# wreuven/h264-scroll-encoder

Measured on AMD Instinct MI355X. Metric: composed frames/sec (1280x720, 360x360 dyn) at 1/2/4/8 GPU; bit-exact vs CPU, higher is better.
Workload: dtype u8; 1 GPU; BASELINE config 3: 256 concurrent 1280x720 streams + 360x360 synthetic dynamic rect (4x4 int transform + quant + CAVLC), composer_write_scroll_frame semantics; resolution=1280x720, streams_per_gpu=256, parallelism=static stream shard x1, no RCCL

## Files before the change

h264-scroll-encoder_amd/csrc/batch.h:

```cpp
#ifndef SCROLL_BATCH_H
#define SCROLL_BATCH_H

#include <hip/hip_runtime.h>

#include <stddef.h>
#include <stdint.h>

#include <vector>

#include "engine.h"
#include "dyn_engine.h"
#include "splice_engine.h"
#include "ingest_engine.h"
#include "pick_engine.h"

#define HIPCHK(x)                                                                  \
    do {                                                                           \
        hipError_t e_ = (x);                                                       \
        if (e_ != hipSuccess) {                                                    \
            set_err("%s failed: %s", #x, hipGetErrorString(e_));                   \
            return SCROLL_ERR_HIP;                                                 \
        }                                                                          \
    } while (0)

constexpr int NEV = 7;
struct ScrollBatch {
    int device = 0;
    int mode = SCROLL_MODE_COMPOSER;
    int max_streams = 0, max_frames = 0, nstreams = 0;
    int debug = 0;
    size_t arena_bytes = 0, ld_arena = 0;
    int ld_nal = 0;
    DevStream *d_st = nullptr;
    DevStream *h_st = nullptr;
    int32_t *d_off = nullptr;
    NalDesc *d_nal = nullptr;
    uint8_t *d_arena = nullptr;
    hipStream_t own = nullptr;
    hipStream_t last = nullptr;
    hipEvent_t ev[NEV] = {};
    int timing = 0;
    int timed_pending = 0;
    float ms[6] = {0, 0, 0, 0, 0, 0};
    std::vector<hipEvent_t> ring;
    std::vector<uint8_t> ring_dyn;
    int ev_dyn = 0;
    int ring_used = 0;
    double acc_ms[6] = {0, 0, 0, 0, 0, 0};
    int acc_n = 0;
    int host_valid = 1;
    int last_plan_mode = SCROLL_PLAN_COMPOSER;
    int last_nframes = 0;
    std::vector<NalDesc> nal_cache;
    int nal_cache_valid = 0;
    uint64_t *d_dbg = nullptr;
    size_t dbg_slots = 0;
    PlanPending *d_pend = nullptr;
    int dyn_on = 0;
    int dyn_pw = 0, dyn_ph = 0;
    int dyn_refs = 0;
    DynGeom geo{};
    DynFrame *d_dfr = nullptr;
    uint8_t *d_src = nullptr, *d_refs = nullptr, *d_stage = nullptr;
    DynScratch dx{};
    int recon_on = 0;
    uint8_t *d_rec = nullptr;
    unsigned long long *d_sse = nullptr;
    hipEvent_t rc_ev[2] = {};
    int rc_timed = 0;
    int recon_hinted = 0;
    int rc_last_hint = 0;
    std::vector<int> rc_fail;
    struct Probe {
        NalDesc *nal = nullptr;
        DynFrame *dfr = nullptr;
        PlanPending *pend = nullptr;
        uint32_t *rows = nullptr, *ctr = nullptr, *done = nullptr;
        uint4 *heads = nullptr;
        ScrollDynProbe *res = nullptr;
        uint8_t *cls = nullptr;
        int hinted = 0;
        int nframes = -1, nstreams = 0, nq = 0;
        uint8_t qps[SCROLL_DYN_PROBE_MAX_QPS] = {};
        hipEvent_t fin = nullptr;
        hipEvent_t ev[2] = {};
        int timed = 0;
    } pb;
    std::vector<uint8_t> h_qpf;
    int qpf_dev = 0;
    struct Rate {
        long long *level = nullptr;
        uint32_t *fb = nullptr;
        PickOut *out = nullptr;
        hipEvent_t fin = nullptr;
        int nframes = -1, nstreams = 0;
    } rt;
    int hint_on = 0;
    int hint_dirty = 0;
    int hint_max_mb = 0;
    std::vector<std::vector<ScrollHintRect>> h_hint;
    std::vector<int16_t> h_hint_mode;
    HintFrame *d_hf = nullptr;
    ScrollHintRect *d_pool = nullptr;
    size_t pool_cap = 0;
    struct SpliceHost {
        int x0 = 0, y0 = 0, w = 0, h = 0;
        std::vector<uint8_t> nal;
        const uint8_t *dnal = nullptr;
        size_t n = 0;
    };
    std::vector<SpliceHost> h_sp;
    std::vector<int32_t> h_dyn_pos;
    int fallback = 0;
    DynFork fork{};
    std::vector<int32_t> h_dyn_qp;
    int dyn_pos_custom = 0;
    int dyn_qp = 26;
    int hd_dirty = 0;
    uint32_t hd_mb_words = 0;
    size_t dyn_cap = 0;
    int sp_n = 0;
    int sp_dirty = 0;
    int sp_parse = 0;
    SpliceFrame *d_spf = nullptr;
    uint8_t *d_sp_nal = nullptr;
    uint32_t *d_sp_rbsp = nullptr;
    SpliceMbRec *d_sp_rec = nullptr;
    int32_t *d_sp_list = nullptr;
    SpliceUnit *d_sp_units = nullptr;
    int32_t *d_sp_lanes = nullptr;
    size_t sp_lanes_cap = 0, sp_nslots = 0;
    int sp_ymax = 1;
    size_t sp_nal_cap = 0, sp_rbsp_cap = 0, sp_rec_cap = 0, sp_list_cap = 0, sp_units_cap = 0;
    uint8_t *d_ing_in = nullptr;
    size_t ing_in_cap = 0;
    IngestFile *d_ing_files = nullptr;
    IngestScan *d_ing_scan = nullptr;
    IngestOut *d_ing_out = nullptr;
    int ing_cap = 0;
    void *d_ing_work = nullptr;
    size_t ing_work_bytes = 0;
    hipEvent_t ing_ev[2] = {};
    uint32_t *d_ipcm_cnt = nullptr;
    size_t ipcm_cap = 0;
    uint8_t *d_ipcm_stg = nullptr;
    size_t ipcm_stg_cap = 0;
    unsigned long long *d_ipcm_hw = nullptr;
    size_t ipcm_hw_cap = 0;
    uint32_t ipcm_epoch = 0;
    double ipcm_ms = 0.0;
    int ipcm_n = 0;
    uint32_t *ipcm_over = nullptr;
    uint32_t *d_ipcm_sticky = nullptr;
    size_t ipcm_over_stride = 0;
    std::vector<hipEvent_t> ipcm_ev;
    size_t ipcm_ev_used = 0;
    double ing_ms = 0.0;
    int ing_n = 0;
    int dyn_grow = 0;
    int32_t *d_upd = nullptr;
    size_t upd_cap = 0;
    uint64_t *d_out_tab = nullptr;
    size_t out_tab_cap = 0;
    hipEvent_t out_ev = nullptr;
};

#pragma GCC visibility push(hidden)
namespace scroll {
namespace batch {

void set_err(const char *fmt, ...);
int usable_devices(std::vector<int> *ids);
int check_cfg(const ComposerConfig *c);
void cfg_to_dev(const ComposerConfig *c, DevStream *d);
void dev_to_cfg(const DevStream *d, ComposerConfig *c);
hipError_t timing_event(hipEvent_t *e);
int hip_fail(const char *who, hipError_t e, bool clear = false);
int dev_grow(void **p, size_t *cap, size_t n, size_t size, const char *who);
int batch_host_sync(ScrollBatch *b);
int launch(ScrollBatch *b, int nframes, int plan_mode, int nal_max, hipStream_t hs, int plan_flags = 0);
int stream_fail_code(ScrollBatch *b, int s);
int load_nals(ScrollBatch *b);

void probe_release(ScrollBatch *b);
void dyn_release(ScrollBatch *b);
int dyn_grow_pools(ScrollBatch *b);
int dyn_reserve_gen(ScrollBatch *b, size_t need);

void rate_release(ScrollBatch *b);
int qp_frames_any(ScrollBatch *b, bool *any);

int hint_upload(ScrollBatch *b);
int hd_setup(ScrollBatch *b);
int hd_upload(ScrollBatch *b);
int splice_upload(ScrollBatch *b);
int splice_frame_status(ScrollBatch *b, size_t i, int *status);
const char *splice_msg(int e);

int ipcm_async_check(ScrollBatch *b);

}
}
#pragma GCC visibility pop

#endif
```

h264-scroll-encoder_amd/csrc/batch_core.hip:

```cpp
#include <hip/hip_runtime.h>

#include <stdarg.h>
#include <stdint.h>
#include <stdio.h>
#include <stdlib.h>
#include <string.h>

#include <algorithm>
#include <vector>

#include "batch.h"
#include "scroll_engine.h"
#include "dyn_engine.h"
#include "recon_engine.h"
#include "hrecon_engine.h"
#include "hint_engine.h"
#include "splice_engine.h"
#include "hdyn_engine.h"

using namespace scroll::batch;

static void event_ms(const hipEvent_t *e, bool dyn, bool lite, float out[6])
{
    auto el = [&](int a, int b) {
        float v = 0.0f;
        return hipEventElapsedTime(&v, e[a], e[b]) == hipSuccess ? v : 0.0f;
    };
    if (lite) {
        for (int k = 0; k < 6; ++k) out[k] = 0.0f;
        if (dyn) out[2] = out[4] = el(1, 6);
        else out[1] = el(1, 4);
        return;
    }
    if (dyn) {
        out[0] = el(0, 1) + el(2, 3);
        out[1] = el(3, 4);
        out[2] = el(1, 2);
        out[3] = el(4, 5);
        out[4] = el(1, 6);
        out[5] = el(6, 2);
    } else {
        out[0] = el(0, 1);
        out[1] = el(1, 4);
        out[2] = out[3] = out[4] = out[5] = 0.0f;
    }
}

static void fold_ring(ScrollBatch *b)
{
    for (int i = 0; i + NEV <= b->ring_used; i += NEV) {
        float m[6];
        event_ms(&b->ring[i], (b->ring_dyn[i / NEV] & 1) != 0, (b->ring_dyn[i / NEV] & 2) != 0, m);
        for (int k = 0; k < 6; ++k) b->acc_ms[k] += m[k];
        b->acc_n++;
    }
    b->ring_used = 0;
}

static int ring_events(ScrollBatch *b, hipEvent_t **evs)
{
    if ((size_t)b->ring_used + NEV > b->ring.size()) {
        if (b->ring.size() >= (size_t)NEV * 256) {
            HIPCHK(hipStreamSynchronize(b->last));
            fold_ring(b);
        } else {
            for (int i = 0; i < NEV; ++i) {
                hipEvent_t e;
                HIPCHK(timing_event(&e));
                b->ring.push_back(e);
            }
            b->ring_dyn.push_back(0);
        }
    }
    *evs = &b->ring[b->ring_used];
    b->ring_used += NEV;
    return SCROLL_OK;
}

static int dbg_stamps(ScrollBatch *b, size_t slots, hipStream_t hs)
{
    if (slots > b->dbg_slots) {
        if (b->d_dbg) (void)hipFree(b->d_dbg);
        HIPCHK(hipMalloc(&b->d_dbg, slots * 8 * sizeof(uint64_t)));
        b->dbg_slots = slots;
    }
    HIPCHK(hipMemsetAsync(b->d_dbg, 0, slots * 8 * sizeof(uint64_t), hs));
    return SCROLL_OK;
}

static int rc_events(ScrollBatch *b)
{
    if (!b->rc_ev[0]) {
        HIPCHK(hipEventCreate(&b->rc_ev[0]));
        HIPCHK(hipEventCreate(&b->rc_ev[1]));
    }
    return SCROLL_OK;
}

namespace scroll {
namespace batch {

static thread_local char g_err[512];

void set_err(const char *fmt, ...)
{
    va_list ap;
    va_start(ap, fmt);
    vsnprintf(g_err, sizeof(g_err), fmt, ap);
    va_end(ap);
}

int usable_devices(std::vector<int> *ids)
{
    int n = 0;
    if (hipGetDeviceCount(&n) != hipSuccess || n <= 0) {
        set_err("no HIP device visible (libh264scroll needs an MI355X / gfx950)");
        return 0;
    }
    int ok = 0;
    for (int i = 0; i < n; ++i) {
        hipDeviceProp_t p;
        if (hipGetDeviceProperties(&p, i) != hipSuccess) continue;
        if (strncmp(p.gcnArchName, "gfx950", 6) == 0) {
            ok++;
            if (ids) ids->push_back(i);
        }
    }
    if (!ok) set_err("no gfx950 device among %d HIP devices", n);
    return ok;
}

int check_cfg(const ComposerConfig *c)
{
    if (c->log2_max_frame_num < 1 || c->log2_max_frame_num > 16 ||
        (c->pic_order_cnt_type == 0 &&
         (c->log2_max_pic_order_cnt_lsb < 1 || c->log2_max_pic_order_cnt_lsb > 16)) ||
        c->num_waypoints < 0 || c->num_waypoints > MAX_WAYPOINTS || c->width < 0 ||
        c->height < 0) {
        set_err("unsupported ComposerConfig (log2 fields must be 1..16, num_waypoints 0..8)");
        return SCROLL_ERR_CONFIG;
    }
    return SCROLL_OK;
}

void cfg_to_dev(const ComposerConfig *c, DevStream *d)
{
    d->w = c->width;
    d->h = c->height;
    d->log2_mfn = c->log2_max_frame_num;
    d->poc_type = c->pic_order_cnt_type;
    d->log2_poc = c->log2_max_pic_order_cnt_lsb;
    d->deblock = c->deblocking_filter_control_present_flag;
    d->frame_num = c->frame_num;
    d->nwp = c->num_waypoints;
    for (int i = 0; i < 8; ++i) {
        d->wp_off[i] = c->waypoints[i].offset_px;
        d->wp_lt[i] = c->waypoints[i].long_term_idx;
        d->wp_valid[i] = c->waypoints[i].valid;
    }
}

void dev_to_cfg(const DevStream *d, ComposerConfig *c)
{
    c->frame_num = d->frame_num;
    c->num_waypoints = d->nwp;
    for (int i = 0; i < 8; ++i) {
        c->waypoints[i].offset_px = d->wp_off[i];
        c->waypoints[i].long_term_idx = d->wp_lt[i];
        c->waypoints[i].valid = d->wp_valid[i];
    }
}

hipError_t timing_event(hipEvent_t *e)
{
    return hipEventCreateWithFlags(e, hipEventDisableSystemFence);
}

int hip_fail(const char *who, hipError_t e, bool clear)
{
    set_err("%s: %s", who, hipGetErrorString(e));
    if (clear) (void)hipGetLastError();
    return e == hipErrorOutOfMemory ? SCROLL_ERR_OOM : SCROLL_ERR_HIP;
}

int dev_grow(void **p, size_t *cap, size_t n, size_t size, const char *who)
{
    if (n <= *cap) return SCROLL_OK;
    (void)hipFree(*p);
    *p = nullptr;
    *cap = 0;
    hipError_t e = hipMalloc(p, std::max<size_t>(n, 1) * size);
    if (e != hipSuccess) return hip_fail(who, e);
    *cap = n;
    return SCROLL_OK;
}

int batch_host_sync(ScrollBatch *b)
{
    if (b->host_valid) return SCROLL_OK;
    HIPCHK(hipSetDevice(b->device));
    HIPCHK(hipStreamSynchronize(b->last));
    HIPCHK(hipMemcpy(b->h_st, b->d_st, (size_t)b->nstreams * sizeof(DevStream),
                     hipMemcpyDeviceToHost));
    b->host_valid = 1;
    return SCROLL_OK;
}

int launch(ScrollBatch *b, int nframes, int plan_mode, int nal_max, hipStream_t hs, int plan_flags)
{
    int S = b->nstreams;
    if (S == 0) return SCROLL_OK;
    hipEvent_t *rev = nullptr;
    if (b->timing) {
        int rc = ring_events(b, &rev);
        if (rc) return rc;
    }
    const bool hint = b->hint_on && plan_mode != SCROLL_PLAN_EXPLICIT;
    const bool dyn = (b->dyn_on || hint) && plan_mode != SCROLL_PLAN_EXPLICIT;
    const bool lite = b->timing == 2;
    const bool lite_row = lite && dyn && !hint;
    auto mark = [&](int k) -> int {
        if (!b->timing || (!dyn && k != 0 && k != 1 && k != 4)) return SCROLL_OK;
        if (lite) {
            if ((k == 1 || k == (dyn ? 6 : 4)) && !lite_row) HIPCHK(hipEventRecord(rev[k], hs));
            return SCROLL_OK;
        }
        HIPCHK(hipEventRecord(b->ev[k], hs));
        HIPCHK(hipEventRecord(rev[k], hs));
        return SCROLL_OK;
    };
    if (b->timing) {
        b->ring_dyn[(b->ring_used - NEV) / NEV] = (uint8_t)((dyn ? 1 : 0) | (lite ? 2 : 0));
        if (!lite) b->ev_dyn = dyn ? 1 : 0;
    }
    const int ld_fr = b->max_frames;
    const int plan_debug = b->debug & (PLAN_REWIND - 1);
    int rc = mark(0);
    if (rc) return rc;
    if (!dyn) {
        scroll_launch_plan(hs, S, b->d_st, b->d_off, b->max_frames, b->d_nal, b->ld_nal, nframes, plan_mode,
                           plan_debug | plan_flags, b->d_pend, b->d_dfr, ld_fr);
        HIPCHK(hipGetLastError());
        if ((rc = mark(1)) || (rc = mark(2)) || (rc = mark(3))) return rc;
    } else {
        const bool dyn_rect = b->dyn_on && !hint;
        scroll_launch_plan(hs, S, b->d_st, b->d_off, b->max_frames, b->d_nal, b->ld_nal, nframes, plan_mode,
                           plan_debug | plan_flags | PLAN_STATE | PLAN_DYN, b->d_pend, b->d_dfr,
                           ld_fr, nullptr, 0u, 0u, dyn_rect ? b->dx.ctr : nullptr);
        HIPCHK(hipGetLastError());
        if ((rc = mark(1))) return rc;
        uint64_t *stamps = nullptr;
        if (b->debug & SCROLL_DEBUG_DYN_STAMPS) {
            const size_t slots = (2 + (size_t)b->geo.ngroups) * (size_t)nframes * S;
            if ((rc = dbg_stamps(b, slots, hs))) return rc;
            stamps = b->d_dbg + 2 * (size_t)nframes * S * 8;
        }
        b->geo.debug = b->debug;
        if (hint) {
            if (b->sp_parse) {
                if (splice_launch_parse(hs, b->sp_n, b->sp_ymax, b->d_sp_list, b->d_spf, b->d_sp_units,
                                        b->d_sp_lanes, b->sp_nslots, b->d_st, ld_fr, b->d_sp_rbsp, b->d_sp_rec)) {
                    set_err("k_splice_parse launch: %s", hipGetErrorString(hipGetLastError()));
                    return SCROLL_ERR_HIP;
                }
                b->sp_parse = 0;
            }
            if (b->fallback && b->dyn_on &&
                hint_launch_fb(hs, nframes, S, b->d_st, b->d_nal, b->ld_nal, b->d_pend, b->d_dfr, ld_fr,
                               b->d_hf, b->d_pool)) {
                set_err("k_hint_fb launch: %s", hipGetErrorString(hipGetLastError()));
                return SCROLL_ERR_HIP;
            }
            if (hint_launch_stage(hs, nframes, S, b->d_st, b->d_nal, b->ld_nal, b->d_pend,
                                  b->d_dfr, ld_fr, b->d_hf, b->d_pool, b->d_stage,
                                  b->geo.slot_bytes)) {
                set_err("k_hint_stage launch: %s", hipGetErrorString(hipGetLastError()));
                return SCROLL_ERR_HIP;
            }
            const bool combined = b->dyn_on;
            if (combined &&
                hdyn_launch_code(hs, nframes, S, b->d_st, b->d_nal, b->ld_nal, b->d_pend, b->d_dfr, ld_fr,
                                 b->d_hf, b->d_pool, b->d_spf, &b->geo, b->d_src, b->d_refs,
                                 b->d_sp_rec, b->d_sp_rbsp, b->hd_mb_words)) {
                set_err("k_hdyn_code launch: %s", hipGetErrorString(hipGetLastError()));
                return SCROLL_ERR_HIP;
            }
            if (combined && b->recon_on && b->recon_hinted) {
                const bool timed = b->timing != 0;
                if (timed && (rc = rc_events(b))) return rc;
                if (hrecon_launch(hs, nframes, S, b->d_st, b->d_nal, b->ld_nal, b->d_pend, b->d_dfr, ld_fr,
                                  b->d_hf, b->d_pool, b->d_spf, &b->geo, b->d_src, b->d_refs, b->d_rec, b->d_sse,
                                  timed ? b->rc_ev[0] : nullptr, timed ? b->rc_ev[1] : nullptr)) {
                    set_err("k_hdyn_recon launch: %s", hipGetErrorString(hipGetLastError()));
                    return SCROLL_ERR_HIP;
                }
                b->rc_timed = timed ? 1 : 0;
                b->rc_last_hint = 1;
                std::fill(b->rc_fail.begin(), b->rc_fail.end(), 0);
            }
            if ((b->sp_n > 0 || combined) &&
                splice_launch_stage(hs, nframes, S, b->d_st, b->d_nal, b->ld_nal, b->d_pend,
                                    b->d_dfr, ld_fr, b->d_hf, b->d_pool, b->d_spf, b->d_sp_rec,
                                    b->d_sp_rbsp, b->d_stage, b->geo.slot_bytes)) {
                set_err("k_splice_stage launch: %s", hipGetErrorString(hipGetLastError()));
                return SCROLL_ERR_HIP;
            }
            if ((rc = mark(6))) return rc;
        } else {
            b->dx.epoch = b->dx.epoch % 0xffffffu + 1u;
            const DynGeom &G = b->geo;
            const DynFork *fk = nullptr;
            static const bool fork_on = [] {
                const char *e = getenv("SCROLL_DYN_FORK");
                return e && e[0] == '1';
            }();
            if (fork_on) {
                if (!b->fork.side) {
                    HIPCHK(hipStreamCreateWithFlags(&b->fork.side, hipStreamNonBlocking));
                    HIPCHK(hipEventCreateWithFlags(&b->fork.e0, hipEventDisableTiming));
                    HIPCHK(hipEventCreateWithFlags(&b->fork.e1, hipEventDisableTiming));
                }
                fk = &b->fork;
            }
            if (dyn_launch_code(hs, nframes, S, b->d_st, b->d_nal, b->ld_nal, b->d_pend, b->d_dfr, ld_fr, &G,
                                b->d_src, b->d_refs, &b->dx, b->dx.epoch, b->dyn_pw / 16, stamps, fk,
                                lite_row ? rev[1] : nullptr, lite_row ? rev[6] : nullptr)) {
                set_err("k_dyn_code launch: %s", hipGetErrorString(hipGetLastError()));
                return SCROLL_ERR_HIP;
            }
            if ((rc = mark(6))) return rc;
            if (b->recon_on) {
                const bool timed = b->timing != 0;
                if (timed && (rc = rc_events(b))) return rc;
                if (recon_launch(hs, nframes, S, b->d_st, b->d_nal, b->ld_nal, b->d_pend, b->d_dfr, ld_fr, &G,
                                 b->dx.rows, b->d_src, b->d_refs, b->d_rec, b->d_sse, b->dx.ctr,
                                 timed ? b->rc_ev[0] : nullptr, timed ? b->rc_ev[1] : nullptr)) {
                    set_err("k_dyn_recon launch: %s", hipGetErrorString(hipGetLastError()));
                    return SCROLL_ERR_HIP;
                }
                b->rc_timed = timed ? 1 : 0;
                b->rc_last_hint = 0;
            }
            if (dyn_launch_pack(hs, nframes, S, b->d_st, b->d_nal, b->ld_nal, b->d_pend, b->d_dfr, ld_fr, &G,
                                &b->dx, b->d_stage, stamps ? b->d_dbg : nullptr, fk)) {
                set_err("k_dyn_static / k_dyn_epfix launch: %s", hipGetErrorString(hipGetLastError()));
                return SCROLL_ERR_HIP;
            }
        }
        if ((rc = mark(2))) return rc;
        scroll_launch_plan(hs, S, b->d_st, b->d_off, b->max_frames, b->d_nal, b->ld_nal, nframes, plan_mode,
                           plan_debug | plan_flags | PLAN_SIZE | PLAN_DYN, b->d_pend, b->d_dfr,
                           ld_fr, (b->dyn_on && !b->hint_on) ? (const uint32_t *)b->dx.ctr : nullptr,
                           b->geo.rs_spill_cap, b->geo.gen_cap);
        HIPCHK(hipGetLastError());
        if ((rc = mark(3))) return rc;
    }
    const size_t slots = scroll_emit_stamp_slots(nal_max, S);
    if (slots && (b->debug & SCROLL_DEBUG_EMIT_STAMPS) && (rc = dbg_stamps(b, slots, hs))) return rc;
    scroll_launch_emit(hs, S, nal_max, b->d_st, b->d_nal, b->ld_nal, b->d_arena, (uint64_t)b->ld_arena, b->debug,
                       b->d_dbg);
    HIPCHK(hipGetLastError());
    if ((rc = mark(4))) return rc;
    if (dyn && dyn_launch_emit(hs, nframes, S, b->d_st, b->d_nal, b->ld_nal, b->d_dfr, ld_fr,
                               &b->geo, b->d_stage, hint ? nullptr : &b->dx, b->d_arena,
                               (uint64_t)b->ld_arena,
                               (b->debug & SCROLL_DEBUG_DYN_STAMPS) && b->d_dbg
                                   ? b->d_dbg + (size_t)nframes * S * 8 : nullptr)) {
        set_err("k_dyn_gather launch: %s", hipGetErrorString(hipGetLastError()));
        return SCROLL_ERR_HIP;
    }
    if ((rc = mark(5))) return rc;
    if (b->timing == 1) b->timed_pending = 1;
    b->host_valid = 0;
    b->nal_cache_valid = 0;
    b->last = hs;
    return SCROLL_OK;
}

int stream_fail_code(ScrollBatch *b, int s)
{
    const int32_t e = b->h_st[s].err;
    if (!e) return SCROLL_OK;
    if (e & SCROLL_DEVERR_HANDOFF) return SCROLL_ERR_DEVICE;
    if (e & SCROLL_DEVERR_SPLICE) {
        int st = 0;
        for (int ff = 0; ff < b->max_frames && !st; ++ff)
            if (splice_frame_status(b, (size_t)s * b->max_frames + ff, &st)) break;
        return st == HDYN_STATUS_OVERFLOW ? SCROLL_ERR_OVERFLOW : SCROLL_ERR_CONFIG;
    }
    if (e & SCROLL_DEVERR_HINT) return SCROLL_ERR_CONFIG;
    return SCROLL_ERR_OVERFLOW;
}

int load_nals(ScrollBatch *b)
{
    if (b->nal_cache_valid) return SCROLL_OK;
    int rc = batch_host_sync(b);
    if (rc) return rc;
    b->nal_cache.resize((size_t)b->nstreams * b->ld_nal);
    HIPCHK(hipMemcpy(b->nal_cache.data(), b->d_nal, b->nal_cache.size() * sizeof(NalDesc),
                     hipMemcpyDeviceToHost));
    b->nal_cache_valid = 1;
    return SCROLL_OK;
}

}
}

extern "C" {

const char *scroll_last_error(void) { return g_err; }

const char *scroll_version(void) { return "h264scroll-amd 0.1 (gfx950)"; }

int scroll_device_count(void) { return usable_devices(nullptr); }

int scroll_batch_create(ScrollBatch **out, const ScrollBatchDesc *desc)
{
    if (!out || !desc || desc->max_streams <= 0 || desc->max_frames <= 0 ||
        desc->arena_bytes == 0 ||
        (desc->mode != SCROLL_MODE_COMPOSER && desc->mode != SCROLL_MODE_EXPERIMENT)) {
        set_err("scroll_batch_create: bad descriptor");
        return SCROLL_ERR_ARG;
    }
    *out = nullptr;
    std::vector<int> ids;
    if (!usable_devices(&ids)) return SCROLL_ERR_NO_DEVICE;
    int n = 0;
    (void)hipGetDeviceCount(&n);
    if (desc->device < 0 || desc->device >= n) {
        set_err("scroll_batch_create: device %d out of range (%d visible)", desc->device, n);
        return SCROLL_ERR_ARG;
    }
    bool ok = false;
    for (int i : ids) ok |= (i == desc->device);
    if (!ok) {
        set_err("scroll_batch_create: device %d is not gfx950", desc->device);
        return SCROLL_ERR_NO_DEVICE;
    }
    HIPCHK(hipSetDevice(desc->device));
    ScrollBatch *b = new ScrollBatch();
    b->device = desc->device;
    b->mode = desc->mode;
    b->max_streams = desc->max_streams;
    b->max_frames = desc->max_frames;
    b->arena_bytes = desc->arena_bytes;
    b->ld_arena = (desc->arena_bytes + 128 + 255) & ~(size_t)255;
    b->ld_nal = 2 * desc->max_frames;
    size_t S = (size_t)desc->max_streams;
    hipError_t e = hipSuccess;
    if (e == hipSuccess) e = hipMalloc(&b->d_st, S * sizeof(DevStream));
    if (e == hipSuccess) e = hipHostMalloc(&b->h_st, S * sizeof(DevStream), hipHostMallocDefault);
    if (e == hipSuccess) e = hipMalloc(&b->d_off, S * (size_t)desc->max_frames * sizeof(int32_t));
    if (e == hipSuccess) e = hipMalloc(&b->d_nal, S * (size_t)b->ld_nal * sizeof(NalDesc));
    if (e == hipSuccess) e = hipMalloc(&b->d_arena, S * b->ld_arena);
    if (e == hipSuccess) e = hipMalloc(&b->d_pend, S * sizeof(PlanPending));
    if (e == hipSuccess) e = hipStreamCreateWithFlags(&b->own, hipStreamNonBlocking);
    for (int i = 0; i < NEV && e == hipSuccess; ++i) e = timing_event(&b->ev[i]);
    if (e == hipSuccess) e = hipMemset(b->d_st, 0, S * sizeof(DevStream));
    if (e == hipSuccess) e = hipMemset(b->d_off, 0, S * (size_t)desc->max_frames * sizeof(int32_t));
    if (e != hipSuccess) {
        scroll_batch_destroy(b);
        return hip_fail("scroll_batch_create", e);
    }
    memset(b->h_st, 0, S * sizeof(DevStream));
    b->last = b->own;
    *out = b;
    return SCROLL_OK;
}

void scroll_batch_destroy(ScrollBatch *b)
{
    if (!b) return;
    (void)hipSetDevice(b->device);
    if (b->own) (void)hipStreamSynchronize(b->own);
    for (int i = 0; i < NEV; ++i)
        if (b->ev[i]) (void)hipEventDestroy(b->ev[i]);
    for (hipEvent_t e : b->ring) (void)hipEventDestroy(e);
    if (b->fork.side) {
        (void)hipStreamSynchronize(b->fork.side);
        (void)hipStreamDestroy(b->fork.side);
        (void)hipEventDestroy(b->fork.e0);
        (void)hipEventDestroy(b->fork.e1);
    }
    if (b->own) (void)hipStreamDestroy(b->own);
    (void)hipFree(b->d_st);
    (void)hipHostFree(b->h_st);
    (void)hipFree(b->d_off);
    (void)hipFree(b->d_nal);
    (void)hipFree(b->d_arena);
    (void)hipFree(b->d_out_tab);
    (void)hipFree(b->d_upd);
    if (b->out_ev) (void)hipEventDestroy(b->out_ev);
    (void)hipFree(b->d_pend);
    (void)hipFree(b->d_dfr);
    (void)hipFree(b->d_src);
    (void)hipFree(b->d_refs);
    (void)hipFree(b->d_stage);
    (void)hipFree(b->d_rec);
    (void)hipFree(b->d_sse);
    for (hipEvent_t e : b->rc_ev)
        if (e) (void)hipEventDestroy(e);
    probe_release(b);
    (void)hipFree(b->dx.qpf);
    rate_release(b);
    (void)hipFree(b->d_hf);
    (void)hipFree(b->d_pool);
    (void)hipFree(b->d_spf);
    (void)hipFree(b->d_sp_nal);
    (void)hipFree(b->d_sp_rbsp);
    (void)hipFree(b->d_sp_rec);
    (void)hipFree(b->d_sp_list);
    (void)hipFree(b->d_sp_units);
    (void)hipFree(b->d_sp_lanes);
    (void)hipFree(b->d_ing_in);
    (void)hipFree(b->d_ipcm_cnt);
    (void)hipFree(b->d_ipcm_stg);
    (void)hipFree(b->d_ipcm_hw);
    (void)hipFree(b->d_ing_files);
    (void)hipFree(b->d_ing_scan);
    (void)hipFree(b->d_ing_out);
    (void)hipFree(b->d_ing_work);
    for (hipEvent_t e : b->ing_ev)
        if (e) (void)hipEventDestroy(e);
    for (hipEvent_t e : b->ipcm_ev)
        if (e) (void)hipEventDestroy(e);
    (void)hipFree(b->d_ipcm_sticky);
    if (b->d_dbg) (void)hipFree(b->d_dbg);
    delete b;
}

int scroll_batch_num_streams(const ScrollBatch *b) { return b ? b->nstreams : 0; }

int scroll_batch_set_debug(ScrollBatch *b, int flags)
{
    if (!b) return SCROLL_ERR_ARG;
    b->debug = flags;
    return SCROLL_OK;
}

int scroll_batch_add_stream(ScrollBatch *b, const ComposerConfig *cfg)
{
    if (!b || !cfg) return SCROLL_ERR_ARG;
    if (b->nstreams >= b->max_streams) {
        set_err("scroll_batch_add_stream: batch full (%d streams)", b->max_streams);
        return SCROLL_ERR_ARG;
    }
    int rc = check_cfg(cfg);
    if (rc) return rc;
    if (b->dyn_on && (cfg->width != b->dyn_pw || cfg->height != b->dyn_ph)) {
        set_err("scroll_batch_add_stream: the dynamic rect needs %dx%d streams", b->dyn_pw,
                b->dyn_ph);
        return SCROLL_ERR_CONFIG;
    }
    if (b->hint_on && ((cfg->width / 16) * (cfg->height / 16) > b->hint_max_mb ||
                       cfg->width / 16 > HINT_MAX_MBW)) {
        set_err("scroll_batch_add_stream: hint staging slots hold %d MBs per picture, %d per row",
                b->hint_max_mb, HINT_MAX_MBW);
        return SCROLL_ERR_CONFIG;
    }
    rc = batch_host_sync(b);
    if (rc) return rc;
    int s = b->nstreams;
    DevStream *d = &b->h_st[s];
    if (b->dyn_qp != 26 && !cfg->deblocking_filter_control_present_flag) {
        set_err("scroll_batch_add_stream: a stream with the deblocking filter on (no "
                "deblocking_filter_control_present_flag) needs the rect at QP 26, the batch's is %d",
                b->dyn_qp);
        return SCROLL_ERR_CONFIG;
    }
    memset(d, 0, sizeof(*d));
    cfg_to_dev(cfg, d);
    d->dyn_qp = b->dyn_qp;
    d->out_pos = 0;
    d->out_cap = b->arena_bytes;
    HIPCHK(hipSetDevice(b->device));
    HIPCHK(hipMemcpy(b->d_st + s, d, sizeof(DevStream), hipMemcpyHostToDevice));
    b->nstreams++;
    return s;
}

int scroll_batch_get_config(ScrollBatch *b, int s, ComposerConfig *cfg)
{
    if (!b || !cfg || s < 0 || s >= b->nstreams) return SCROLL_ERR_ARG;
    int rc = batch_host_sync(b);
    if (rc) return rc;
    const DevStream *d = &b->h_st[s];
    composer_config_init(cfg, d->w, d->h);
    cfg->log2_max_frame_num = d->log2_mfn;
    cfg->pic_order_cnt_type = d->poc_type;
    cfg->log2_max_pic_order_cnt_lsb = d->log2_poc;
    cfg->deblocking_filter_control_present_flag = d->deblock;
    dev_to_cfg(d, cfg);
    return SCROLL_OK;
}

int scroll_batch_set_config(ScrollBatch *b, int s, const ComposerConfig *cfg)
{
    if (!b || !cfg || s < 0 || s >= b->nstreams) return SCROLL_ERR_ARG;
    int rc = check_cfg(cfg);
    if (rc) return rc;
    rc = batch_host_sync(b);
    if (rc) return rc;
    DevStream *d = &b->h_st[s];
    if (!cfg->deblocking_filter_control_present_flag) {
        bool bad = d->dyn_qp != 26;
        const size_t F = (size_t)b->max_frames, i0 = (size_t)s * F;
        for (size_t f = 0; !bad && f < F && i0 + f < b->h_dyn_qp.size(); ++f) {
            const int q = b->h_dyn_qp[i0 + f];
            bad = q >= 0 && q != 26;
        }
        bool any = false;
        if (!bad && b->dx.qpf && !qp_frames_any(b, &any))
            for (size_t f = 0; !bad && f < F; ++f) bad = b->h_qpf[i0 + f] != 0xFFu && b->h_qpf[i0 + f] != 26u;
        if (bad) {
            set_err("scroll_batch_set_config: stream %d's rect QP is not 26: it cannot turn the deblocking "
                    "filter on (no deblocking_filter_control_present_flag)", s);
            return SCROLL_ERR_CONFIG;
        }
    }
    cfg_to_dev(cfg, d);
    HIPCHK(hipSetDevice(b->device));
    HIPCHK(hipMemcpy(b->d_st + s, d, sizeof(DevStream), hipMemcpyHostToDevice));
    return SCROLL_OK;
}

int scroll_batch_set_offsets(ScrollBatch *b, const int32_t *offsets, int nframes)
{
    if (!b || !offsets || nframes < 0 || nframes > b->max_frames) return SCROLL_ERR_ARG;
    if (nframes == 0 || b->nstreams == 0) return SCROLL_OK;
    HIPCHK(hipSetDevice(b->device));
    HIPCHK(hipMemcpy2D(b->d_off, (size_t)b->max_frames * sizeof(int32_t), offsets,
                       (size_t)nframes * sizeof(int32_t), (size_t)nframes * sizeof(int32_t),
                       (size_t)b->nstreams, hipMemcpyHostToDevice));
    return SCROLL_OK;
}

int32_t *scroll_batch_offsets_device(ScrollBatch *b) { return b ? b->d_off : nullptr; }

int scroll_batch_compose(ScrollBatch *b, int nframes, void *hip_stream)
{
    return scroll_batch_compose_ex(b, nframes, hip_stream, 0);
}

int scroll_batch_compose_ex(ScrollBatch *b, int nframes, void *hip_stream, int flags)
{
    if (!b || nframes < 0 || nframes > b->max_frames) {
        set_err("scroll_batch_compose: nframes %d out of range", nframes);
        return SCROLL_ERR_ARG;
    }
    if (b->dyn_on && !b->dyn_refs) {
        set_err("scroll_batch_compose: dynamic rect without reference pictures");
        return SCROLL_ERR_CONFIG;
    }
    HIPCHK(hipSetDevice(b->device));
    const bool combined = b->hint_on && b->dyn_on;
    if (b->dyn_pos_custom && !b->hint_on) {
        set_err("scroll_batch_compose: per-frame dynamic rect positions need UI hints "
                "(scroll_batch_set_hints)");
        return SCROLL_ERR_CONFIG;
    }
    if (b->recon_on && b->hint_on) {
        bool spliced = b->sp_n > 0;
        for (const ScrollBatch::SpliceHost &sp : b->h_sp) spliced |= sp.w > 0;
        if (!b->recon_hinted || spliced) {
            set_err("scroll_batch_compose: the dynamic rect's reconstruction (scroll_batch_set_dyn_recon) "
                    "covers the plain dynamic rect, and the rect under UI hints with "
                    "scroll_batch_set_dyn_recon_hinted, never spliced slices: clear the hints / splices, opt "
                    "in or turn it off");
            return SCROLL_ERR_CONFIG;
        }
    }
    if (b->hint_on && b->dx.qpf) {
        bool any = false;
        int rc = qp_frames_any(b, &any);
        if (rc) return rc;
        if (any) {
            set_err("scroll_batch_compose: per-frame rect QPs are set (scroll_batch_set_dyn_qp_frames / "
                    "scroll_batch_dyn_pick) and so are UI hints: clear one of them "
                    "(scroll_batch_clear_dyn_qp_frames; under hints: scroll_batch_set_dyn_qp_at)");
            return SCROLL_ERR_CONFIG;
        }
    }
    if (b->hint_on && b->sp_dirty) {
        int rc = splice_upload(b);
        if (rc) return rc;
        if (combined) b->hd_dirty = 1;
    }
    if (combined && b->hd_dirty) {
        int rc = hd_upload(b);
        if (rc) return rc;
    }
    if (b->hint_on && b->hint_dirty) {
        int rc = hint_upload(b);
        if (rc) return rc;
    }
    hipStream_t hs = hip_stream ? (hipStream_t)hip_stream : b->own;
    int plan = b->mode == SCROLL_MODE_EXPERIMENT ? SCROLL_PLAN_EXPERIMENT : SCROLL_PLAN_COMPOSER;
    int nal_max = plan == SCROLL_PLAN_COMPOSER ? 2 * nframes : nframes;
    b->last_plan_mode = plan;
    b->last_nframes = nframes;
    return launch(b, nframes, plan, nal_max, hs,
                  (flags & SCROLL_COMPOSE_REWIND) ? PLAN_REWIND : 0);
}

int scroll_batch_sync(ScrollBatch *b)
{
    if (!b) return SCROLL_ERR_ARG;
    {
        int rc0 = batch_host_sync(b);
        if (rc0) return rc0;
        if ((rc0 = ipcm_async_check(b))) return rc0;
    }
    if (b->timed_pending) {
        event_ms(b->ev, b->ev_dyn != 0, false, b->ms);
        b->timed_pending = 0;
    }
    int rc = SCROLL_OK;
    for (int s = 0; s < b->nstreams; ++s) {
        if (!b->h_st[s].err) continue;
        if (b->rc_last_hint && (size_t)s < b->rc_fail.size())
            b->rc_fail[s] = stream_fail_code(b, s);
        if (rc == SCROLL_OK && (b->h_st[s].err & SCROLL_DEVERR_HANDOFF)) {
            set_err("stream %d: a dynamic-rect row waited past its bound for the row above's "
                    "TotalCoeffs (k_dyn_row hand-off); the stream committed nothing", s);
            rc = SCROLL_ERR_DEVICE;
        } else if (rc == SCROLL_OK && (b->h_st[s].err & SCROLL_DEVERR_SPLICE)) {
            int st = 0, ff = 0;
            for (; ff < b->max_frames && !st; ++ff)
                if (splice_frame_status(b, (size_t)s * b->max_frames + ff, &st)) break;
            if (st == HDYN_STATUS_OVERFLOW) {
                set_err("stream %d frame %d: a dynamic-rect MB under hints outgrew its %u-byte "
                        "region (raise slot_bytes of scroll_batch_set_dyn_rect)", s, ff - 1,
                        4u * b->hd_mb_words);
                rc = SCROLL_ERR_OVERFLOW;
            } else {
                set_err("stream %d frame %d: %s: %s", s, ff - 1,
                        b->dyn_on ? "dynamic rect under hints" : "spliced slice", splice_msg(st));
                rc = SCROLL_ERR_CONFIG;
            }
        } else if (rc == SCROLL_OK && (b->h_st[s].err & SCROLL_DEVERR_HINT)) {
            set_err("stream %d: a hint rect names a reference that is not valid in its frame "
                    "(ref 2 + i needs waypoint i)", s);
            rc = SCROLL_ERR_CONFIG;
        } else if (rc == SCROLL_OK && (b->h_st[s].err & SCROLL_DEVERR_DYN)) {
            uint32_t used[2] = {0, 0};
            if (b->dyn_on && !b->hint_on && b->dx.ctr)
                HIPCHK(hipMemcpy(used, b->dx.ctr, sizeof(used), hipMemcpyDeviceToHost));
            if (used[0] > b->geo.rs_spill_cap || used[1] > b->geo.gen_cap) {
                const int grc = dyn_grow_pools(b);
                set_err("stream %d: the dynamic rect's %s pool ran out (%u of %u); %s", s,
                        used[0] > b->geo.rs_spill_cap ? "row-stage spill" : "general-path record",
                        used[0] > b->geo.rs_spill_cap ? used[0] : used[1],
                        used[0] > b->geo.rs_spill_cap ? b->geo.rs_spill_cap : b->geo.gen_cap,
                        grc ? "growing it failed" : "grown: compose again");
            } else {
                set_err("stream %d: a staged NAL outgrew its staging slot (%llu bytes)", s,
                        (unsigned long long)b->geo.slot_bytes);
            }
            rc = SCROLL_ERR_OVERFLOW;
        } else if (rc == SCROLL_OK) {
            set_err("stream %d: output arena overflow (%llu bytes used, capacity %llu)", s,
                    (unsigned long long)b->h_st[s].out_pos,
                    (unsigned long long)b->h_st[s].out_cap);
            rc = SCROLL_ERR_OVERFLOW;
        }
        b->h_st[s].err = 0;
        HIPCHK(hipMemcpy(&b->d_st[s].err, &b->h_st[s].err, sizeof(int32_t),
                         hipMemcpyHostToDevice));
    }
    if (rc) return rc;
    return SCROLL_OK;
}

size_t scroll_batch_output_size(ScrollBatch *b, int s)
{
    if (!b || s < 0 || s >= b->nstreams || batch_host_sync(b)) return 0;
    return (size_t)b->h_st[s].out_pos;
}

int scroll_batch_copy_output(ScrollBatch *b, int s, size_t from, uint8_t *dst, size_t n)
{
    if (!b || s < 0 || s >= b->nstreams || (!dst && n)) return SCROLL_ERR_ARG;
    int rc = batch_host_sync(b);
    if (rc) return rc;
    if (from + n > b->h_st[s].out_pos) {
        set_err("scroll_batch_copy_output: range beyond stream output");
// ... 178 lines not shown
```

h264-scroll-encoder_amd/csrc/dyn_engine.h:

```cpp
#ifndef SCROLL_DYN_ENGINE_H
#define SCROLL_DYN_ENGINE_H

#include <hip/hip_runtime.h>
#include "engine.h"

typedef struct {
    uint32_t *rows;
    uint16_t *meta;
    uint2 *body_lo, *body_hi;
    uint4 *body_w;
    uint4 *heads;
    unsigned long long *tcx;
    uint32_t *rowstage;
    uint32_t *gbits;
    uint32_t *spill;
    uint32_t *ctr;
    uint32_t ctr_frames;
    uint32_t epoch;
    uint8_t *qpf;
} DynScratch;
#define DYN_HEAD_VECS 16
#define DYN_CTR_LIST 4

typedef struct {
    hipStream_t side;
    hipEvent_t e0, e1;
} DynFork;
int dyn_launch_rows(hipStream_t hs, int nframes, int S, const DevStream *st, const NalDesc *nal, int ld_nal,
                    const PlanPending *pend, DynFrame *dfr, int ld_fr, const DynGeom *g, uint32_t *rows,
                    uint32_t *ctr, uint4 *heads, const uint8_t *qpf);
int dyn_launch_code(hipStream_t hs, int nframes, int S, DevStream *st, const NalDesc *nal,
                    int ld_nal, const PlanPending *pend, DynFrame *dfr, int ld_fr,
                    const DynGeom *g, const uint8_t *src, const uint8_t *refs, const DynScratch *x,
                    uint32_t epoch, int mbw, uint64_t *stamps, const DynFork *fk, hipEvent_t ev0 = nullptr,
                    hipEvent_t ev1 = nullptr);
int dyn_launch_static(hipStream_t hs, int nframes, int S, DevStream *st, const NalDesc *nal, int ld_nal,
                      const PlanPending *pend, DynFrame *dfr, int ld_fr, const DynGeom *g, const DynScratch *x);
int dyn_launch_pack(hipStream_t hs, int nframes, int S, DevStream *st, const NalDesc *nal,
                    int ld_nal, const PlanPending *pend, DynFrame *dfr, int ld_fr,
                    const DynGeom *g, const DynScratch *x, uint8_t *eps, uint64_t *stamps, const DynFork *fk);
int dyn_launch_emit(hipStream_t hs, int nframes, int S, const DevStream *st, const NalDesc *nal,
                    int ld_nal, const DynFrame *dfr, int ld_fr, const DynGeom *g,
                    const uint8_t *stage, const DynScratch *x, uint8_t *arena, uint64_t ld_arena,
                    uint64_t *stamps);
int dyn_launch_synth(hipStream_t hs, int nframes, int S, uint8_t *src, const DynGeom *g,
                     int stream_base, int t0);

void dyn_rowstage_geom(DynGeom *g, int mbw, int mbh);
size_t dyn_slot_bound(int mbw, int mbh, int rw, int rh);
uint32_t dyn_ep_cap(int rw, int rh, int debug);

#endif
```

h264-scroll-encoder_amd/csrc/dyn_kernels.hip:

```cpp
#include <hip/hip_runtime.h>

#include <stdint.h>
#include <mutex>

#include "dyn_device.h"
#include "dyn_engine.h"
#include "nal_ctx.h"
#include "stage_util.h"

using namespace scroll;
using namespace scroll::dyn;
using namespace scroll::stage;

namespace {

__constant__ Tabs g_tabs = SCROLL_DYN_TABS;
constexpr Tabs k_tabs = SCROLL_DYN_TABS;
__constant__ PTabs g_ptabs = make_ptabs(k_tabs);
__device__ uint32_t g_tzrb[TZRB_N];
__constant__ LvTab g_lvt = make_lvt();

struct QpPair {
    QParams l, c;
};
struct QpTab {
    QpPair q[QP_MAX + 1];
};
constexpr QpTab make_qptab()
{
    QpTab T{};
    for (int i = 0; i <= QP_MAX; ++i) T.q[i] = QpPair{qparams(i), qparams(qp_chroma(i))};
    return T;
}
__constant__ QpTab g_qptab = make_qptab();

__global__ __launch_bounds__(256) void k_tzrb_init()
{
    const int i = blockIdx.x * 256 + threadIdx.x;
    if (i < TZRB_N) g_tzrb[i] = i < 65536 ? tzrb_entry(g_tabs, (uint32_t)i, 16) : tzrb_entry(g_tabs, (uint32_t)(i - 65536), 15);
}

__device__ inline void load_ptabs(PTabs &dst, int t, int nthr)
{
    constexpr int N = (int)(sizeof(PTabs) / 16);
    static_assert(sizeof(PTabs) % 16 == 0, "PTabs copies as uint4");
    for (int i = t; i < N; i += nthr) reinterpret_cast<uint4 *>(&dst)[i] = reinterpret_cast<const uint4 *>(&g_ptabs)[i];
}

__device__ inline void load_rowtabs(RowTabs &dst, int t, int nthr)
{
    constexpr int NC = (int)(sizeof(dst.ct) / 4), NZ = (int)(sizeof(dst.tzdc) / 4), NR = (int)(sizeof(dst.rb) / 4);
    static_assert(sizeof(dst.ct) % 4 == 0 && sizeof(dst.tzdc) % 4 == 0 && sizeof(dst.rb) % 4 == 0, "word copies");
    const uint32_t *ct = reinterpret_cast<const uint32_t *>(g_ptabs.ct);
    const uint32_t *tz = reinterpret_cast<const uint32_t *>(g_ptabs.tzdc);
    const uint32_t *rb = reinterpret_cast<const uint32_t *>(g_ptabs.rb);
    uint32_t *dc = reinterpret_cast<uint32_t *>(dst.ct), *dz = reinterpret_cast<uint32_t *>(dst.tzdc);
    uint32_t *dr = reinterpret_cast<uint32_t *>(dst.rb);
    for (int i = t; i < NC + NZ + NR; i += nthr) {
        if (i < NC) dc[i] = ct[i];
        else if (i < NC + NZ) dz[i - NC] = tz[i - NC];
        else dr[i - NC - NZ] = rb[i - NC - NZ];
    }
}


constexpr int HEAD_MAX = 160;
constexpr int HDR_MAX = 1024;
constexpr int OBUF = 6400;

constexpr uint32_t DF_OVER = 1u, DF_GENERAL = 2u, DF_HANDOFF = 4u;
constexpr uint64_t HANDOFF_TICKS = 5000000ull;
constexpr uint64_t HANDOFF_GAP = 100000ull;
constexpr uint32_t DF_EPSLOW = 0x100u;
constexpr uint32_t DF_FIXED = 0x200u;

constexpr int EPC_ROW = 256, EPC_STATIC = 4096;

__device__ inline uint32_t ep_data(uint32_t w, uint32_t gi, uint32_t bits)
{
    const uint32_t b0 = 32u * gi;
    if (__builtin_expect(b0 + 32u <= bits, 1)) return w;
    return w | (bits > b0 ? 0xffffffffu >> (bits - b0) : 0xffffffffu);
}

__device__ inline uint32_t ep_run_starts(uint32_t pw, uint32_t w, uint32_t nx, uint32_t gi, uint32_t bits)
{
    uint64_t X = (uint64_t)ep_data(w, gi, bits) << 32 | ep_data(nx, gi + 1u, bits);
    X |= X << 1;
    X |= X << 2;
    X |= X << 4;
    X |= X << 8;
    X |= X << 6;
    const uint32_t z22 = ~(uint32_t)(X >> 32);
    return z22 & ((ep_data(w, gi, bits) >> 1) | (pw << 31));
}

__device__ inline bool ep_quick(uint32_t w, uint32_t nx)
{
    uint32_t y = w | w << 1;
    y |= y << 2;
    y |= y << 4;
    y |= y << 8;
    y |= y << 6;
    const uint32_t tz = w ? (uint32_t)__builtin_ctz(w) : 32u, lz = nx ? (uint32_t)__builtin_clz(nx) : 32u;
    return (~y & 0xffe00000u) != 0u || tz + lz >= 22u;
}

__device__ inline void flush_window(const uint32_t *buf, uint32_t n, uint32_t p0, bool last, uint32_t *out,
                                    uint32_t *ncand, uint32_t *cg, uint32_t cmax, int t, int nthr)
{
    const int lane = t & 63;
    for (uint32_t i0 = 0; i0 < n; i0 += (uint32_t)nthr) {
        const uint32_t i = i0 + (uint32_t)t;
        bool q = false;
        if (i < n) {
            const uint32_t w = buf[i];
            out[p0 + i] = w;
            q = ep_quick(w, i + 1 < n ? buf[i + 1] : (last ? 0xffffffffu : 0u));
        }
        const uint64_t m = __builtin_amdgcn_ballot_w64(q);
        if (m) {
            uint32_t base = 0;
            if (lane == (int)__builtin_ctzll(m)) base = atomicAdd(ncand, (uint32_t)__builtin_popcountll(m));
            base = (uint32_t)__shfl((int)base, (int)__builtin_ctzll(m), 64);
            const uint32_t k = base + (uint32_t)__builtin_popcountll(m & ((1ull << lane) - 1ull));
            if (q && k < cmax) cg[1 + k] = p0 + i;
        }
    }
}

__device__ inline uint32_t ld32(const uint8_t *p) { return *reinterpret_cast<const uint32_t *>(p); }

constexpr int NPC = DYN_PIECES;

__device__ inline void put_body(uint2 *BL, uint2 *BH, size_t i, uint4 v, bool hi)
{
    BL[i] = make_uint2(v.x, v.y);
    if (hi) BH[i] = make_uint2(v.z, v.w);
}

__device__ inline uint4 get_body(const uint2 *BL, const uint2 *BH, size_t i, bool hi)
{
    const uint2 a = BL[i], b = hi ? BH[i] : make_uint2(0u, 0u);
    return make_uint4(a.x, a.y, b.x, b.y);
}

__device__ inline int rec_of(int q, int pc, int ndt)
{
    return pc < 16 ? 16 * q + pc : (pc < 18 ? 24 * ndt + 2 * q + (pc - 16) : 16 * ndt + 8 * q + (pc - 18));
}
constexpr uint32_t M_OVF = 1u << 15;
constexpr uint32_t ROW_GEN = 1u << 31, ROW_OFF = 0x0fffffffu;

#ifndef SCROLL_CODE_T
#define SCROLL_CODE_T 256
#endif
constexpr int CODE_T = SCROLL_CODE_T, CODE_NW = CODE_T / 64;
#ifndef SCROLL_SORT_KEYS
#define SCROLL_SORT_KEYS 9
#endif
constexpr int SORT_KEYS = SCROLL_SORT_KEYS;
static_assert(SORT_KEYS >= 2 && SORT_KEYS <= 17, "TotalCoeff classes");

__device__ inline void code_frame(const DevStream *__restrict__ st,
                                                     const DynFrame *__restrict__ dfr, int ld_fr,
                                                     const PlanPending *__restrict__ pend,
                                                     const NalDesc *__restrict__ nal, int ld_nal,
                                                     DynGeom g, const uint32_t *__restrict__ rows,
                                                     const uint8_t *__restrict__ src,
                                                     const uint8_t *__restrict__ refs,
                                                     uint16_t *__restrict__ meta, uint2 *__restrict__ blo,
                                                     uint2 *__restrict__ bhi, uint4 *__restrict__ bwd, int s,
                                                     int f, int bx)
{
    __shared__ uint4 lv[CODE_T];
    __shared__ int16_t lw[CODE_T][16];
    __shared__ uint16_t wc[CODE_NW][SORT_KEYS];
    __shared__ uint16_t order[CODE_T];
    __shared__ PTabs ptabs;
    __shared__ int32_t wo[8], wv[8];
    const int t = threadIdx.x;
    const int lane = t & 63, wave = t >> 6;
    const DynFrame df = dfr[(size_t)s * ld_fr + f];
    if (df.nal < 0 || !(df.err & DF_GENERAL)) return;
    load_ptabs(ptabs, t, CODE_T);
    if (t < 8) {
        wo[t] = pend[s].wo[t];
        wv[t] = pend[s].wv[t];
    }
    __syncthreads();

    const int ndt = g.w * g.h, ntask = 24 * ndt;
    const int task = bx * CODE_T + t;
    const int qpy = __builtin_amdgcn_readfirstlane((int)df.ep);
    const QParams ql = qparams_rt(qpy), qc = qparams_rt(qp_chroma(qpy));
    const bool wide = qpy < QP_MIN;
    const size_t nb = (size_t)s * ld_fr + f;
    const uint32_t *rw = rows + nb * (size_t)(32 * g.h);
    const int w = st[s].w, h = st[s].h;
    const uint32_t ysz = (uint32_t)w * (uint32_t)h, csz = ysz / 4;
    const uint8_t *rb = refs + (size_t)s * g.ref_ld;
    const uint8_t *fs = src + (size_t)s * g.src_ld + (size_t)f * g.src_fr;
    const int lstride = 16 * g.w, cstride = 8 * g.w;
    const uint8_t *fcb = fs + (size_t)256 * ndt, *fcr = fcb + (size_t)64 * ndt;
    const uint32_t m_rw = magic32((uint32_t)g.w);
    const size_t gs = df.rbsp_bytes;
    uint16_t *M = meta + gs * (size_t)(NPC * ndt);
    uint2 *BL = blo + gs * (size_t)(NPC * ndt), *BH = bhi + gs * (size_t)(NPC * ndt);
    uint4 *BW = bwd + gs * (size_t)(NPC * ndt);

    const bool luma = task < 16 * ndt;
    const bool act = task < ntask;
    int k, r, p = 0;
    if (luma) {
        k = task >> 4;
        r = task & 15;
    } else {
        const int jj = task - 16 * ndt;
        k = jj >> 3;
        p = (jj >> 2) & 1;
        r = jj & 3;
    }
    const int ry = (int)div_m((uint32_t)k, m_rw), cx = k - ry * g.w;
    const int col = g.x0 + cx;
    uint32_t pk[4] = {0, 0, 0, 0};
    int n = 0, w0 = 0;
    if (act && luma) {
        const int bx = r & 3, by = r >> 2;
        const uint8_t *sp = fs + (size_t)(16 * ry + 4 * by) * lstride + 16 * cx + 4 * bx;
        const uint8_t *pp = rb + 16 * col + 4 * bx;
        const uint32_t *re = rw + 16 * ry + 4 * by;
        uint32_t sv[4], pv[4];
#pragma unroll
        for (int i = 0; i < 4; ++i) {
            sv[i] = ld32(sp + (size_t)i * lstride);
            pv[i] = ld32(pp + re[i]);
        }
        int res[16], W[16];
#pragma unroll
        for (int i = 0; i < 4; ++i)
#pragma unroll
            for (int x = 0; x < 4; ++x)
                res[4 * i + x] = (int)((sv[i] >> (8 * x)) & 255u) - (int)((pv[i] >> (8 * x)) & 255u);
        fwd4x4(res, W);
#pragma unroll
        for (int k2 = 0; k2 < 16; ++k2) {
            const int v = quant(W[ZZ[k2]], ZZ[k2], ql);
            pk[k2 >> 2] |= ((uint32_t)v & 255u) << (8 * (k2 & 3));
            if (wide) lw[t][k2] = (int16_t)v;
            n += v != 0;
        }
    } else if (act) {
        const int bx = r & 1, by = r >> 1;
        const uint8_t *sp = (p ? fcr : fcb) + (size_t)(8 * ry + 4 * by) * cstride + 8 * cx + 4 * bx;
        const int X = 8 * col + 4 * bx;
        const uint8_t *cp = rb + (size_t)p * csz + X;
        const uint32_t *re = rw + 16 * g.h + 8 * ry + 4 * by;
        int res[16], W[16];
#pragma unroll
        for (int i = 0; i < 4; ++i) {
            const uint32_t sv = ld32(sp + (size_t)i * cstride);
            const uint32_t ea = re[i];
            int pred[4];
            if (!(ea & ROW_GEN)) {
                const uint32_t fr = (ea >> 28) & 7u;
                const uint32_t av = ld32(cp + (ea & ROW_OFF));
                const uint32_t bv = fr ? ld32(cp + (re[8 * g.h + i] & ROW_OFF)) : 0u;
#pragma unroll
                for (int x = 0; x < 4; ++x) {
                    const int a = (int)((av >> (8 * x)) & 255u), b = (int)((bv >> (8 * x)) & 255u);
                    pred[x] = ((8 - (int)fr) * a + (int)fr * b + 4) >> 3;
                }
            } else {
                {
                    const NalDesc d = nal[(size_t)s * ld_nal + df.nal];
                    const int off = d.off, a_end = (h - off) / 16;
                    const int row = g.y0 + ry;
                    int32_t wl0[8] = {0, 0, 0, 0, 0, 0, 0, 0};
                    const NalCtx c = nal_ctx(st + s, d, wo, wl0, wv);
                    const Regions rg = regions(c);
                    const bool cA = row < a_end;
                    const int ref = cA ? rg.ra : rg.rb, q = 4 * (cA ? rg.mva : rg.mvb);
                    const int o = q >> 3, fr = q & 7;
                    const WpTab T{wo, wv, h};
                    RefPics P;
                    P.w = w;
                    P.h = h;
                    const size_t pic = (size_t)ysz + 2 * csz;
                    for (int i2 = 0; i2 < 2; ++i2) {
                        P.pl[i2][0] = rb + i2 * pic;
                        P.pl[i2][1] = P.pl[i2][0] + ysz;
                        P.pl[i2][2] = P.pl[i2][1] + csz;
                    }
                    const int ya = 8 * row + 4 * by + i + o;
                    for (int x = 0; x < 4; ++x) {
                        const int a = chroma_px_any<9>(T, P, ref, 1 + p, X + x, ya);
                        const int b = fr ? chroma_px_any<9>(T, P, ref, 1 + p, X + x, ya + 1) : 0;
                        pred[x] = ((8 - fr) * a + fr * b + 4) >> 3;
                    }
                }
            }
#pragma unroll
            for (int x = 0; x < 4; ++x) res[4 * i + x] = (int)((sv >> (8 * x)) & 255u) - pred[x];
        }
        fwd4x4(res, W);
        w0 = W[0];
#pragma unroll
        for (int k2 = 1; k2 < 16; ++k2) {
            const int v = quant(W[ZZ[k2]], ZZ[k2], qc);
            pk[(k2 - 1) >> 2] |= ((uint32_t)v & 255u) << (8 * ((k2 - 1) & 3));
// ... 32 lines not shown
            CapSink cap{0, 0, 0};
            const int tc = cavlc_dc4(cap, ptabs, dq);
            const size_t idx = (size_t)24 * ndt + 2 * k + p;
            if (cap.n <= 128) {
                M[idx] = (uint16_t)(cap.n | (uint32_t)tc << 8);
                if (cap.n)
                    put_body(BL, BH, idx, make_uint4((uint32_t)cap.lo, (uint32_t)(cap.lo >> 32), (uint32_t)cap.hi,
                                                     (uint32_t)(cap.hi >> 32)), cap.n > 64);
            } else {
                M[idx] = (uint16_t)((uint32_t)tc << 8 | M_OVF);
                put_body(BL, BH, idx, make_uint4(((uint32_t)dq[0] & 0xffffu) | (uint32_t)dq[1] << 16,
                                                 ((uint32_t)dq[2] & 0xffffu) | (uint32_t)dq[3] << 16, 0u, 0u), false);
            }
        }
        if (t < SORT_KEYS) {
            uint32_t tot = 0;
#pragma unroll
            for (int w2 = 0; w2 < CODE_NW; ++w2) tot += wc[w2][t];
            uint32_t kb = tot;
#pragma unroll
            for (int d = 1; d < 32; d <<= 1) {
                const uint32_t o = __shfl_up(kb, d, 64);
                if (lane >= d) kb += o;
            }
            uint32_t run = kb - tot;
#pragma unroll
            for (int w2 = 0; w2 < CODE_NW; ++w2) {
                const uint32_t c = wc[w2][t];
                wc[w2][t] = (uint16_t)run;
                run += c;
            }
        }
        __syncthreads();
        order[wc[wave][key] + below] = (uint16_t)t;
    }
    __syncthreads();
    const int u = order[t];
    const int tk = bx * CODE_T + u;
    const uint4 v4 = lv[u];
    const bool ul = tk < 16 * ndt;
    CapSink cap{0, 0, 0};
    int t1 = 0;
    bool ok = true;
    int tc = 0;
    if (tk < ntask && !wide) {
        tc = cavlc_body(cap, ptabs, v4, ul ? 16 : 15, t1, ok);
    } else if (tk < ntask) {
        const int max = ul ? 16 : 15;
        tc = tc_t1_of(lw[u], max, t1);
        uint32_t tv;
        int tl;
        coeff_token(g_tabs, tc, t1, 0, tv, tl);
        SkipSink<CapSink> sk{cap, (uint32_t)tl};
        cavlc_block(sk, g_tabs, lw[u], max, 0);
        ok = cap.n <= 128;
    }
    if (tk < ntask) {
        const uint16_t mm = ok ? (uint16_t)(cap.n | (uint32_t)tc << 8 | (uint32_t)t1 << 13)
                               : (uint16_t)((uint32_t)tc << 8 | (uint32_t)t1 << 13 | M_OVF);
        M[tk] = mm;
        uint4 ov = v4;
        if (wide && !ok) {
            const uint4 *l2 = reinterpret_cast<const uint4 *>(lw[u]);
            ov = l2[0];
            BW[tk] = l2[1];
        }
        if ((mm & 255u) || (mm & M_OVF))
            put_body(BL, BH, tk,
                     ok ? make_uint4((uint32_t)cap.lo, (uint32_t)(cap.lo >> 32), (uint32_t)cap.hi,
                                     (uint32_t)(cap.hi >> 32))
                        : ov,
                     (mm & 255u) > 64u || (mm & M_OVF));
    }
}

#ifndef SCROLL_CODE_GEN_Y
#define SCROLL_CODE_GEN_Y 64
#endif
constexpr int CODE_GEN_Y = SCROLL_CODE_GEN_Y;
__global__ __launch_bounds__(CODE_T) void k_dyn_code_general(const DevStream *__restrict__ st,
                                                             const DynFrame *__restrict__ dfr, int ld_fr,
                                                             const PlanPending *__restrict__ pend,
                                                             const NalDesc *__restrict__ nal, int ld_nal,
                                                             DynGeom g, const uint32_t *__restrict__ rows,
                                                             const uint8_t *__restrict__ src,
                                                             const uint8_t *__restrict__ refs,
                                                             uint16_t *__restrict__ meta,
                                                             uint2 *__restrict__ blo, uint2 *__restrict__ bhi,
                                                             uint4 *__restrict__ bwd, const uint32_t *__restrict__ ctr)
{
    const uint32_t n = min(__builtin_amdgcn_readfirstlane(ctr[1]), g.gen_cap);
    for (uint32_t j = blockIdx.y; j < n; j += gridDim.y) {
        const uint32_t q = __builtin_amdgcn_readfirstlane(ctr[DYN_CTR_LIST + j]);
        const int s = (int)(q / (uint32_t)ld_fr), f = (int)(q - (uint32_t)s * (uint32_t)ld_fr);
        code_frame(st, dfr, ld_fr, pend, nal, ld_nal, g, rows, src, refs, meta, blo, bhi, bwd, s, f, blockIdx.x);
        __syncthreads();
    }
}

struct LdsOrWin {
    uint32_t *b;
    uint32_t lo, n;
    __device__ inline void operator()(uint32_t i, uint32_t v) const
    {
        const uint32_t k = i - lo;
        if (k < n) atomicOr(&b[k], v);
    }
};
typedef OrSink<LdsOrWin> WSink;


__device__ inline int tc_of(uint32_t m) { return (int)((m >> 8) & 31u); }

struct HeadSel {
    int a_end, mbw;
    __device__ inline int sel(int row, int col) const
    {
        const bool curA = row < a_end, abvA = (row - 1) < a_end;
        return 3 * (row == 0 ? 0 : (curA ? 1 : (abvA ? 2 : 3))) + (col == 0 ? 0 : (col == mbw - 1 ? 2 : 1));
    }
};
struct HeadCtx : HeadSel {
    Regions rg;
    int nrefs;
    template <class S>
    __device__ inline void put_class(S &sk, int cls) const
    {
        const int ty = cls / 3, pos = cls - 3 * ty;
        const int x = pos == 0 ? 0 : (pos == 1 ? min(1, mbw - 1) : mbw - 1);
        const bool cur = ty == 0 ? 0 < a_end : ty == 1;
        const bool abv = ty == 1 || ty == 2;
        const int ref = cur ? rg.ra : rg.rb, mv4 = 4 * (cur ? rg.mva : rg.mvb);
        const int aref = abv ? rg.ra : rg.rb, amv4 = 4 * (abv ? rg.mva : rg.mvb);
        int px, py;
        predict(x, ty == 0 ? 0 : 1, mbw, ref, mv4, aref, amv4, px, py);
        put_mb_head(sk, ref, 0 - px, mv4 - py, nrefs);
    }
    template <class S>
    __device__ inline void put_slow(S &sk, int row, int col) const
    {
        const bool curA = row < a_end, abvA = (row - 1) < a_end;
        const int ref = curA ? rg.ra : rg.rb, mv4 = 4 * (curA ? rg.mva : rg.mvb);
        const int aref = abvA ? rg.ra : rg.rb, amv4 = 4 * (abvA ? rg.mva : rg.mvb);
        int px, py;
        predict(col, row, mbw, ref, mv4, aref, amv4, px, py);
        put_mb_head(sk, ref, 0 - px, mv4 - py, nrefs);
    }
};

__device__ inline HeadCtx head_ctx(const NalCtx &c)
{
    HeadCtx H;
    H.rg = regions(c);
    H.a_end = (c.h - c.off) / 16;
    H.mbw = c.w / 16;
    H.nrefs = 2 + c.nwp;
    return H;
}

__device__ inline HeadSel head_sel(const DevStream *S, const NalDesc &d)
{
    HeadSel H;
    H.a_end = (S->h - d.off) / 16;
    H.mbw = S->w / 16;
    return H;
}

__device__ inline uint32_t row_static_bits(const HeadCtx &H, const uint32_t *hlen, int row, const Rect &R)
{
    const int mbw = H.mbw;
    const bool in = row >= R.y0 && row < R.y0 + R.h;
    auto isdyn = [&](int col) { return in && col >= R.x0 && col < R.x0 + R.w; };
    const int base = H.sel(row, 0) - 0;
    uint32_t bits = isdyn(0) ? 0u : hlen[base] + 1u;
    if (mbw >= 2) {
        if (!isdyn(mbw - 1)) bits += hlen[base + 2] + 1u;
        int nmid = mbw - 2;
        if (in) nmid -= max(0, min(R.x0 + R.w, mbw - 1) - max(R.x0, 1));
        bits += (uint32_t)nmid * (hlen[base + 1] + 1u);
    }
    return bits;
}

__device__ inline void lb_store(unsigned long long *p, uint64_t v)
{
    __hip_atomic_store(p, v, __ATOMIC_RELAXED, __HIP_MEMORY_SCOPE_AGENT);
}

__host__ __device__ inline uint64_t rs_group_words(const DynGeom &g, int nA, int gi)
{
    if (gi < nA) return (uint64_t)gi * g.rs_static_words;
    if (gi < nA + g.h) return (uint64_t)nA * g.rs_static_words + (uint64_t)(gi - nA) * g.rs_row_words;
    return (uint64_t)(gi - g.h) * g.rs_static_words + (uint64_t)g.h * g.rs_row_words;
}

__host__ __device__ inline uint64_t rs_runs_words(const DynGeom &g, int nA, int gi)
{
    const bool row = gi >= nA && gi < nA + g.h;
    return rs_group_words(g, nA, gi) + (row ? g.rs_row_words - EPC_ROW : g.rs_static_words - EPC_STATIC);
}

constexpr uint32_t LO_LEN = 0x7ffu;

__device__ inline void piece_token(const uint16_t (*ct)[68], uint32_t mv, int nC, uint32_t &tv, uint32_t &tl)
{
    const int tc = tc_of(mv), t1 = (int)((mv >> 13) & 3u);
    if (nC >= 8) {
        tv = tc ? (uint32_t)(((tc - 1) << 2) | t1) : 3u;
        tl = 6;
    } else {
        const uint32_t e = ct[nC < 2 ? 0 : (nC < 4 ? 1 : 2)][4 * tc + t1];
        tv = e & 255u;
        tl = e >> 8;
    }
}

__device__ inline void wave_sync()
{
    __builtin_amdgcn_fence(__ATOMIC_RELEASE, "wavefront");
    __builtin_amdgcn_wave_barrier();
    __builtin_amdgcn_fence(__ATOMIC_ACQUIRE, "wavefront");
}

template <int CTRL, int ROWS>
__device__ inline uint32_t dpp_or0(uint32_t v)
{
    return (uint32_t)__builtin_amdgcn_update_dpp(0, (int)v, CTRL, ROWS, 0xf, false);
}

__device__ inline uint32_t seg32_incl_sum(uint32_t v)
{
    v += dpp_or0<0x111, 0xf>(v);
    v += dpp_or0<0x112, 0xf>(v);
    v += dpp_or0<0x114, 0xf>(v);
    v += dpp_or0<0x118, 0xf>(v);
    v += dpp_or0<0x142, 0xa>(v);
    return v;
}

__device__ inline uint32_t wave_incl_sum_dpp(uint32_t v)
{
    v = seg32_incl_sum(v);
    v += dpp_or0<0x143, 0xc>(v);
    return v;
}

template <class S>
__device__ inline void ovf_code(S &sk, const PTabs &PT, const Tabs &TB, uint4 bd, const uint4 *bw, int pc, int nC)
{
    if (nC == -1) {
        const int dq[4] = {(int)(int16_t)(bd.x & 0xffffu), (int)(int16_t)(bd.x >> 16),
                           (int)(int16_t)(bd.y & 0xffffu), (int)(int16_t)(bd.y >> 16)};
        cavlc_dc4(sk, PT, dq);
    } else if (bw) {
        const uint4 hi = *bw;
        const uint32_t w8[8] = {bd.x, bd.y, bd.z, bd.w, hi.x, hi.y, hi.z, hi.w};
        int16_t l16[16];
#pragma unroll
        for (int i = 0; i < 8; ++i) {
            l16[2 * i] = (int16_t)(w8[i] & 0xffffu);
            l16[2 * i + 1] = (int16_t)(w8[i] >> 16);
        }
        cavlc_block(sk, TB, l16, pc < 16 ? 16 : 15, nC);
    } else {
        const int8_t *lvp = reinterpret_cast<const int8_t *>(&bd);
        cavlc_block(sk, TB, lvp, pc < 16 ? 16 : 15, nC);
    }
}

__device__ __attribute__((noinline)) uint32_t ovf_bits(const PTabs &PT, const Tabs &TB, uint4 bd, const uint4 *bw,
                                                       int pc, int nC)
{
    CountSink cn{0};
    ovf_code(cn, PT, TB, bd, bw, pc, nC);
    return cn.n;
}

typedef __attribute__((address_space(3))) uint32_t *LdsWords;
__device__ __attribute__((noinline)) void ovf_put(LdsWords win, uint32_t lo, uint32_t n, uint32_t pos,
                                                  const PTabs &PT, const Tabs &TB, uint4 bd, const uint4 *bw, int pc,
                                                  int nC)
{
    uint32_t *buf = (uint32_t *)win;
    WSink sk{LdsOrWin{buf, lo, n}, 0, 0, 0};
    sk.start(pos);
    ovf_code(sk, PT, TB, bd, bw, pc, nC);
    sk.finish();
}

__device__ inline uint4 body_msb(uint64_t hi, uint64_t lo, uint32_t n)
{
    const uint32_t k = 128u - n;
    uint64_t H, Lw;
    if (k >= 64u) {
        H = k >= 128u ? 0ull : lo << (k - 64u);
        Lw = 0ull;
    } else {
        H = k ? (hi << k) | (lo >> (64u - k)) : hi;
        Lw = lo << k;
    }
    return make_uint4((uint32_t)(H >> 32), (uint32_t)H, (uint32_t)(Lw >> 32), (uint32_t)Lw);
}

__global__ __launch_bounds__(256) void k_dyn_rows(const DevStream *__restrict__ st,
                                                  const NalDesc *__restrict__ nal, int ld_nal,
                                                  const PlanPending *__restrict__ pend,
                                                  DynFrame *__restrict__ dfr, int ld_fr, DynGeom g,
                                                  uint32_t *__restrict__ rows, uint32_t *__restrict__ ctr,
                                                  uint4 *__restrict__ heads, const uint8_t *__restrict__ qpf)
{
    __shared__ int32_t wo[8], wl[8], wv[8];
    __shared__ int32_t gen;
    const int s = blockIdx.y, f = blockIdx.x, t = threadIdx.x;
    DynFrame *DF = dfr + (size_t)s * ld_fr + f;
    const int j = DF->nal;
    if (j < 0) return;
    if (t < 8) {
        wo[t] = pend[s].wo[t];
        wl[t] = pend[s].wl[t];
        wv[t] = pend[s].wv[t];
    }
    if (t == 0) gen = 0;
    __syncthreads();
    const DevStream *S = st + s;
    const NalDesc d = nal[(size_t)s * ld_nal + j];
    const NalCtx c = nal_ctx(S, d, wo, wl, wv);
    if (t < 12) {
        const HeadCtx H = head_ctx(c);
        CapSink hc{0, 0, 0};
        H.put_class(hc, t);
        uint4 *hv = heads + ((size_t)s * ld_fr + f) * DYN_HEAD_VECS;
        hv[t] = body_msb(hc.hi, hc.lo, min(hc.n, 128u));
        reinterpret_cast<uint32_t *>(hv + 12)[t] = hc.n | (hc.over() ? 0x80000000u : 0u);
    }
    const Regions rg = regions(c);
    const int w = c.w, h = c.h, a_end = (h - c.off) / 16;
    const uint32_t ysz = (uint32_t)w * (uint32_t)h, pic = ysz + ysz / 2;
    const WpTab T{wo, wv, h};
    uint32_t *rw = rows + ((size_t)s * ld_fr + f) * (size_t)(32 * g.h);
    bool my_gen = false;
    for (int i = t; i < 32 * g.h; i += 256) {
        uint32_t e;
        if (i < 16 * g.h) {
            const int Y = 16 * g.y0 + i, row = Y >> 4;
            const bool cA = row < a_end;
            int yo;
            const int b = luma_row(T, cA ? rg.ra : rg.rb, Y + (cA ? rg.mva : rg.mvb), yo);
            e = (uint32_t)b * pic + (uint32_t)yo * (uint32_t)w;
        } else {
            const int i2 = i - 16 * g.h, bot = i2 >= 8 * g.h;
            const int Y = 8 * g.y0 + (bot ? i2 - 8 * g.h : i2), row = Y >> 3;
            const bool cA = row < a_end;
            const int q = 4 * (cA ? rg.mva : rg.mvb), o = q >> 3, fr = q & 7;
            int yo;
            const int b = chroma_row(T, cA ? rg.ra : rg.rb, Y + o + bot, yo);
            if (b < 0) {
                e = ROW_GEN;
                if (!bot || fr) my_gen = true;
            } else {
                e = ((uint32_t)b * pic + ysz + (uint32_t)yo * (uint32_t)(w / 2)) | (uint32_t)fr << 28;
            }
        }
        rw[i] = e;
    }
    const uint32_t qe = qpf ? qpf[(size_t)s * ld_fr + f] : 0xFFu;
    const int qpy = qe <= 51u ? (int)qe : S->dyn_qp;
    if (my_gen || qpy < QP_MIN) gen = 1;
    __syncthreads();
    if (t == 0) {
        uint32_t e = 0u;
        if (gen) {
            const uint32_t k = atomicAdd(&ctr[1], 1u);
            if (k < g.gen_cap) {
                DF->rbsp_bytes = k;
                ctr[DYN_CTR_LIST + k] = (uint32_t)((size_t)s * ld_fr + f);
                e = DF_GENERAL;
            } else {
                e = DF_OVER;
            }
        }
        DF->err = e;
        DF->ep = (uint32_t)qpy;
    }
}

constexpr int GW = 64;
#ifndef SCROLL_GBUF_WORDS
#define SCROLL_GBUF_WORDS 256
#endif
constexpr int GBUF_WORDS = SCROLL_GBUF_WORDS;

struct StaticFixed {
    uint32_t ncand;
    uint32_t buf[GBUF_WORDS];
    uint64_t hhi[12], hlo[12];
    uint4 pat[12];
    uint32_t hlen[12];
    int32_t head_over;
    int32_t wo[8], wl[8], wv[8];
    uint32_t moff[DYN_STATIC_ROWS + 1];
};

__global__ __launch_bounds__(GW) void k_dyn_static(const DevStream *__restrict__ st,
                                                   const NalDesc *__restrict__ nal, int ld_nal,
                                                   const PlanPending *__restrict__ pend,
                                                   const DynFrame *__restrict__ dfr, int ld_fr, DynGeom g,
                                                   uint32_t *__restrict__ rowstage, uint32_t *__restrict__ gbits)
{
    __shared__ StaticFixed L;
    constexpr int SR = DYN_STATIC_ROWS;
    const Rect R{g.x0, g.y0, g.w, g.h};
    const int nA = max(1, (R.y0 + SR - 1) / SR);
    const int gi = (int)blockIdx.x >= nA ? (int)blockIdx.x + R.h : (int)blockIdx.x;
    const int ng = g.ngroups, f = blockIdx.y, s = blockIdx.z, t = threadIdx.x;
    const size_t nb = (size_t)s * ld_fr + f;
    const DynFrame df = dfr[nb];
    const int j = df.nal;
    if (j < 0) return;
    const bool first = gi == 0, last = gi == ng - 1;
    if (t < 8) {
        L.wo[t] = pend[s].wo[t];
        L.wl[t] = pend[s].wl[t];
        L.wv[t] = pend[s].wv[t];
    }
    if (t == 0) {
        L.head_over = 0;
        L.ncand = 0;
    }
    const DevStream *S = st + s;
    const NalDesc d = nal[(size_t)s * ld_nal + j];
    wave_sync();
    NalCtx c = nal_ctx(S, d, L.wo, L.wl, L.wv);
    c.qpd = (int)df.ep - QP_DEFAULT;
    const HeadCtx H = head_ctx(c);
    const int mbw = H.mbw, mbh = c.h / 16;
    int ra, rb;
    if (gi < nA) {
        ra = gi * SR;
        rb = min(ra + SR, R.y0);
    } else {
        ra = R.y0 + R.h + (gi - nA - R.h) * SR;
        rb = min(ra + SR, mbh);
    }
    uint32_t F = 0;
    if (first) {
        CountSink hc{0};
        emit_slice_header(hc, c);
        F = hc.n;
    }
    if (t < 12) {
        CapSink hc{0, 0, 0};
        H.put_class(hc, t);
        L.hhi[t] = hc.hi;
        L.hlo[t] = hc.lo;
        L.hlen[t] = hc.n;
        if (hc.over()) L.head_over = 1;
        if (hc.n < 128u) {
            const uint64_t hi = (hc.hi << 1) | (hc.lo >> 63), lo = (hc.lo << 1) | 1u;
            L.pat[t] = body_msb(hi, lo, hc.n + 1u);
        } else {
            L.head_over = 1;
        }
    }
    wave_sync();
    const bool head_over = L.head_over;
    auto head_bits = [&](int r, int col) -> uint32_t {
        if (!head_over) return L.hlen[H.sel(r, col)];
        CountSink cn{0};
        H.put_slow(cn, r, col);
        return cn.n;
    };
    uint32_t len = 0;
    const int r = ra + t;
    if (r < rb) {
        if (!head_over) {
            len = row_static_bits(H, L.hlen, r, R);
        } else {
            for (int col = 0; col < mbw; ++col) len += head_bits(r, col) + 1u;
        }
    }
    const uint32_t incl = wave_incl_sum(len, t);
    if (r < rb) L.moff[r - ra] = F + incl - len;
    const uint32_t rows_end = F + __shfl(incl, GW - 1, GW);
    if (t == 0) L.moff[rb - ra] = rows_end;
    const uint32_t bits = rows_end + (last ? 1u : 0u);
    if (t == 0) gbits[nb * (size_t)ng + gi] = bits;
    wave_sync();

    uint32_t *out = rowstage + nb * g.rs_frame_words + rs_group_words(g, nA, gi);
    const uint32_t nw = min((bits + 31u) >> 5, g.rs_static_words - EPC_STATIC);
    const int ne = rb - ra;
    auto cnt_le = [&](uint32_t x) -> int {
        int lo = 0, hi = ne + 1;
        while (lo < hi) {
            const int mid = (lo + hi) >> 1;
            if (L.moff[mid] <= x) lo = mid + 1;
            else hi = mid;
        }
        return lo;
    };
    const uint32_t m_mbw = magic32((uint32_t)mbw);
    for (uint32_t p0 = 0; p0 < nw; p0 += GBUF_WORDS) {
        const uint32_t n = min((uint32_t)GBUF_WORDS, nw - p0);
        for (uint32_t i = (uint32_t)t; i < n; i += GW) L.buf[i] = 0u;
        wave_sync();
        const LdsOrWin win{L.buf, p0, n};
        if (head_over && first && t == 0 && p0 * 32u < F) {
            WSink hs{win, 0, 0, 0};
            hs.start(0);
            emit_slice_header(hs, c);
            hs.finish();
        }
        if (!head_over) {
            const uint32_t rbeg = L.moff[0], rend = L.moff[ne];
            for (uint32_t i = (uint32_t)t; i < n; i += GW) {
                const uint32_t W0 = 32u * (p0 + i), W1 = W0 + 32u;
                uint32_t acc = 0, b = max(W0, rbeg), R0 = 0, R1 = 0, L0 = 0, Lm = 1;
                int b3 = 0;
                float inv = 1.0f;
                while (b < W1 && b < rend) {
                    if (b >= R1 || b < R0) {
                        const int e = cnt_le(b) - 1;
                        R0 = L.moff[e];
                        R1 = L.moff[e + 1];
                        b3 = H.sel(ra + e, 0);
                        L0 = L.hlen[b3] + 1u;
                        Lm = L.hlen[b3 + 1] + 1u;
                        inv = 1.0f / (float)Lm;
                    }
                    const uint32_t o = b - R0;
                    uint32_t cl = (uint32_t)b3, off = o;
                    if (o >= L0) {
                        const uint32_t o2 = o - L0;
                        uint32_t q = (uint32_t)((float)o2 * inv);
                        if (q * Lm > o2) --q;
                        else if ((q + 1u) * Lm <= o2) ++q;
                        if (q < (uint32_t)(mbw - 2)) {
                            cl = (uint32_t)b3 + 1u;
                            off = o2 - q * Lm;
                        } else {
                            cl = (uint32_t)b3 + 2u;
                            off = o2 - (uint32_t)(mbw - 2) * Lm;
                        }
                    }
                    const uint32_t k = min(L.hlen[cl] + 1u - off, W1 - b);
                    const uint4 P = L.pat[cl];
                    const uint32_t wi = off >> 5, sh = off & 31u;
                    const uint32_t w0 = wi == 0 ? P.x : (wi == 1 ? P.y : (wi == 2 ? P.z : P.w));
                    const uint32_t w1 = wi == 0 ? P.y : (wi == 1 ? P.z : (wi == 2 ? P.w : 0u));
                    uint32_t v = sh ? __builtin_amdgcn_alignbit(w0, w1, 32u - sh) : w0;
                    v &= k >= 32u ? 0xffffffffu : ~(0xffffffffu >> k);
                    acc |= v >> (b - W0);
                    b += k;
                }
                L.buf[i] = acc;
            }
            wave_sync();
            if (first && t == 0 && p0 * 32u < F) {
                WSink hs{win, 0, 0, 0};
                hs.start(0);
                emit_slice_header(hs, c);
                hs.finish();
            }
            if (last && t == 0) {
                WSink sk{win, 0, 0, 0};
                sk.start(bits - 1u);
                sk.put(1, 1);
                sk.finish();
            }
            wave_sync();
            flush_window(L.buf, n, p0, p0 + n >= nw, out, &L.ncand,
                         rowstage + nb * g.rs_frame_words + rs_runs_words(g, nA, gi), EPC_STATIC - 1, t, GW);
            wave_sync();
            continue;
        }
        const int ea = max(cnt_le(32u * p0) - 1, 0), eb = min(cnt_le(32u * (p0 + n) - 1u), ne);
        const int nm = eb * mbw;
        for (int m = ea * mbw + t; m < nm; m += GW) {
            const int rr = (int)div_m((uint32_t)m, m_mbw), col = m - rr * mbw, rw = ra + rr;
            uint32_t off = L.moff[rr];
            WSink sk{win, 0, 0, 0};
            if (!head_over) {
                const int b3 = H.sel(rw, 0);
                off += col == 0 ? 0u : L.hlen[b3] + 1u + (uint32_t)(col - 1) * (L.hlen[b3 + 1] + 1u);
                if (off >= 32u * (p0 + n)) continue;
                const int cls = b3 + (col == 0 ? 0 : (col == mbw - 1 ? 2 : 1));
                if (off + L.hlen[cls] + 1u <= 32u * p0) continue;
                sk.start(off);
                sk.put_cap(CapSink{L.hhi[cls], L.hlo[cls], L.hlen[cls]});
            } else {
                for (int c2 = 0; c2 < col; ++c2) off += head_bits(rw, c2) + 1u;
                sk.start(off);
                H.put_slow(sk, rw, col);
            }
            sk.put(1, 1);
            sk.finish();
        }
        if (last && t == 0) {
            WSink sk{win, 0, 0, 0};
            sk.start(bits - 1u);
            sk.put(1, 1);
            sk.finish();
        }
        wave_sync();
        flush_window(L.buf, n, p0, p0 + n >= nw, out, &L.ncand,
                     rowstage + nb * g.rs_frame_words + rs_runs_words(g, nA, gi), EPC_STATIC - 1, t, GW);
        wave_sync();
    }
    if (t == 0) rowstage[nb * g.rs_frame_words + rs_runs_words(g, nA, gi)] = L.ncand;
}


__device__ inline CapSink cap_of_msb(uint64_t a, uint64_t b, uint32_t n)
{
    if (n == 0u) return CapSink{0, 0, 0};
    const uint32_t sh = 128u - n;
    if (sh >= 64u) return CapSink{0, a >> (sh - 64u), n};
    if (sh == 0u) return CapSink{a, b, n};
    return CapSink{a >> sh, (b >> sh) | (a << (64u - sh)), n};
}

__device__ inline void put_piece(uint32_t *buf, uint32_t p0, uint32_t n, uint32_t pos, uint32_t tv, uint32_t tl,
                                 uint4 b, uint32_t bl)
{
    const uint32_t tw = tv & low_mask((int)tl);
    const uint32_t c0 = __builtin_amdgcn_alignbit(tw, b.x, tl), c1 = __builtin_amdgcn_alignbit(b.x, b.y, tl);
    const uint32_t c2 = __builtin_amdgcn_alignbit(b.y, b.z, tl), c3 = __builtin_amdgcn_alignbit(b.z, b.w, tl);
    const uint32_t c4 = __builtin_amdgcn_alignbit(b.w, 0u, tl);
    const uint32_t sh = pos & 31u;
    const uint32_t o[6] = {c0 >> sh, __builtin_amdgcn_alignbit(c0, c1, sh), __builtin_amdgcn_alignbit(c1, c2, sh),
                           __builtin_amdgcn_alignbit(c2, c3, sh), __builtin_amdgcn_alignbit(c3, c4, sh),
                           __builtin_amdgcn_alignbit(c4, 0u, sh)};
    const uint32_t nw = (sh + tl + bl + 31u) >> 5, w0 = (pos >> 5) - p0;
#pragma unroll
    for (uint32_t j = 0; j < 6; ++j)
        if (j < nw && w0 + j < n && o[j]) atomicOr(&buf[w0 + j], o[j]);
}

constexpr uint32_t ROW_PAD = 4;

__device__ inline void put_piece1(uint32_t *buf, uint32_t pos, uint32_t tv, uint32_t tl, uint4 b, uint32_t bl)
{
    const uint32_t tw = tv & low_mask((int)tl);
    const uint32_t c0 = __builtin_amdgcn_alignbit(tw, b.x, tl), c1 = __builtin_amdgcn_alignbit(b.x, b.y, tl);
    const uint32_t c2 = __builtin_amdgcn_alignbit(b.y, b.z, tl), c3 = __builtin_amdgcn_alignbit(b.z, b.w, tl);
    const uint32_t c4 = __builtin_amdgcn_alignbit(b.w, 0u, tl);
    const uint32_t sh = pos & 31u, nw = (sh + tl + bl + 31u) >> 5;
    uint32_t *d = buf + (pos >> 5);
    atomicOr(d, c0 >> sh);
    if (nw > 1u) atomicOr(d + 1, __builtin_amdgcn_alignbit(c0, c1, sh));
    if (nw > 2u) atomicOr(d + 2, __builtin_amdgcn_alignbit(c1, c2, sh));
    if (nw > 3u) {
        atomicOr(d + 3, __builtin_amdgcn_alignbit(c2, c3, sh));
        if (nw > 4u) {
            atomicOr(d + 4, __builtin_amdgcn_alignbit(c3, c4, sh));
            if (nw > 5u) atomicOr(d + 5, __builtin_amdgcn_alignbit(c4, 0u, sh));
        }
    }
}

constexpr int ROW_MAXT = 1024;
#ifndef SCROLL_ROW_WAVES
#define SCROLL_ROW_WAVES 8
#endif
#ifndef SCROLL_ROW_NP
#define SCROLL_ROW_NP 3
#endif
#ifndef SCROLL_ROW_NP_WIDE
#define SCROLL_ROW_NP_WIDE 4
#endif
#ifndef SCROLL_ROW_WIDE
#define SCROLL_ROW_WIDE 40
#endif
constexpr int ROW_NPMAX = 8;
#ifndef SCROLL_ROW_GB
#define SCROLL_ROW_GB 896
#endif
constexpr int ROW_GB = SCROLL_ROW_GB;

struct RowFixed {
    RowTabs ptabs;
    union {
        uint32_t buf[ROW_GB + 4];
        struct {
            uint32_t kc[2][SORT_KEYS];
            uint32_t kc_pad[32 - 2 * SORT_KEYS];
            uint32_t lvt[LVT_N];
        };
    };
    uint64_t hhi[12], hlo[12];
    uint32_t hlen[12];
    int32_t wo[8], wl[8], wv[8];
    int32_t head_over;
    uint32_t rt[32];
    uint32_t ncand;
    uint32_t spill;
    uint32_t pcd[NPC];
};

static_assert(2 * SORT_KEYS <= 32 && 32 + LVT_N <= ROW_GB, "the sort counts and the level table share the bit window");
static_assert(ROW_PAD == 4, "RowFixed::buf holds ROW_PAD spare words");
static_assert(offsetof(RowFixed, lvt) % 8 == 0, "the level table is copied in 8-byte words");

__host__ __device__ inline size_t row_lds_base(int w)
{
    return (size_t)16 * NPC * w + (size_t)4 * (w + 1) + (size_t)2 * (3 * NPC * w) + (size_t)10 * w + 16;
}
#ifndef SCROLL_ROW_GB_WIDE
#define SCROLL_ROW_GB_WIDE 1248
#endif
constexpr int ROW_GB_WIDE = SCROLL_ROW_GB_WIDE;
__host__ __device__ inline size_t row_wide_off(int w) { return (row_lds_base(w) + 15) & ~(size_t)15; }
__host__ __device__ inline bool row_wide_win(int w)
{
    return w > SCROLL_ROW_WIDE && row_wide_off(w) + 4 * (size_t)(ROW_GB_WIDE + ROW_PAD) + sizeof(RowFixed) <= 163840;
}
__host__ __device__ inline size_t row_lds_bytes(int w)
{
    return row_wide_win(w) ? row_wide_off(w) + 4 * (size_t)(ROW_GB_WIDE + ROW_PAD) : row_lds_base(w);
}

__host__ __device__ constexpr uint32_t pc_desc(int pc)
{
    if (pc == 16 || pc == 17) return 1u << 17;
    int da = 0, db = 0, e = 0;
    bool al = false, bt = false;
    if (pc < 16) {
        const int bx = pc & 3, by = pc >> 2;
        al = bx == 0;
        da = al ? 3 - NPC : -1;
        bt = by == 0;
        db = bt ? 0 : -4;
        e = bt ? pc : 0;
    } else {
        const int b = (pc - 18) & 3, bx = b & 1, by = b >> 1;
        al = bx == 0;
        da = al ? 1 - NPC : -1;
        bt = by == 0;
        db = bt ? 0 : -2;
        e = bt ? (pc < 22 ? pc - 14 : pc - 16) : 0;
    }
    return (uint32_t)(da + 32) | (al ? 1u : 0u) << 6 | (uint32_t)(db + 32) << 7 | (bt ? 1u : 0u) << 13 |
           (uint32_t)e << 14;
}

struct EpfLds {
    uint32_t *goff, *gb, *gw, *cw, *cbase, *lst, *cnt;
    uint32_t *ws;
};
__host__ __device__ inline int row_chroma0(int w) { return (16 * w + 63) & ~63; }
__host__ __device__ inline int row_vtasks(int w) { return row_chroma0(w) + 8 * w; }

__host__ __device__ inline int row_threads(int w)
{
    const int nt = row_vtasks(w), np = w > SCROLL_ROW_WIDE ? SCROLL_ROW_NP_WIDE : SCROLL_ROW_NP;
    const int a = (((nt + np - 1) / np) + 63) & ~63;
    const int b = (((nt + ROW_NPMAX - 1) / ROW_NPMAX) + 63) & ~63;
    const int t = a > b ? a : b;
    return t < ROW_MAXT ? t : ROW_MAXT;
}

struct BlkPix {
    uint32_t a[4], b[4], c;
};

__device__ inline __amdgpu_buffer_rsrc_t buf_rsrc(const void *p, uint32_t n)
{
    return __builtin_amdgcn_make_buffer_rsrc(const_cast<void *>(p), (short)0, (int)n, 0x00020000);
}

struct FetchOff {
    uint32_t s, b[4], c;
    int pb;
};

__device__ inline void fetch_luma(FetchOff &o, int v, int ry, const DynGeom &g, const uint32_t *rt)
{
    const int k = v >> 4, r = v & 15, bx = r & 3, by = r >> 2;
    o.s = (uint32_t)((16 * ry + 4 * by) * (16 * g.w) + 16 * k + 4 * bx);
    const uint32_t po = (uint32_t)(16 * (g.x0 + k) + 4 * bx);
#pragma unroll
    for (int i = 0; i < 4; ++i) o.b[i] = po + rt[4 * by + i];
    o.c = o.b[3];
}

__device__ inline void fetch_chroma(FetchOff &o, int e, int ry, const DynGeom &g, uint32_t csz, const uint32_t *ru,
                                    const uint32_t *rd)
{
    const int ndt = g.w * g.h, k = e >> 3, p = (e >> 2) & 1, r = e & 3, bx = r & 1, by = r >> 1;
    o.s = (uint32_t)(256 * ndt + (p ? 64 * ndt : 0) + (8 * ry + 4 * by) * (8 * g.w) + 8 * k + 4 * bx);
    const uint32_t co = (uint32_t)p * csz + (uint32_t)(8 * (g.x0 + k) + 4 * bx);
#pragma unroll
    for (int i = 0; i < 4; ++i) o.b[i] = co + (ru[4 * by + i] & ROW_OFF);
    o.c = co + (rd[4 * by + 3] & ROW_OFF);
}

__device__ inline void fetch_pass9(const FetchOff &o, uint32_t adv, uint32_t stride, __amdgpu_buffer_rsrc_t fs,
                                   __amdgpu_buffer_rsrc_t rb, BlkPix &px)
{
#pragma unroll
    for (int i = 0; i < 4; ++i) {
        px.a[i] = __builtin_amdgcn_raw_buffer_load_b32(fs, o.s, adv + (uint32_t)i * stride, 0);
        px.b[i] = __builtin_amdgcn_raw_buffer_load_b32(rb, o.b[i], adv, 0);
    }
    px.c = __builtin_amdgcn_raw_buffer_load_b32(rb, o.c, adv, 0);
}

__device__ inline uint32_t bilin4(uint32_t b, uint32_t c, uint32_t f)
{
    const uint32_t g = 8u - f;
    const uint32_t be = b & 0x00ff00ffu, bo = (b >> 8) & 0x00ff00ffu;
    const uint32_t ce = c & 0x00ff00ffu, co = (c >> 8) & 0x00ff00ffu;
    const uint32_t ve = __umul24(g, be) + __umul24(f, ce) + 0x00040004u;
    const uint32_t vo = __umul24(g, bo) + __umul24(f, co) + 0x00040004u;
    return ((ve >> 3) & 0x00ff00ffu) | (((vo >> 3) & 0x00ff00ffu) << 8);
}

static_assert(NPC == 26 && NPC * DYN_MAX_W < 18724, "div_npc's reciprocal (10083 / 2^18) is exact below 18724");
__device__ inline int div_npc(int i) { return (int)(__umul24((uint32_t)i, 10083u) >> 18); }

__device__ inline int row_slot(int task, int w)
{
    const int jj = task - 16 * w;
    const bool l = jj < 0;
    const int k = l ? task >> 4 : jj >> 3, pc = l ? task & 15 : 18 + (jj & 7);
    return (int)__umul24((uint32_t)k, (uint32_t)NPC) + pc;
}

struct RowArgs {
    DevStream *st;
    const NalDesc *nal;
    const PlanPending *pend;
    DynFrame *dfr;
    const uint32_t *rows;
    const uint8_t *src, *refs;
    const uint4 *heads;
    int32_t ld_nal, ld_fr;
    DynGeom g;
    unsigned long long *tcx;
    uint32_t epoch, pad0;
    uint32_t *rowstage, *gbits, *spill, *ctr;
    const uint16_t *meta;
    const uint2 *blo, *bhi;
    const uint4 *bwd;
    uint64_t *stamps;
};
static_assert(std::is_trivially_copyable<RowArgs>::value && std::is_standard_layout<RowArgs>::value,
              "RowArgs is copied into the kernel-argument segment as it is: offsetof = kernarg offset");
static_assert(offsetof(RowArgs, st) == 0 && alignof(RowArgs) == 8 && sizeof(RowArgs) % 8 == 0,
              "the only kernel parameter starts the kernel-argument segment");
static_assert(offsetof(RowArgs, tcx) % 16 == 0 && offsetof(RowArgs, epoch) == offsetof(RowArgs, tcx) + 8,
              "tcx and epoch: one 16-byte scalar load");
static_assert(offsetof(RowArgs, gbits) == offsetof(RowArgs, rowstage) + 8 &&
                  offsetof(RowArgs, ctr) == offsetof(RowArgs, rowstage) + 24,
              "phase 5's four pointers are adjacent");

typedef const char __attribute__((address_space(4))) *KargPtr;
__device__ inline KargPtr kargs_here()
{
    KargPtr p = (KargPtr)__builtin_amdgcn_kernarg_segment_ptr();
    asm volatile("" : "+s"(p));
    return p;
}
template <class T>
__device__ inline T karg_at(KargPtr p, size_t off)
{
    return *reinterpret_cast<const T __attribute__((address_space(4))) *>(p + off);
}
#define row_arg(K, F) karg_at<decltype(RowArgs::F)>(K, offsetof(RowArgs, F))

template <bool GEN, bool DBG>
__global__ __launch_bounds__(ROW_MAXT) __attribute__((amdgpu_waves_per_eu(SCROLL_ROW_WAVES))) void k_dyn_row(const RowArgs a)
{
    __shared__ RowFixed L;
    extern __shared__ uint4 rdyn[];
    const DynGeom &g = a.g;
    uint64_t *const stamps = DBG ? a.stamps : nullptr;
    const uint64_t t_entry = stamps ? __builtin_amdgcn_s_memrealtime() : 0ull;
    const int r = blockIdx.x, t = threadIdx.x, T = blockDim.x, lane = t & 63, wave = t >> 6, nwv = T >> 6;
    int f = blockIdx.y, s = blockIdx.z;
    const int ld_fr = a.ld_fr;
    if (GEN) {
        const uint32_t *ctr = a.ctr;
        const uint32_t j = blockIdx.y, n = min(__builtin_amdgcn_readfirstlane(ctr[1]), g.gen_cap);
        if (j >= n) return;
        const uint32_t q = __builtin_amdgcn_readfirstlane(ctr[DYN_CTR_LIST + j]);
        s = (int)(q / (uint32_t)ld_fr);
        f = (int)(q - (uint32_t)s * (uint32_t)ld_fr);
    }
    const size_t nb = (size_t)s * ld_fr + f;
    constexpr bool general = GEN;
    constexpr int SR = DYN_STATIC_ROWS;
    uint64_t *stp = nullptr;
    if (DBG && stamps && t == 0)
        stp = stamps + (((size_t)s * gridDim.y + f) * g.ngroups + (max(1, (g.y0 + SR - 1) / SR) + r)) * 8;
    if (stp) stp[0] = t_entry;
    const Rect R{g.x0, g.y0, g.w, g.h};
    const int w = R.w, ndt = R.w * R.h, row = R.y0 + r, npc = NPC * w, ntask = 24 * w;
    const int nA = max(1, (R.y0 + SR - 1) / SR);
    const DevStream *S = a.st + s;
    const uint32_t *const rows = a.rows;
    const int mbw = g.pw / 16;
    const uint32_t ysz = (uint32_t)g.pw * (uint32_t)g.ph, csz = ysz / 4;
    const int L0 = row_chroma0(w), nl = 16 * w, ntv = L0 + 8 * w;
    const int np = (ntv + T - 1) / T;
    const int wv0 = 64 * __builtin_amdgcn_readfirstlane(wave);
    auto kind_of = [&](int q) -> int {
        const int v0 = q * T + wv0;
        return v0 < nl ? 0 : (v0 < ntv ? 1 : 2);
    };
    const __amdgpu_buffer_rsrc_t fs = buf_rsrc(a.src + (size_t)s * g.src_ld + (size_t)f * g.src_fr, (uint32_t)g.src_fr);
    const __amdgpu_buffer_rsrc_t rb = buf_rsrc(a.refs + (size_t)s * g.ref_ld, 3u * ysz);
// ... 707 lines not shown
                    v = (a[k] & ~(0xffffffffu >> keep)) | (y[0] >> keep);
                }
                a[k] = v;
            }
        }
#pragma unroll
        for (int k = 0; k < 8; ++k) w[k] = __builtin_bswap32(a[k]);
    } else {
#pragma unroll
        for (int k = 0; k < 8; ++k) {
            const uint32_t Pk = P + 32u * (uint32_t)k;
            int g2 = gg;
            w[k] = Pk < T ? __builtin_bswap32(rs_word_span(Pk, g2, ng, T, goff, gb, gw, fr)) : 0u;
        }
    }
}

template <int NT>
__device__ uint32_t ep_scan(const uint32_t *fr, int ng, uint32_t T, const uint32_t *goff, const uint32_t *gb,
                            const uint32_t *gw, uint32_t *cbuf, int *wmax, uint32_t &ep_n, uint32_t *eplist, int t, uint32_t ecap)
{
    constexpr int CH = NT * 4 * EPS_KW;
    const uint32_t nin = (T + 7) >> 3;
    uint4 *cbuf4 = reinterpret_cast<uint4 *>(cbuf);
    if (t == 0) ep_n = 0;
    __syncthreads();
    ScanLoads ld;
    int gcarry = 0;
    if (nin > 0) {
        gcarry = rs_group_at(32u * (uint32_t)t, ng, goff);
        scan_load<NT>(ld, 0u, t, ng, T, goff, gb, gw, fr, gcarry);
    }
    for (uint32_t c0 = 0; c0 < nin; c0 += CH) {
        {
            const uint32_t P0 = c0 * 8u + 32u * (uint32_t)t;
#pragma unroll
            for (int k = 0; k < EPS_KW; ++k) {
                const uint32_t P = P0 + 32u * NT * (uint32_t)k;
                const int g0 = ld.g[k];
                const uint32_t lp = P - goff[g0], sh = lp & 31u;
                uint32_t v = 0;
                if (P < T) {
                    const uint32_t avail = gb[g0] - lp;
                    v = sh ? (ld.x0[k] << sh) | (ld.x1[k] >> (32u - sh)) : ld.x0[k];
                    if (avail < 32u) {
                        v &= ~(0xffffffffu >> avail);
                        if (goff[g0] + gb[g0] < T) {
                            if (g0 + 1 < ng && gb[g0 + 1] >= 32u - avail) {
                                v |= ld.y[k] >> avail;
                            } else {
                                int g2 = g0;
                                v = rs_word_span(P, g2, ng, T, goff, gb, gw, fr);
                            }
                        }
                    }
                }
                cbuf[t + NT * k] = __builtin_bswap32(v);
            }
        }
        const uint32_t cn = c0 + CH;
        if (cn < nin) scan_load<NT>(ld, cn, t, ng, T, goff, gb, gw, fr, gcarry);
        lds_barrier();
        int lz = -1;
        if (t == 0 && c0 > 0 && (cbuf[0] & 255u) <= 3u) {
            for (int64_t P = 8ll * c0 - 32; P >= 0; P -= 32) {
                const uint32_t w = rs_word((uint32_t)P, ng, T, goff, gb, gw, fr);
                if (w) {
                    lz = (int)(P >> 3) + 3 - (__builtin_ctz(w) >> 3);
                    break;
                }
            }
        }
        const uint32_t ib = c0 + 4u * EPS_KW * (uint32_t)t;
        uint32_t wv[EPS_KW];
#pragma unroll
        for (int j = 0; j < EPS_KW / 4; ++j) {
            const uint4 a = cbuf4[(EPS_KW / 4) * t + j];
            wv[4 * j] = a.x; wv[4 * j + 1] = a.y; wv[4 * j + 2] = a.z; wv[4 * j + 3] = a.w;
        }
        int lnz = -1;
#pragma unroll
        for (int w = 0; w < EPS_KW; ++w) {
            const uint32_t m = ib + 4u * w < nin ? wv[w] : 0u;
            if (m) lnz = (int)(ib + 4u * w) + 3 - (__builtin_clz(m) >> 3);
        }
        if (t == 0 && lnz < 0) lnz = lz;
        int ex, tot;
        block_excl_max<NT / 64, true>(lnz, wmax, ex, tot);
        int prev = t == 0 ? lz : ex;
        uint32_t ins = 0;
#pragma unroll
        for (int i = 0; i < 4 * EPS_KW; ++i) {
            const uint32_t gi2 = ib + (uint32_t)i;
            const uint32_t b = gi2 < nin ? (wv[i >> 2] >> (8 * (i & 3))) & 255u : 256u;
            ins |= (ep_insert(b, (int)gi2 - 1 - prev) ? 1u : 0u) << i;
            prev = b ? (int)gi2 : prev;
        }
        if (ins) {
            uint32_t k = atomicAdd(&ep_n, (uint32_t)__builtin_popcount(ins));
            while (ins) {
                const int i = __builtin_ctz(ins);
                ins &= ins - 1u;
                if (k < ecap) eplist[k] = ib + (uint32_t)i;
                k++;
            }
        }
    }
    __syncthreads();
    return ep_n;
}

#ifndef SCROLL_EPF_T
#define SCROLL_EPF_T 128
#endif
#ifndef SCROLL_EPF_LIST
#define SCROLL_EPF_LIST 2048
#endif
constexpr int EPF_T = SCROLL_EPF_T;

__device__ inline void ep_put(uint32_t j, bool bm, uint32_t *lst, uint32_t *nlst, uint32_t lcap)
{
    if (bm) {
        atomicOr(&lst[j >> 5], 1u << (j & 31u));
    } else {
        const uint32_t q = atomicAdd(nlst, 1u);
        if (q < lcap) lst[q] = j;
    }
}

__device__ inline void ep_eval_bytes(uint32_t B, uint32_t Bend, uint32_t nin, int ng, uint32_t T,
                                     const uint32_t *goff, const uint32_t *gb, const uint32_t *gw,
                                     const uint32_t *fr, bool bm, uint32_t *lst, uint32_t *nlst, uint32_t lcap)
{
    uint32_t cw = 0, ci = 0xffffffffu;
    auto byte_at = [&](uint32_t i) -> uint32_t {
        if ((i >> 2) != ci) {
            ci = i >> 2;
            cw = rs_word(32u * ci, ng, T, goff, gb, gw, fr);
        }
        return (cw >> (8u * (3u - (i & 3u)))) & 255u;
    };
    int k = 0;
    for (int64_t i = (int64_t)B - 1; i >= 0; --i) {
        if (byte_at((uint32_t)i)) break;
        ++k;
    }
    for (uint32_t i = B; i < nin; ++i) {
        const uint32_t b = byte_at(i);
        if (ep_insert(b, k)) ep_put(i, bm, lst, nlst, lcap);
        if (b == 0) {
            ++k;
        } else {
            if (i >= Bend) break;
            k = 0;
        }
    }
}

__device__ inline int cand_group(uint32_t i, int ng, const uint32_t *cbase)
{
    int lo = 0, hi = ng;
    while (hi - lo > 1) {
        const int mid = (lo + hi) >> 1;
        if (cbase[mid] <= i) lo = mid;
        else hi = mid;
    }
    return lo;
}

template <int NT, int LCAP>
__device__ __attribute__((always_inline)) inline uint32_t ep_list_windows(uint32_t *lst, uint32_t n, uint32_t nin,
                                                                          uint32_t *eplist, uint32_t *ws, int t,
                                                                          int lane, int wave, uint32_t ecap)
{
    const uint32_t ws0 = (n + 4u * NT - 1u) / (4u * NT) * (4u * NT);
    const uint32_t HW = (uint32_t)LCAP - ws0, CH = HW / (uint32_t)NT;
    uint32_t *win = lst + ws0;
    const uint4 *wv = reinterpret_cast<const uint4 *>(win) + (uint32_t)t * (CH / 4u);
    uint32_t base = 0;
    for (uint32_t w0 = 0; w0 < nin; w0 += 32u * HW) {
        for (uint32_t i = (uint32_t)t; i < HW / 4u; i += (uint32_t)NT)
            reinterpret_cast<uint4 *>(win)[i] = make_uint4(0u, 0u, 0u, 0u);
        __syncthreads();
        for (uint32_t i = (uint32_t)t; i < n; i += (uint32_t)NT) {
            const uint32_t v = lst[i] - w0;
            if (v < 32u * HW) atomicOr(&win[v >> 5], 1u << (v & 31u));
        }
        __syncthreads();
        uint32_t mine = 0;
        for (uint32_t k = 0; k < CH / 4u; ++k) {
            const uint4 q = wv[k];
            mine += (uint32_t)(__builtin_popcount(q.x) + __builtin_popcount(q.y) + __builtin_popcount(q.z) +
                               __builtin_popcount(q.w));
        }
        const uint32_t incl = wave_incl_sum(mine, lane);
        if (lane == 63) ws[wave] = incl;
        __syncthreads();
        uint32_t ex = base, tot = 0;
        for (int q = 0; q < NT / 64; ++q) {
            if (q < wave) ex += ws[q];
            tot += ws[q];
        }
        ex += incl - mine;
        for (uint32_t k = 0; mine && k < CH / 4u; ++k) {
            const uint4 q = wv[k];
            const uint32_t wv4[4] = {q.x, q.y, q.z, q.w};
#pragma unroll
            for (int e = 0; e < 4; ++e)
                for (uint32_t m = wv4[e]; m; m &= m - 1u) {
                    if (ex < ecap)
                        eplist[ex] = w0 + 32u * ((uint32_t)t * CH + 4u * k + (uint32_t)e) + (uint32_t)__builtin_ctz(m);
                    ++ex;
                }
        }
        base += tot;
        __syncthreads();
    }
    return base;
}

template <int NT, int LCAP>
__device__ inline void ep_fix(DevStream *st, DynFrame *DF, size_t nb, int s, const DynGeom &g,
                              const uint32_t *rowstage, const uint32_t *gbits, uint8_t *eps, const EpfLds &E,
                              int t, uint64_t *stp)
{
    static_assert(NT >= 128 && NT % 64 == 0, "ep_fix: one seam wave and at least one candidate wave");
    static_assert(LCAP % (4 * NT) == 0 && LCAP >= 8 * NT, "ep_fix: the bitmap in whole 16-byte chunks per thread");
    auto stamp = [&](int k) {
        if (stp && t == 0) stp[k] = __builtin_amdgcn_s_memrealtime();
    };
    stamp(0);
    uint32_t *goff = E.goff, *gb = E.gb, *gw = E.gw, *cw = E.cw, *cbase = E.cbase, *lst = E.lst;
    uint32_t &nlst = E.cnt[0], &nu = E.cnt[1], &slow = E.cnt[2], &bad = E.cnt[3];
    const uint32_t lcap = LCAP;
    const uint32_t err0 = DF->err;
    if (err0 & (DF_OVER | DF_HANDOFF)) {
        if (t == 0) {
            DF->rbsp_bytes = 0;
            DF->ep = 0;
            DF->err = err0 | DF_FIXED;
            atomicOr((unsigned int *)&st[s].err,
                     (err0 & DF_HANDOFF) ? SCROLL_DEVERR_HANDOFF : SCROLL_DEVERR_DYN);
        }
        return;
    }
    const int ng = g.ngroups;
    constexpr int SR = DYN_STATIC_ROWS;
    const int nA = max(1, (g.y0 + SR - 1) / SR);
    const uint32_t *fr = rowstage + nb * g.rs_frame_words;
    for (uint32_t i = (uint32_t)t; i < lcap / 4u; i += (uint32_t)NT)
        reinterpret_cast<uint4 *>(lst)[i] = make_uint4(0u, 0u, 0u, 0u);
    if (t < 64) {
        if (t == 0) bad = 0u;
        wave_sync();
        rs_table(gbits, nb, g, fr, goff, gb, gw, cw, t, &bad, cbase);
        wave_sync();
        uint32_t carry = 0;
        bool ov = false;
        for (int g0 = 0; g0 < ng; g0 += 64) {
            const int gi = g0 + t;
            const uint32_t c = gi < ng ? cbase[gi] : 0u;
            const uint32_t cmax = (gi >= nA && gi < nA + g.h) ? EPC_ROW - 1u : EPC_STATIC - 1u;
            const uint32_t cc = min(c, cmax);
            const uint32_t incl = wave_incl_sum(cc, t);
            if (gi < ng) cbase[gi] = carry + incl - cc;
            ov |= __builtin_amdgcn_ballot_w64(c > cmax) != 0;
            carry += __shfl(incl, 63, 64);
        }
        if (t == 0) {
            cbase[ng] = carry;
            slow = ov ? 1u : 0u;
            nlst = 0;
        }
    }
    __syncthreads();
    stamp(1);
    if (bad) {
        if (t == 0) {
            DF->err = DF_OVER | DF_FIXED;
            DF->rbsp_bytes = 0;
            DF->ep = 0;
            atomicOr((unsigned int *)&st[s].err, SCROLL_DEVERR_DYN);
        }
        return;
    }
    const uint32_t T = goff[ng];
    const uint32_t nin = (T + 7) >> 3;
    if (((nin + 31u) & ~31u) > g.slot_bytes - DYN_OVF_BYTES) {
        if (t == 0) {
            DF->err = DF_OVER | DF_FIXED;
            DF->rbsp_bytes = 0;
            DF->ep = 0;
            atomicOr((unsigned int *)&st[s].err, SCROLL_DEVERR_DYN);
        }
        return;
    }
    const uint32_t nbw = (nin + 31u) >> 5;
    const bool bm = nbw <= lcap;
    const int wave = t >> 6, lane = t & 63;
    constexpr int NC = NT;
    const uint32_t nc = cbase[ng];
    if (!slow) {
        if (wave == NT / 64 - 1) {
            for (int k = lane; k < ng; k += 64) {
                const uint32_t S = goff[k];
                if (S < T) ep_eval_bytes(S >> 3, (S + 7) >> 3, nin, ng, T, goff, gb, gw, fr, bm, lst, &nlst, lcap);
            }
            if (stp && lane == 0) stp[7] = __builtin_amdgcn_s_memrealtime();
        }
        constexpr int CB = NC >= 192 ? 2 : 4;
        for (uint32_t i0 = 0; i0 < nc; i0 += (uint32_t)(CB * NC)) {
            uint32_t wi[CB], gg[CB];
#pragma unroll
            for (int q = 0; q < CB; ++q) {
                const uint32_t ci = i0 + (uint32_t)(q * NC + t);
                gg[q] = ci < nc ? (uint32_t)cand_group(ci, ng, cbase) : 0u;
                wi[q] = ci < nc ? fr[cw[gg[q]] + 1u + (ci - cbase[gg[q]])] : 0xffffffffu;
            }
            uint32_t pw[CB], w[CB], nx[CB], nwd[CB];
#pragma unroll
            for (int q = 0; q < CB; ++q) {
                const uint32_t *src = fr + gw[gg[q]];
                nwd[q] = (gb[gg[q]] + 31u) >> 5;
                const bool ok = wi[q] < nwd[q];
                pw[q] = ok && wi[q] ? src[wi[q] - 1u] : 0u;
                w[q] = ok ? src[wi[q]] : 0u;
                nx[q] = ok && wi[q] + 1u < nwd[q] ? src[wi[q] + 1u] : 0u;
            }
#pragma unroll
            for (int q = 0; q < CB; ++q) {
                if (wi[q] >= nwd[q]) continue;
                const uint32_t bits = gb[gg[q]], O = goff[gg[q]], x = wi[q];
                const uint32_t *src = fr + gw[gg[q]];
                const uint32_t wd = ep_data(w[q], x, bits);
                const uint32_t nd = x + 1u < nwd[q] ? ep_data(nx[q], x + 1u, bits) : 0xffffffffu;
                uint32_t m = ep_run_starts(pw[q], wd, nd, x, bits);
                while (m) {
                    const uint32_t a = (uint32_t)__builtin_clz(m);
                    m &= ~(0x80000000u >> a);
                    const uint64_t Y = ((uint64_t)wd << 32 | nd) << a;
                    uint32_t e = bits;
                    if (Y) {
                        e = 32u * x + a + (uint32_t)__builtin_clzll(Y);
                    } else {
                        for (uint32_t r = x + 2u; r < nwd[q]; ++r) {
                            const uint32_t v = ep_data(src[r], r, bits);
                            if (v) {
                                e = 32u * r + (uint32_t)__builtin_clz(v);
                                break;
                            }
                        }
                    }
                    const uint32_t A = (O + 32u * x + a + 7u) & ~7u, E2 = O + e;
                    for (uint32_t j = A + 16u; j + 6u <= E2; j += 16u) ep_put(j >> 3, bm, lst, &nlst, lcap);
                }
            }
        }
        stamp(4);
    }
    __syncthreads();
    stamp(2);
    const uint32_t n = nlst;
    uint32_t *eplist = reinterpret_cast<uint32_t *>(eps + nb * eps_stride(g));
    if (slow || (!bm && n > lcap)) {
        static_assert(NT * EPS_KW <= LCAP, "ep_scan's chunk buffer is the position set's LDS");
        __syncthreads();
        const uint32_t ne = ep_scan<NT>(fr, ng, T, goff, gb, gw, lst, reinterpret_cast<int *>(E.ws), nlst, eplist, t, g.ep_cap);
        if (t == 0) {
            DF->err = DF_EPSLOW | DF_FIXED;
            DF->rbsp_bytes = nin;
            DF->ep = ne;
        }
        return;
    }
    constexpr int CW = LCAP / NT;
    if (!bm && n <= lcap - 4u * NT) {
        const uint32_t base = ep_list_windows<NT, LCAP>(lst, n, nin, eplist, E.ws, t, lane, wave, g.ep_cap);
        stamp(3);
        if (t == 0) nu = base;
    } else if (!bm) {
        const uint32_t P = n <= 1u ? 1u : 1u << (32 - __builtin_clz(n - 1u));
        for (uint32_t i = (uint32_t)t + n; i < P; i += (uint32_t)NT) lst[i] = 0xffffffffu;
        __syncthreads();
        for (uint32_t k = 2; k <= P; k <<= 1)
            for (uint32_t j = k >> 1; j > 0; j >>= 1) {
                for (uint32_t i = (uint32_t)t; i < P; i += (uint32_t)NT) {
                    const uint32_t l = i ^ j;
                    if (l > i) {
                        const uint32_t a = lst[i], b = lst[l];
                        if ((a > b) == ((i & k) == 0u)) {
                            lst[i] = b;
                            lst[l] = a;
                        }
                    }
                }
                __syncthreads();
            }
        stamp(3);
        const uint32_t C = (n + (uint32_t)NT - 1u) / (uint32_t)NT, c0 = (uint32_t)t * C, c1 = min(c0 + C, n);
        uint32_t mine = 0;
        for (uint32_t i = c0; i < c1; ++i) mine += (i == 0u || lst[i] != lst[i - 1u]) ? 1u : 0u;
        uint32_t ex = 0;
        const uint32_t incl = wave_incl_sum(mine, lane);
        if (lane == 63) E.ws[wave] = incl;
        __syncthreads();
        for (int q = 0; q < wave; ++q) ex += E.ws[q];
        ex += incl - mine;
        if (t == NT - 1) nu = ex + mine;
        for (uint32_t i = c0; i < c1; ++i)
            if (i == 0u || lst[i] != lst[i - 1u]) {
                if (ex < g.ep_cap) eplist[ex] = lst[i];
                ++ex;
            }
    } else {
        stamp(3);
        uint4 bw[CW / 4];
        uint32_t mine = 0;
#pragma unroll
        for (int k = 0; k < CW / 4; ++k) {
            bw[k] = reinterpret_cast<const uint4 *>(lst)[t * (CW / 4) + k];
            mine += (uint32_t)(__builtin_popcount(bw[k].x) + __builtin_popcount(bw[k].y) +
                               __builtin_popcount(bw[k].z) + __builtin_popcount(bw[k].w));
        }
        uint32_t ex = 0;
        {
            const uint32_t incl = wave_incl_sum(mine, lane);
            if (lane == 63) E.ws[wave] = incl;
            __syncthreads();
            for (int q = 0; q < wave; ++q) ex += E.ws[q];
            ex += incl - mine;
            if (t == NT - 1) nu = ex + mine;
        }
        if (mine) {
#pragma unroll
            for (int k = 0; k < CW / 4; ++k) {
                const uint32_t wv4[4] = {bw[k].x, bw[k].y, bw[k].z, bw[k].w};
#pragma unroll
                for (int e = 0; e < 4; ++e)
                    for (uint32_t m = wv4[e]; m; m &= m - 1u) {
                        if (ex < g.ep_cap)
                            eplist[ex] = 32u * (uint32_t)(t * CW + 4 * k + e) + (uint32_t)__builtin_ctz(m);
                        ++ex;
                    }
            }
        }
    }
    __syncthreads();
    if (t == 0) {
        DF->err = DF_FIXED;
        DF->rbsp_bytes = nin;
        DF->ep = nu;
        if (stp) stp[6] = (uint64_t)nc | (uint64_t)nu << 32;
    }
    stamp(5);
}

constexpr int EPF_LIST = SCROLL_EPF_LIST;
#ifndef SCROLL_EPF_WAVES
#define SCROLL_EPF_WAVES 0
#endif
#if SCROLL_EPF_WAVES
#define EPF_ATTR __attribute__((amdgpu_waves_per_eu(SCROLL_EPF_WAVES)))
#else
#define EPF_ATTR
#endif
template <int NT, int LCAP>
__global__ __launch_bounds__(NT) EPF_ATTR void k_dyn_epfix(DevStream *__restrict__ st, DynFrame *__restrict__ dfr,
                                                     int ld_fr, int nframes, DynGeom g,
                                                     const uint32_t *__restrict__ rowstage,
                                                     const uint32_t *__restrict__ gbits, uint8_t *__restrict__ eps,
                                                     uint64_t *__restrict__ stamps)
{
    __shared__ __attribute__((aligned(16))) uint32_t lst[LCAP];
    extern __shared__ uint32_t gdyn[];
    const GTab GT = gtab_of(gdyn, g.ngroups);
    uint32_t *goff = GT.goff, *gb = GT.gb, *gw = GT.gw, *cw = GT.cw, *cbase = GT.cbase;
    __shared__ uint32_t cnt[4], ws[NT / 64];
    const int f = blockIdx.x, s = blockIdx.y, t = threadIdx.x;
    if (f >= nframes) return;
    const size_t nb = (size_t)s * ld_fr + f;
    DynFrame *DF = dfr + nb;
    if (DF->nal < 0) return;
    const EpfLds E{goff, gb, gw, cw, cbase, lst, cnt, ws};
    ep_fix<NT, LCAP>(st, DF, nb, s, g, rowstage, gbits, eps, E, t, stamps ? stamps + ((size_t)s * nframes + f) * 8 : nullptr);
}
constexpr int EPF_BIG_LIST = 8192;
constexpr int EPF_BIG_MBS = 1024;
inline bool epf_big_rect(int64_t mbs)
{
    static const int env = [] {
        const char *e = getenv("SCROLL_EPF_BIG");
        return e ? atoi(e) : -1;
    }();
    return env >= 0 ? env != 0 : mbs > EPF_BIG_MBS;
}

__device__ inline void store16(uint8_t *A, uint64_t p, const uint8_t *src, uint64_t lo, uint64_t hi)
{
    if (p >= lo && p + 16 <= hi) {
        *reinterpret_cast<uint4 *>(A + p) = *reinterpret_cast<const uint4 *>(src);
        return;
    }
    for (int i = 0; i < 16; ++i)
        if (p + i >= lo && p + i < hi) A[p + i] = src[i];
}

__device__ __attribute__((always_inline)) inline void emit_serial(const NalDesc &d, const DynFrame &df, size_t nb, int s,
                                                      const DynGeom &g, const uint8_t *__restrict__ stage,
                                                      const uint32_t *__restrict__ rowstage,
                                                      const uint32_t *__restrict__ gbits,
                                                      uint8_t *__restrict__ arena, uint64_t ld_arena,
                                                      uint32_t *goff, uint32_t *gb, uint32_t *gw, uint8_t *ob,
                                                      int32_t *wmax, uint32_t *wsum, int t)
{
    uint8_t *A = arena + (size_t)s * ld_arena;
    const uint64_t o0 = d.out_off, o1 = o0 + d.size;
    const bool RS = rowstage != nullptr;
    const uint8_t *in = RS ? nullptr : stage + nb * g.slot_bytes;
    const uint32_t *fr = RS ? rowstage + nb * g.rs_frame_words : nullptr;
    if (RS) rs_table(gbits, nb, g, fr, goff, gb, gw, nullptr, t);
    __syncthreads();
    const int ng = g.ngroups;
    const uint32_t T = RS ? goff[ng] : 0u;
    const uint32_t nin = df.rbsp_bytes;

    uint64_t lb = o0 & ~127ull;
    uint32_t fill = (uint32_t)(o0 - lb);
    if (t < 5) ob[fill + t] = t < 3 ? 0 : (t == 3 ? 1 : nal_header_byte(0));
    fill += 5;
    int carry = -1;
    for (uint32_t i0 = 0; i0 < nin; i0 += DT * 16) {
        const uint32_t ib = i0 + 16u * (uint32_t)t;
        const uint32_t n = ib < nin ? min(16u, nin - ib) : 0u;
        uint8_t b[16];
        {
            uint4 v = make_uint4(0, 0, 0, 0);
            if (n && RS) {
                const uint32_t P = 8u * ib;
                v = make_uint4(__builtin_bswap32(rs_word(P, ng, T, goff, gb, gw, fr)),
                               __builtin_bswap32(rs_word(P + 32u, ng, T, goff, gb, gw, fr)),
                               __builtin_bswap32(rs_word(P + 64u, ng, T, goff, gb, gw, fr)),
                               __builtin_bswap32(rs_word(P + 96u, ng, T, goff, gb, gw, fr)));
            } else if (n) {
                v = *reinterpret_cast<const uint4 *>(in + ib);
            }
            const uint32_t wv[4] = {v.x, v.y, v.z, v.w};
#pragma unroll
            for (int i = 0; i < 16; ++i) b[i] = (uint8_t)(wv[i >> 2] >> (8 * (i & 3)));
        }
        int lnz = -1;
#pragma unroll
        for (int i = 0; i < 16; ++i)
            if ((uint32_t)i < n && b[i]) lnz = (int)(ib + i);
        int ex, tot;
        block_excl_max(lnz, wmax, ex, tot);
        int prev = max(carry, ex);
        uint32_t ins = 0, cnt = 0;
#pragma unroll
        for (int i = 0; i < 16; ++i) {
            if ((uint32_t)i >= n) break;
            if (ep_insert(b[i], (int)(ib + i) - 1 - prev)) {
                ins |= 1u << i;
                cnt++;
            }
            if (b[i]) prev = (int)(ib + i);
        }
        uint32_t opos, otot;
        block_excl_sum(n + cnt, wsum, opos, otot);
        uint32_t p = fill + opos;
        for (int i = 0; i < 16; ++i) {
            if ((uint32_t)i >= n) break;
            if ((ins >> i) & 1u) ob[p++] = 3;
            ob[p++] = b[i];
        }
        __syncthreads();
        const uint32_t nf = fill + otot, nlines = nf >> 7;
        for (uint32_t c = (uint32_t)t; c < nlines * 8; c += DT)
            store16(A, lb + 16u * c, ob + 16u * c, o0, o1);
        const uint32_t rem = nf - (nlines << 7);
        const uint8_t keep = (uint32_t)t < rem ? ob[(nlines << 7) + t] : 0;
        __syncthreads();
        if ((uint32_t)t < rem) ob[t] = keep;
        lb += (uint64_t)nlines << 7;
        fill = rem;
        carry = max(carry, tot);
        __syncthreads();
    }
    for (uint32_t c = (uint32_t)t; 16u * c < fill; c += DT) store16(A, lb + 16u * c, ob + 16u * c, o0, o1);
}
static_assert(OBUF <= 4 * EPLIST_MAX && NW <= EPLIST_MAX, "emit_serial's buffers fit the gathers' LDS lists");

__device__ inline uint32_t pick4(const uint32_t w[8], int i)
{
    const uint32_t a = (i & 1) ? w[1] : w[0], b = (i & 1) ? w[3] : w[2];
    const uint32_t c = (i & 1) ? w[5] : w[4], e = (i & 1) ? w[7] : w[6];
    const uint32_t ab = (i & 2) ? b : a, ce = (i & 2) ? e : c;
    return (i & 4) ? ce : ab;
}

#ifndef SCROLL_GATHER_Z
#define SCROLL_GATHER_Z 1
#endif
constexpr int GATHER_Z = SCROLL_GATHER_Z;

template <int U, bool RS>
__global__ __launch_bounds__(DT) void k_dyn_emit_gather(const DevStream *__restrict__ st,
                                                        const NalDesc *__restrict__ nal, int ld_nal,
                                                        const DynFrame *__restrict__ dfr, int ld_fr,
                                                        DynGeom g, const uint8_t *__restrict__ stage,
                                                        const uint32_t *__restrict__ rowstage,
                                                        const uint32_t *__restrict__ gbits,
                                                        uint8_t *__restrict__ arena, uint64_t ld_arena,
                                                        uint64_t *__restrict__ stamps)
{
    __shared__ alignas(16) uint32_t raw[EPLIST_MAX];
    __shared__ uint32_t sp[EPLIST_MAX];
    extern __shared__ uint32_t gdyn[];
    const GTab GT = gtab_of(gdyn, RS ? g.ngroups : 0);
    uint32_t *goff = GT.goff, *gb = GT.gb, *gw = GT.gw;
    const int s = blockIdx.y, f = dyn_frame_of(blockIdx.x, s), t = threadIdx.x;
    uint64_t *stp = stamps && t == 0 && blockIdx.z == 0 ? stamps + ((size_t)s * gridDim.x + f) * 8 : nullptr;
    if (stp) stp[0] = __builtin_amdgcn_s_memrealtime();
    const DynFrame df = dfr[(size_t)s * ld_fr + f];
    const int j = df.nal;
    if (j < 0 || j >= st[s].nnal || (df.err & ~(DF_EPSLOW | DF_FIXED))) return;
    const uint32_t n = df.ep;
    const NalDesc d = nal[(size_t)s * ld_nal + j];
    if (d.slow != 2) return;
    const size_t nb = (size_t)s * ld_fr + f;
    if (n > min(ep_cap(g, RS), (uint32_t)EPLIST_MAX)) {
        if (blockIdx.z == 0)
            emit_serial(d, df, nb, s, g, stage, rowstage, gbits, arena, ld_arena, goff, gb, gw,
                        reinterpret_cast<uint8_t *>(raw), reinterpret_cast<int32_t *>(sp), sp + NW, t);
        return;
    }
    const uint8_t *in = RS ? nullptr : stage + nb * g.slot_bytes;
    const uint32_t *el = reinterpret_cast<const uint32_t *>(RS ? stage + nb * eps_stride(g)
                                                               : in + g.slot_bytes - DYN_OVF_BYTES);
    const uint32_t *fr = RS ? rowstage + nb * g.rs_frame_words : nullptr;
    if (RS) rs_table(gbits, nb, g, fr, goff, gb, gw, nullptr, t);
    const bool sorted = RS && !(df.err & DF_EPSLOW);
    for (uint32_t i = t; i < n; i += DT) (sorted ? sp : raw)[i] = el[i];
    __syncthreads();
    const int ng = RS ? g.ngroups : 0;
    const uint32_t T = RS ? goff[ng] : 0u;
    const __amdgpu_buffer_rsrc_t rr = buf_rsrc(fr, RS ? 0xfffffffcu : 0u);
    int gcar = 0;
    for (uint32_t i = t; i < (sorted ? 0u : n); i += DT) {
        const uint32_t v = raw[i];
        uint32_t r = 0;
        for (uint32_t k = 0; k < n; ++k) r += raw[k] < v ? 1u : 0u;
        sp[r] = v;
    }
    __syncthreads();
    if (stp) {
        stp[1] = __builtin_amdgcn_s_memrealtime();
        stp[3] = n;
        stp[4] = (uint64_t)(uint32_t)__builtin_amdgcn_s_getreg((31 << 11) | 4);
    }

    uint8_t *A = arena + (size_t)s * ld_arena;
    const uint64_t o0 = d.out_off, o1 = o0 + d.size;
    const uint32_t nin = df.rbsp_bytes;
    const uint8_t hdr[5] = {0, 0, 0, 1, nal_header_byte(0)};
    const uint64_t cfirst = o0 >> 4, cnal = ((o1 + 15) >> 4) - cfirst;
    const uint64_t per = (cnal + gridDim.z - 1) / gridDim.z;
    const uint64_t cbeg = cfirst + per * blockIdx.z, cend = min(cfirst + cnal, cbeg + per);
    int lg = 0;
    while ((1u << lg) <= n) lg++;
    int cs = 10;
    while ((d.size >> cs) >= 1024) cs++;
    const int nblk = (int)(d.size >> cs) + 1;
    for (int bi = t; bi < nblk; bi += DT) {
        const int64_t e0 = (int64_t)bi << cs;
        uint32_t K = 0;
        for (int b = lg - 1; b >= 0; --b) {
            const uint32_t k2 = K + (1u << b);
            K = k2 <= n && (int64_t)(sp[k2 - 1] + (k2 - 1)) < e0 ? k2 : K;
        }
        raw[bi] = K;
    }
    __syncthreads();
    for (uint64_t cb = cbeg + (uint64_t)t; cb < cend; cb += (uint64_t)U * DT) {
        uint32_t Ku[U], epm[U], shv[U];
        bool inner[U];
        uint4 x[U], y[U];
#pragma unroll
        for (int u = 0; u < U; ++u) {
            const uint64_t q0 = (cb + (uint64_t)u * DT) << 4;
            const int64_t u0 = (int64_t)q0 - (int64_t)o0 - 5;
            uint32_t K = u0 > 0 ? raw[min((int)(u0 >> cs), nblk - 1)] : 0u;
            while (K < n && (int64_t)(sp[K] + K) < u0) K++;
            Ku[u] = K;
            inner[u] = u0 >= 0 && q0 + 16 <= o1;
            epm[u] = 0;
            shv[u] = 0;
            x[u] = y[u] = make_uint4(0, 0, 0, 0);
            if (inner[u]) {
                uint32_t em = 0;
                for (uint32_t m = K; m < n; ++m) {
                    const int64_t e = (int64_t)(sp[m] + m) - u0;
                    if (e >= 16) break;
                    em |= 1u << e;
                }
                epm[u] = em;
                const uint32_t i0 = (uint32_t)u0 - K, a0 = i0 & ~15u;
                shv[u] = i0 & 15u;
                if constexpr (RS) {
                    uint32_t w8[8];
                    rs_load8(8u * a0, gcar, ng, T, goff, gb, gw, fr, rr, w8);
                    x[u] = make_uint4(w8[0], w8[1], w8[2], w8[3]);
                    y[u] = make_uint4(w8[4], w8[5], w8[6], w8[7]);
                } else {
                    x[u] = *reinterpret_cast<const uint4 *>(in + a0);
                    if (a0 + 16 < nin) y[u] = *reinterpret_cast<const uint4 *>(in + a0 + 16);
                }
            }
        }
#pragma unroll
        for (int u = 0; u < U; ++u) {
            const uint64_t c = cb + (uint64_t)u * DT;
            if (c >= cend) break;
            const uint64_t q0 = c << 4;
            if (inner[u]) {
                const uint32_t w[8] = {x[u].x, x[u].y, x[u].z, x[u].w, y[u].x, y[u].y, y[u].z, y[u].w};
                const uint32_t sh = shv[u], em = epm[u];
                uint32_t o[4];
                if (em == 0) {
                    const int wi = (int)(sh >> 2), bs = (int)(sh & 3u);
#pragma unroll
                    for (int k = 0; k < 4; ++k) {
                        const uint32_t lo = pick4(w, wi + k), hi = pick4(w, wi + k + 1);
                        o[k] = bs ? __builtin_amdgcn_alignbyte(hi, lo, (uint32_t)bs) : lo;
                    }
                } else {
#pragma unroll
                    for (int k = 0; k < 4; ++k) {
                        const uint32_t b0 = 4u * (uint32_t)k;
                        const uint32_t r0 = sh + b0 - (uint32_t)__builtin_popcount(em & ((1u << b0) - 1u));
                        const uint32_t base = r0 >> 2;
                        const uint32_t lo = pick4(w, (int)base), hi = pick4(w, (int)base + 1);
                        uint32_t sel = 0, three = 0;
#pragma unroll
                        for (int i = 0; i < 4; ++i) {
                            const uint32_t bb = b0 + (uint32_t)i;
                            uint32_t v;
                            if ((em >> bb) & 1u) {
                                v = 0x0cu;
                                three |= 3u << (8 * i);
                            } else {
                                v = sh + bb - (uint32_t)__builtin_popcount(em & ((1u << bb) - 1u)) - 4u * base;
                            }
                            sel |= v << (8 * i);
                        }
                        o[k] = __builtin_amdgcn_perm(hi, lo, sel) | three;
                    }
                }
                *reinterpret_cast<uint4 *>(A + q0) = make_uint4(o[0], o[1], o[2], o[3]);
            } else {
                uint32_t kk = Ku[u];
                uint32_t w8[8] = {0, 0, 0, 0, 0, 0, 0, 0}, a0 = 0;
                if constexpr (RS) {
                    const int64_t ue = (int64_t)q0 - (int64_t)o0 - 5;
                    a0 = (uint32_t)(ue > 0 ? ue : 0) - kk;
                    a0 &= ~15u;
                    if (a0 < nin) rs_load8(8u * a0, gcar, ng, T, goff, gb, gw, fr, rr, w8);
                }
                for (int b = 0; b < 16; ++b) {
                    const uint64_t q = q0 + (uint64_t)b;
                    if (q < o0 || q >= o1) continue;
                    const int64_t uu = (int64_t)q - (int64_t)o0 - 5;
                    uint8_t v;
                    if (uu < 0) {
                        v = hdr[q - o0];
                    } else if (kk < n && (int64_t)(sp[kk] + kk) == uu) {
                        v = 3;
                        kk++;
                    } else if constexpr (RS) {
                        const uint32_t r = (uint32_t)uu - kk - a0;
                        const uint32_t wd = pick4(w8, (int)(r >> 2));
// ... 30 lines not shown
                                                  const DynFrame *__restrict__ dfr, int ld_fr, DynGeom g,
                                                  const uint8_t *__restrict__ eps,
                                                  const uint32_t *__restrict__ rowstage,
                                                  const uint32_t *__restrict__ gbits,
                                                  uint8_t *__restrict__ arena, uint64_t ld_arena,
                                                  uint64_t *__restrict__ stamps)
{
    __shared__ alignas(16) uint32_t raw[EPLIST_MAX];
    __shared__ uint32_t sp[EPLIST_MAX + 1];
    extern __shared__ uint32_t gdyn[];
    const GTab GT = gtab_of(gdyn, g.ngroups);
    uint32_t *goff = GT.goff, *gb = GT.gb, *gw = GT.gw;
    const int s = blockIdx.y, f = dyn_frame_of(blockIdx.x, s), t = threadIdx.x;
    const DynFrame df = dfr[(size_t)s * ld_fr + f];
    const int j = df.nal;
    if (j < 0 || j >= st[s].nnal || (df.err & ~(DF_EPSLOW | DF_FIXED))) return;
    const uint32_t n = df.ep;
    const NalDesc d = nal[(size_t)s * ld_nal + j];
    if (d.slow != 2) return;
    const bool sorted = !(df.err & DF_EPSLOW);
    const uint32_t wcap = (g.debug & SCROLL_DEBUG_DYN_EPWIN) ? 7u : (uint32_t)EPLIST_MAX - 1u;
    if (n > ep_cap(g, true) || (!sorted && n > wcap)) {
        if (blockIdx.z == 0)
            emit_serial(d, df, (size_t)s * ld_fr + f, s, g, nullptr, rowstage, gbits, arena, ld_arena, goff, gb,
                        gw, reinterpret_cast<uint8_t *>(raw), reinterpret_cast<int32_t *>(sp), sp + NW, t);
        return;
    }
    uint64_t *stp = stamps && blockIdx.z == 0 && t == 0 ? stamps + ((size_t)s * gridDim.x + blockIdx.x) * 8 : nullptr;
    if (stp) stp[0] = __builtin_amdgcn_s_memrealtime();
    const size_t nb = (size_t)s * ld_fr + f;
    const uint32_t *el = reinterpret_cast<const uint32_t *>(eps + nb * eps_stride(g));
    const uint32_t *fr = rowstage + nb * g.rs_frame_words;
    rs_table(gbits, nb, g, fr, goff, gb, gw, nullptr, t);
    const int ng = g.ngroups;
    const uint64_t rsb = 4u * (((uint64_t)g.rs_frames - nb) * g.rs_frame_words +
                               (uint64_t)g.rs_spill_cap * g.rs_spill_words);
    const __amdgpu_buffer_rsrc_t rr = buf_rsrc(fr, (uint32_t)min(rsb, (uint64_t)0xfffffffcu));
    uint8_t *A = arena + (size_t)s * ld_arena;
    const uint64_t o0 = d.out_off, o1 = o0 + d.size;
    const uint8_t hdr[5] = {0, 0, 0, 1, nal_header_byte(0)};
    const uint64_t cfirst = o0 >> 4;
    const uint32_t cnal = (uint32_t)(((o1 + 15) >> 4) - cfirst);
    const uint32_t per = ((cnal + gridDim.z - 1) / gridDim.z + GR - 1) / GR * GR;
    const uint32_t cbeg = per * blockIdx.z, cend = min(cnal, cbeg + per);
    const int32_t d0 = (int32_t)(o0 - (cfirst << 4)) + 5;
    const int32_t nebsp = (int32_t)(d.size - 5);
    int gg = 0;
    const bool whole = n <= wcap;
    __shared__ uint32_t win[3];
    __shared__ uint32_t slowq[SLOWQ], nslow;
    uint32_t kb = 0, T = 0;
    int32_t ub = 0;
    int cs = 8, nblk = 1;
    auto slow_byte = [&](uint32_t c, uint32_t b) {
        const uint64_t qa = ((cfirst + c) << 4) + (uint64_t)b;
        if (qa < o0 || qa >= o1) return;
        const int32_t uu = (int32_t)(qa - o0) - 5;
        uint8_t v;
        if (uu < 0) {
            v = hdr[qa - o0];
        } else {
            const int32_t du = uu - ub;
            uint32_t K = raw[du > 0 ? min(du >> cs, nblk - 1) : 0];
            while ((int32_t)(sp[K] + K) < uu) K++;
            if ((int32_t)(sp[K] + K) == uu) {
                v = 3;
            } else {
                const uint32_t ri = (uint32_t)uu - K - kb;
                const uint32_t wd = rs_word(32u * (ri >> 2), ng, T, goff, gb, gw, fr);
                v = (uint8_t)(wd >> (8u * (3u - (ri & 3u))));
            }
        }
        A[qa] = v;
    };
    struct GRun {
        uint32_t c, K, s, rem, yo;
        int32_t u0;
        bool fast, two;
        uint32_t x[GRW + 1];
    };
    uint32_t wend = cend;
    auto prep = [&](uint32_t c, GRun &S) {
        const int32_t u0 = 16 * (int32_t)c - d0, du = u0 - ub;
        uint32_t K = raw[du > 0 ? min(du >> cs, nblk - 1) : 0];
        uint32_t wo = 0u;
        S.c = c;
        S.u0 = u0;
        S.fast = false;
        S.two = false;
        S.s = 32u;
        S.rem = S.yo = 0u;
        if (c + GR <= wend && u0 >= 0 && u0 + 16 * GR <= nebsp) {
            while ((int32_t)(sp[K] + K) < u0) K++;
            const uint32_t i0 = (uint32_t)u0 - K - kb, P = 8u * i0;
            while (gg + 1 < ng && goff[gg + 1] <= P) ++gg;
            const uint32_t lp = P - goff[gg], rem = gb[gg] - lp;
            const uint32_t sh = lp & 31u, adj = sh ? 0u : 1u, wb = gw[gg] + (lp >> 5);
            const uint32_t s = sh + 32u * adj, q = (s + rem) >> 5;
            const bool two = rem < 128u * GR && gg + 1 < ng;
            if (wb >= adj && (!two || (gb[gg + 1] >= 128u * GR - rem && gw[gg + 1] >= q))) {
                S.fast = true;
                S.two = two;
                S.s = s;
                S.rem = rem;
                wo = 4u * (wb - adj);
                S.yo = two ? 4u * (gw[gg + 1] - q) : 0u;
            }
        }
        S.K = K;
#pragma unroll
        for (int k = 0; k < GR; ++k) {
            const auto xa = __builtin_amdgcn_raw_buffer_load_b128(rr, wo + 16u * (uint32_t)k, 0, 0);
            S.x[4 * k] = (uint32_t)xa[0]; S.x[4 * k + 1] = (uint32_t)xa[1];
            S.x[4 * k + 2] = (uint32_t)xa[2]; S.x[4 * k + 3] = (uint32_t)xa[3];
        }
        S.x[GRW] = __builtin_amdgcn_raw_buffer_load_b32(rr, wo + 16u * GR, 0, 0);
    };
    auto assemble = [&](const GRun &S, uint32_t O[GRW]) {
        uint32_t W[GRW + 1];
#pragma unroll
        for (int k = 0; k <= GRW; ++k) W[k] = S.x[k];
        if (S.two) {
            const uint32_t e = S.s + S.rem, q = e >> 5, r = e & 31u;
            const uint32_t hm = ~(0xffffffffu >> r);
            uint32_t Y[GRW + 1];
#pragma unroll
            for (int k = 0; k < GR; ++k) {
                const auto ya = __builtin_amdgcn_raw_buffer_load_b128(rr, S.yo + 16u * (uint32_t)k, 0, 0);
                Y[4 * k] = (uint32_t)ya[0]; Y[4 * k + 1] = (uint32_t)ya[1];
                Y[4 * k + 2] = (uint32_t)ya[2]; Y[4 * k + 3] = (uint32_t)ya[3];
            }
            Y[GRW] = __builtin_amdgcn_raw_buffer_load_b32(rr, S.yo + 16u * GR, 0, 0);
#pragma unroll
            for (int k = 0; k <= GRW; ++k) {
                const uint32_t yp = k > 0 && (uint32_t)k > q ? Y[k > 0 ? k - 1 : 0] : 0u;
                const uint32_t a = __builtin_amdgcn_alignbit(yp, Y[k], r);
                const uint32_t keep = (uint32_t)k < q ? 0xffffffffu : ((uint32_t)k == q ? hm : 0u);
                W[k] = (W[k] & keep) | ((uint32_t)k < q ? 0u : a);
            }
        }
        const uint32_t fs = (32u - S.s) & 31u;
#pragma unroll
        for (int k = 0; k < GRW; ++k) O[k] = __builtin_amdgcn_alignbit(W[k], W[k + 1], fs);
    };
    auto emit = [&](uint32_t c, uint32_t K, int32_t u0, bool fast, uint32_t O[GRW]) {
        if (!fast) {
            const uint32_t i = atomicAdd(&nslow, 1u);
            if (i < (uint32_t)SLOWQ) {
                slowq[i] = c;
            } else {
                for (uint32_t b = 0; b < 16u * GR; ++b)
                    if (c + (b >> 4) < wend) slow_byte(c + (b >> 4), b & 15u);
            }
            return;
        }
        for (uint32_t m = K;; ++m) {
            const int32_t e = (int32_t)(sp[m] + m) - u0;
            if (e >= 16 * GR) break;
#pragma unroll
            for (int k = GRW - 1; k >= 0; --k) {
                const int32_t d = 8 * e - 32 * k;
                const uint32_t sk = __builtin_amdgcn_alignbit(k ? O[k > 0 ? k - 1 : 0] : 0u, O[k], 8u);
                const uint32_t dd = (uint32_t)d & 31u;
                const uint32_t km = ~(0xffffffffu >> dd);
                const uint32_t mix = (O[k] & km) | (sk & ~km & ~(0xff000000u >> dd)) | (3u << (24u - dd));
                O[k] = d >= 32 ? O[k] : (d < 0 ? sk : mix);
            }
        }
#pragma unroll
        for (int k = 0; k < GR; ++k)
            *reinterpret_cast<uint4 *>(A + ((cfirst + c + (uint32_t)k) << 4)) =
                make_uint4(__builtin_bswap32(O[4 * k]), __builtin_bswap32(O[4 * k + 1]),
                           __builtin_bswap32(O[4 * k + 2]), __builtin_bswap32(O[4 * k + 3]));
    };
    for (uint32_t cb = cbeg; cb < cend; cb = wend) {
        uint32_t m = n;
        if (whole) {
            kb = 0;
            wend = cend;
        } else {
            __syncthreads();
            if (t == 0) {
                const int32_t ulo = 16 * (int32_t)cb - d0;
                uint32_t lo = 0, hi = n;
                while (lo < hi) {
                    const uint32_t mid = (lo + hi) >> 1;
                    if ((int32_t)(el[mid] + mid) < ulo) lo = mid + 1;
                    else hi = mid;
                }
                const uint32_t mm = min(n - lo, wcap);
                uint32_t ce = cend;
                if (lo + mm < n) ce = min(cend, max(cb + 1u, (uint32_t)((int32_t)(el[lo + mm] + lo + mm) + d0) >> 4));
                win[0] = lo;
                win[1] = mm;
                win[2] = ce;
            }
            __syncthreads();
            kb = win[0];
            m = win[1];
            wend = win[2];
        }
        for (uint32_t i = t; i < m; i += DT) (sorted ? sp : raw)[i] = el[kb + i] + kb;
        if (t == 0) {
            sp[m] = 0x3fffffffu;
            nslow = 0u;
        }
        __syncthreads();
        for (uint32_t i = t; i < (sorted ? 0u : m); i += DT) {
            const uint32_t v = raw[i];
            uint32_t r = 0;
            for (uint32_t k = 0; k < m; ++k) r += raw[k] < v ? 1u : 0u;
            sp[r] = v;
        }
        __syncthreads();
        T = goff[ng];
        ub = whole ? 0 : max(0, 16 * (int32_t)cb - d0);
        const uint32_t span = whole ? d.size : (uint32_t)(16 * (int32_t)wend - d0 - ub + 16);
        int lg = 0;
        while ((1u << lg) <= m) lg++;
        cs = 8;
        while ((span >> cs) >= (uint32_t)EPLIST_MAX) cs++;
        nblk = (int)(span >> cs) + 1;
        for (int bi = t; bi < nblk; bi += DT) {
            const uint32_t e0 = (uint32_t)ub + ((uint32_t)bi << cs);
            uint32_t K = 0;
            for (int b = lg - 1; b >= 0; --b) {
                const uint32_t k2 = K + (1u << b);
                K = k2 <= m && sp[k2 - 1] + (k2 - 1) < e0 ? k2 : K;
            }
            raw[bi] = K;
        }
        __syncthreads();
        if (stp && cb == cbeg) stp[1] = __builtin_amdgcn_s_memrealtime();
        GRun S;
        uint32_t c = cb + (uint32_t)(GR * t);
        if (c < wend) prep(c, S);
        while (c < wend) {
            uint32_t O[GRW];
            const uint32_t K = S.K;
            const int32_t u0 = S.u0;
            const bool fast = S.fast;
            assemble(S, O);
            prep(c + GR * DT, S);
            emit(c, K, u0, fast, O);
            c += GR * DT;
        }
        __syncthreads();
        const uint32_t nq = min(nslow, (uint32_t)SLOWQ);
        for (uint32_t i = (uint32_t)t; i < nq * 16u * GR; i += DT) {
            const uint32_t cq = slowq[i / (16u * GR)] + ((i / 16u) & (uint32_t)(GR - 1));
            if (cq < wend) slow_byte(cq, i & 15u);
        }
    }
    if (stamps) {
        __syncthreads();
        if (stp) stp[2] = __builtin_amdgcn_s_memrealtime();
    }
}

__device__ inline uint32_t mix32(uint32_t x)
{
    x ^= x >> 16;
    x *= 0x7feb352du;
    x ^= x >> 15;
    x *= 0x846ca68bu;
    x ^= x >> 16;
    return x;
}

__global__ __launch_bounds__(256) void k_dyn_synth(uint8_t *__restrict__ src, DynGeom g,
                                                   int stream_base, int t0)
{
    const uint32_t i = blockIdx.x * 256u + threadIdx.x;
    const int f = blockIdx.y, s = blockIdx.z;
    const uint32_t npx = 384u * (uint32_t)g.w * (uint32_t)g.h;
    if (i >= npx) return;
    const uint32_t tt = (uint32_t)(t0 + f);
    const uint32_t seed = (0x9E3779B9u * (uint32_t)(stream_base + s)) ^ (0x85EBCA6Bu * tt);
    const uint32_t hv = mix32(seed + i * 0x9E3779B9u);
    const uint32_t ly = 256u * (uint32_t)g.w * (uint32_t)g.h;
    int v;
    if (i < ly) {
        const int lw = 16 * g.w;
        const int y = (int)(i / (uint32_t)lw), x = (int)(i - (uint32_t)(y * lw));
        const int X = 16 * g.x0 + x, Y = 16 * g.y0 + y;
        v = 128 + ((X + 2 * Y + 3 * (int)tt) & 63) - 32 + (int)(hv >> 28) - 8;
    } else {
        const uint32_t r = (i - ly) % (64u * (uint32_t)g.w * (uint32_t)g.h);
        const int cw = 8 * g.w;
        const int y = (int)(r / (uint32_t)cw), x = (int)(r - (uint32_t)(y * cw));
        const int X = 8 * g.x0 + x, Y = 8 * g.y0 + y;
        v = 128 + ((X + Y + (int)tt) & 15) - 8 + (int)(hv >> 30);
    }
    src[(size_t)s * g.src_ld + (size_t)f * g.src_fr + i] = (uint8_t)clampi(v, 0, 255);
}

}

int dyn_launch_rows(hipStream_t hs, int nframes, int S, const DevStream *st, const NalDesc *nal, int ld_nal,
                    const PlanPending *pend, DynFrame *dfr, int ld_fr, const DynGeom *g, uint32_t *rows,
                    uint32_t *ctr, uint4 *heads, const uint8_t *qpf)
{
    if (nframes <= 0 || S <= 0) return 0;
    hipLaunchKernelGGL(k_dyn_rows, dim3(nframes, S), dim3(256), 0, hs, st, nal, ld_nal, pend, dfr, ld_fr,
                       *g, rows, ctr, heads, qpf);
    return hipGetLastError() != hipSuccess ? -1 : 0;
}

int dyn_launch_code(hipStream_t hs, int nframes, int S, DevStream *st, const NalDesc *nal,
                    int ld_nal, const PlanPending *pend, DynFrame *dfr, int ld_fr,
                    const DynGeom *g, const uint8_t *src, const uint8_t *refs, const DynScratch *x,
                    uint32_t epoch, int mbw, uint64_t *stamps, const DynFork *fk, hipEvent_t ev0, hipEvent_t ev1)
{
    if (nframes <= 0 || S <= 0) return 0;
    {
        static std::mutex mu;
        static uint64_t ready = 0;
        int dev = 0;
        if (hipGetDevice(&dev) != hipSuccess || dev >= 64) return -1;
        std::lock_guard<std::mutex> lk(mu);
        if (!(ready >> dev & 1u)) {
            hipLaunchKernelGGL(k_tzrb_init, dim3((TZRB_N + 255) / 256), dim3(256), 0, hs);
            if (hipGetLastError() != hipSuccess || hipStreamSynchronize(hs) != hipSuccess) return -1;
            ready |= 1ull << dev;
        }
    }
    if (dyn_launch_rows(hs, nframes, S, st, nal, ld_nal, pend, dfr, ld_fr, g, x->rows, x->ctr, x->heads, x->qpf))
        return -1;
    hipStream_t hg = hs;
    if (fk) {
        if (hipEventRecord(fk->e0, hs) != hipSuccess || hipStreamWaitEvent(fk->side, fk->e0, 0) != hipSuccess)
            return -1;
        hg = fk->side;
    }
    const int nchunk = (24 * g->w * g->h + CODE_T - 1) / CODE_T;
    hipLaunchKernelGGL(k_dyn_code_general, dim3(nchunk, CODE_GEN_Y), dim3(CODE_T), 0, hg, st, dfr, ld_fr,
                       pend, nal, ld_nal, *g, x->rows, src, refs, x->meta, x->body_lo, x->body_hi, x->body_w,
                       x->ctr);
    if (hipGetLastError() != hipSuccess) return -1;
    const bool dbg = stamps || (g->debug & SCROLL_DEBUG_DYN_NOPUBLISH);
    void (*const krow)(RowArgs) = dbg ? &k_dyn_row<false, true> : &k_dyn_row<false, false>;
    void (*const kgen)(RowArgs) = dbg ? &k_dyn_row<true, true> : &k_dyn_row<true, false>;
    if (row_lds_bytes(g->w) > 65536) {
        const int rl = (int)row_lds_bytes(g->w);
        if (hipFuncSetAttribute(reinterpret_cast<const void *>(krow), hipFuncAttributeMaxDynamicSharedMemorySize,
                                rl) != hipSuccess ||
            hipFuncSetAttribute(reinterpret_cast<const void *>(kgen), hipFuncAttributeMaxDynamicSharedMemorySize,
                                rl) != hipSuccess)
            return -1;
    }
    RowArgs ra{};
    ra.st = st;
    ra.nal = nal;
    ra.pend = pend;
    ra.dfr = dfr;
    ra.rows = x->rows;
    ra.src = src;
    ra.refs = refs;
    ra.heads = x->heads;
    ra.ld_nal = ld_nal;
    ra.ld_fr = ld_fr;
    ra.g = *g;
    ra.tcx = x->tcx;
    ra.epoch = epoch;
    ra.rowstage = x->rowstage;
    ra.gbits = x->gbits;
    ra.spill = x->spill;
    ra.ctr = x->ctr;
    ra.meta = x->meta;
    ra.blo = x->body_lo;
    ra.bhi = x->body_hi;
    ra.bwd = x->body_w;
    ra.stamps = stamps;
    if (ev0 && hipEventRecord(ev0, hs) != hipSuccess) return -1;
    hipLaunchKernelGGL(krow, dim3(g->h, nframes, S), dim3(row_threads(g->w)), row_lds_bytes(g->w), hs, ra);
    if (hipGetLastError() != hipSuccess) return -1;
    if (ev1 && hipEventRecord(ev1, hs) != hipSuccess) return -1;
    hipLaunchKernelGGL(kgen, dim3(g->h, std::min<uint32_t>(g->gen_cap, (uint32_t)(nframes * S)), 1),
                       dim3(row_threads(g->w)), row_lds_bytes(g->w), hg, ra);
    if (hipGetLastError() != hipSuccess) return -1;
    if (fk) {
        if (dyn_launch_static(hg, nframes, S, st, nal, ld_nal, pend, dfr, ld_fr, g, x) ||
            hipEventRecord(fk->e1, hg) != hipSuccess)
            return -1;
    }
    return 0;
}

int dyn_launch_static(hipStream_t hs, int nframes, int S, DevStream *st, const NalDesc *nal, int ld_nal,
                      const PlanPending *pend, DynFrame *dfr, int ld_fr, const DynGeom *g, const DynScratch *x)
{
    if (nframes <= 0 || S <= 0) return 0;
    hipLaunchKernelGGL(k_dyn_static, dim3(g->ngroups - g->h, nframes, S), dim3(GW), 0, hs, st, nal, ld_nal,
                       pend, dfr, ld_fr, *g, x->rowstage, x->gbits);
    return hipGetLastError() == hipSuccess ? 0 : -1;
}

int dyn_launch_pack(hipStream_t hs, int nframes, int S, DevStream *st, const NalDesc *nal,
                    int ld_nal, const PlanPending *pend, DynFrame *dfr, int ld_fr,
                    const DynGeom *g, const DynScratch *x, uint8_t *eps, uint64_t *stamps, const DynFork *fk)
{
    if (nframes <= 0 || S <= 0) return 0;
    if (fk) {
        if (hipStreamWaitEvent(hs, fk->e1, 0) != hipSuccess) return -1;
    } else if (dyn_launch_static(hs, nframes, S, st, nal, ld_nal, pend, dfr, ld_fr, g, x)) {
        return -1;
    }
    if (g->ep_cap >= (uint32_t)EPF_BIG_LIST)
        hipLaunchKernelGGL((k_dyn_epfix<EPF_T, EPF_BIG_LIST>), dim3(nframes, S), dim3(EPF_T), gtab_bytes(g->ngroups, true),
                           hs, st, dfr, ld_fr, nframes, *g, x->rowstage, x->gbits, eps, stamps);
    else
        hipLaunchKernelGGL((k_dyn_epfix<EPF_T, EPF_LIST>), dim3(nframes, S), dim3(EPF_T), gtab_bytes(g->ngroups, true),
                           hs, st, dfr, ld_fr, nframes, *g, x->rowstage, x->gbits, eps, stamps);
    return hipGetLastError() == hipSuccess ? 0 : -1;
}

int dyn_launch_emit(hipStream_t hs, int nframes, int S, const DevStream *st, const NalDesc *nal,
                    int ld_nal, const DynFrame *dfr, int ld_fr, const DynGeom *g,
                    const uint8_t *stage, const DynScratch *x, uint8_t *arena, uint64_t ld_arena,
                    uint64_t *stamps)
{
    if (nframes <= 0 || S <= 0) return 0;
    const bool big = (int64_t)g->w * g->h > 1024;
    const uint32_t *rs = x ? x->rowstage : nullptr, *gbits = x ? x->gbits : nullptr;
    const dim3 grid(nframes, S, GATHER_Z);
    const size_t gl = x ? gtab_bytes(g->ngroups, false) : 0;
    if (x && !(g->debug & SCROLL_DEBUG_DYN_GATHER1))
        hipLaunchKernelGGL(k_dyn_gather, dim3(nframes, S, gather_z(*g, (int64_t)nframes * S)), dim3(DT), gl, hs, st, nal, ld_nal, dfr,
                           ld_fr, *g, stage, rs, gbits, arena, ld_arena, stamps);
    else if (x && big)
        hipLaunchKernelGGL((k_dyn_emit_gather<4, true>), grid, dim3(DT), gl, hs, st, nal, ld_nal, dfr, ld_fr, *g,
                           stage, rs, gbits, arena, ld_arena, stamps);
    else if (x)
        hipLaunchKernelGGL((k_dyn_emit_gather<1, true>), grid, dim3(DT), gl, hs, st, nal, ld_nal, dfr, ld_fr, *g,
                           stage, rs, gbits, arena, ld_arena, stamps);
    else if (big)
        hipLaunchKernelGGL((k_dyn_emit_gather<4, false>), grid, dim3(DT), 0, hs, st, nal, ld_nal, dfr, ld_fr,
                           *g, stage, rs, gbits, arena, ld_arena, stamps);
    else
        hipLaunchKernelGGL((k_dyn_emit_gather<1, false>), grid, dim3(DT), 0, hs, st, nal, ld_nal, dfr, ld_fr,
                           *g, stage, rs, gbits, arena, ld_arena, stamps);
    return hipGetLastError() == hipSuccess ? 0 : -1;
}

int dyn_launch_synth(hipStream_t hs, int nframes, int S, uint8_t *src, const DynGeom *g,
                     int stream_base, int t0)
{
    if (nframes <= 0 || S <= 0) return 0;
    const uint32_t npx = 384u * (uint32_t)g->w * (uint32_t)g->h;
    hipLaunchKernelGGL(k_dyn_synth, dim3((npx + 255) / 256, nframes, S), dim3(256), 0, hs, src, *g,
                       stream_base, t0);
    return hipGetLastError() == hipSuccess ? 0 : -1;
}

void dyn_rowstage_geom(DynGeom *g, int mbw, int mbh)
{
    const int SR = DYN_STATIC_ROWS;
    const int above = g->y0 < SR ? g->y0 : SR, below0 = mbh - g->y0 - g->h;
    const int below = below0 < SR ? below0 : SR;
    const int maxrows = above > below ? above : below;
    auto words = [](uint64_t bits) { return (uint32_t)((((bits + 31) / 32) + 63) & ~(uint64_t)63); };
    g->rs_static_words = words((uint64_t)HDR_MAX + (uint64_t)maxrows * mbw * (HEAD_MAX + 1) + 64) + EPC_STATIC;
    g->rs_spill_words = words((uint64_t)mbw * (HEAD_MAX + 1) + (uint64_t)g->w * MB_BITS_MAX + 64) + EPC_ROW;
    g->rs_row_words = words((uint64_t)mbw * (HEAD_MAX + 1) + (uint64_t)g->w * SCROLL_DYN_ROW_KBITS + 64) + EPC_ROW;
    if (g->rs_row_words > g->rs_spill_words) g->rs_row_words = g->rs_spill_words;
    g->rs_frame_words = (uint64_t)(g->ngroups - g->h) * g->rs_static_words + (uint64_t)g->h * g->rs_row_words;
}

uint32_t dyn_ep_cap(int rw, int rh, int debug)
{
    return (debug & SCROLL_DEBUG_DYN_EPWIN) || epf_big_rect((int64_t)rw * rh) ? (uint32_t)EPF_BIG_LIST
                                                                            : (uint32_t)EPLIST_MAX;
}

size_t dyn_slot_bound(int mbw, int mbh, int rw, int rh)
{
    const size_t bits = (size_t)HDR_MAX + (size_t)mbw * mbh * (HEAD_MAX + 1) +
                        (size_t)rw * rh * MB_BITS_MAX + 64;
    return ((bits / 8 + 32 + DYN_OVF_BYTES) + 255) & ~(size_t)255;
}

extern "C" int scroll_debug_row_occupancy(int w, int mbw, int extra_lds)
{
    int n = -1;
    (void)mbw;
    const size_t lds = (size_t)((long)row_lds_bytes(w) + extra_lds);
    if (hipOccupancyMaxActiveBlocksPerMultiprocessor(&n, reinterpret_cast<const void *>(&k_dyn_row<false, false>),
                                                     row_threads(w), lds) != hipSuccess)
        return -1;
    return n;
}
```

Baseline: 3.134 million frames/s.

## Fuse static-group bit packing into row-planning kernel and prune seam walks

Moves the static-row bitstream packing that k_dyn_static did into a templated k_dyn_rows front kernel. One block per frame now handles all static groups, with a larger LDS word buffer and a precomputed slice header. The optional side-stream fork path is removed, and the pack step only launches the emulation-prevention fix kernel. The epfix kernel gains a seam rule that skips walking group boundaries whose leading and trailing zero runs cannot form a start-code pattern. This cuts a kernel launch and redundant per-group setup, but puts more serial work and LDS in each front block and adds a hard limit on the static group count.

```diff
diff --git a/h264-scroll-encoder_amd/csrc/batch.h b/h264-scroll-encoder_amd/csrc/batch.h
--- a/h264-scroll-encoder_amd/csrc/batch.h
+++ b/h264-scroll-encoder_amd/csrc/batch.h
@@ -112,7 +112,6 @@
     std::vector<SpliceHost> h_sp;
     std::vector<int32_t> h_dyn_pos;
     int fallback = 0;
-    DynFork fork{};
     std::vector<int32_t> h_dyn_qp;
     int dyn_pos_custom = 0;
     int dyn_qp = 26;
diff --git a/h264-scroll-encoder_amd/csrc/batch_core.hip b/h264-scroll-encoder_amd/csrc/batch_core.hip
--- a/h264-scroll-encoder_amd/csrc/batch_core.hip
+++ b/h264-scroll-encoder_amd/csrc/batch_core.hip
@@ -309,21 +309,8 @@
         } else {
             b->dx.epoch = b->dx.epoch % 0xffffffu + 1u;
             const DynGeom &G = b->geo;
-            const DynFork *fk = nullptr;
-            static const bool fork_on = [] {
-                const char *e = getenv("SCROLL_DYN_FORK");
-                return e && e[0] == '1';
-            }();
-            if (fork_on) {
-                if (!b->fork.side) {
-                    HIPCHK(hipStreamCreateWithFlags(&b->fork.side, hipStreamNonBlocking));
-                    HIPCHK(hipEventCreateWithFlags(&b->fork.e0, hipEventDisableTiming));
-                    HIPCHK(hipEventCreateWithFlags(&b->fork.e1, hipEventDisableTiming));
-                }
-                fk = &b->fork;
-            }
             if (dyn_launch_code(hs, nframes, S, b->d_st, b->d_nal, b->ld_nal, b->d_pend, b->d_dfr, ld_fr, &G,
-                                b->d_src, b->d_refs, &b->dx, b->dx.epoch, b->dyn_pw / 16, stamps, fk,
+                                b->d_src, b->d_refs, &b->dx, b->dx.epoch, b->dyn_pw / 16, stamps,
                                 lite_row ? rev[1] : nullptr, lite_row ? rev[6] : nullptr)) {
                 set_err("k_dyn_code launch: %s", hipGetErrorString(hipGetLastError()));
                 return SCROLL_ERR_HIP;
@@ -341,9 +328,9 @@
                 b->rc_timed = timed ? 1 : 0;
                 b->rc_last_hint = 0;
             }
-            if (dyn_launch_pack(hs, nframes, S, b->d_st, b->d_nal, b->ld_nal, b->d_pend, b->d_dfr, ld_fr, &G,
-                                &b->dx, b->d_stage, stamps ? b->d_dbg : nullptr, fk)) {
-                set_err("k_dyn_static / k_dyn_epfix launch: %s", hipGetErrorString(hipGetLastError()));
+            if (dyn_launch_pack(hs, nframes, S, b->d_st, b->d_dfr, ld_fr, &G, &b->dx, b->d_stage,
+                                stamps ? b->d_dbg : nullptr)) {
+                set_err("k_dyn_epfix launch: %s", hipGetErrorString(hipGetLastError()));
                 return SCROLL_ERR_HIP;
             }
         }
@@ -477,12 +464,6 @@
     for (int i = 0; i < NEV; ++i)
         if (b->ev[i]) (void)hipEventDestroy(b->ev[i]);
     for (hipEvent_t e : b->ring) (void)hipEventDestroy(e);
-    if (b->fork.side) {
-        (void)hipStreamSynchronize(b->fork.side);
-        (void)hipStreamDestroy(b->fork.side);
-        (void)hipEventDestroy(b->fork.e0);
-        (void)hipEventDestroy(b->fork.e1);
-    }
     if (b->own) (void)hipStreamDestroy(b->own);
     (void)hipFree(b->d_st);
     (void)hipHostFree(b->h_st);
diff --git a/h264-scroll-encoder_amd/csrc/dyn_engine.h b/h264-scroll-encoder_amd/csrc/dyn_engine.h
--- a/h264-scroll-encoder_amd/csrc/dyn_engine.h
+++ b/h264-scroll-encoder_amd/csrc/dyn_engine.h
@@ -22,23 +22,16 @@
 #define DYN_HEAD_VECS 16
 #define DYN_CTR_LIST 4
 
-typedef struct {
-    hipStream_t side;
-    hipEvent_t e0, e1;
-} DynFork;
 int dyn_launch_rows(hipStream_t hs, int nframes, int S, const DevStream *st, const NalDesc *nal, int ld_nal,
                     const PlanPending *pend, DynFrame *dfr, int ld_fr, const DynGeom *g, uint32_t *rows,
                     uint32_t *ctr, uint4 *heads, const uint8_t *qpf);
 int dyn_launch_code(hipStream_t hs, int nframes, int S, DevStream *st, const NalDesc *nal,
                     int ld_nal, const PlanPending *pend, DynFrame *dfr, int ld_fr,
                     const DynGeom *g, const uint8_t *src, const uint8_t *refs, const DynScratch *x,
-                    uint32_t epoch, int mbw, uint64_t *stamps, const DynFork *fk, hipEvent_t ev0 = nullptr,
+                    uint32_t epoch, int mbw, uint64_t *stamps, hipEvent_t ev0 = nullptr,
                     hipEvent_t ev1 = nullptr);
-int dyn_launch_static(hipStream_t hs, int nframes, int S, DevStream *st, const NalDesc *nal, int ld_nal,
-                      const PlanPending *pend, DynFrame *dfr, int ld_fr, const DynGeom *g, const DynScratch *x);
-int dyn_launch_pack(hipStream_t hs, int nframes, int S, DevStream *st, const NalDesc *nal,
-                    int ld_nal, const PlanPending *pend, DynFrame *dfr, int ld_fr,
-                    const DynGeom *g, const DynScratch *x, uint8_t *eps, uint64_t *stamps, const DynFork *fk);
+int dyn_launch_pack(hipStream_t hs, int nframes, int S, DevStream *st, DynFrame *dfr, int ld_fr,
+                    const DynGeom *g, const DynScratch *x, uint8_t *eps, uint64_t *stamps);
 int dyn_launch_emit(hipStream_t hs, int nframes, int S, const DevStream *st, const NalDesc *nal,
                     int ld_nal, const DynFrame *dfr, int ld_fr, const DynGeom *g,
                     const uint8_t *stage, const DynScratch *x, uint8_t *arena, uint64_t ld_arena,
diff --git a/h264-scroll-encoder_amd/csrc/dyn_kernels.hip b/h264-scroll-encoder_amd/csrc/dyn_kernels.hip
--- a/h264-scroll-encoder_amd/csrc/dyn_kernels.hip
+++ b/h264-scroll-encoder_amd/csrc/dyn_kernels.hip
@@ -6,6 +6,7 @@
 #include "dyn_device.h"
 #include "dyn_engine.h"
 #include "nal_ctx.h"
+#include "seam_rule.h"
 #include "stage_util.h"
 
 using namespace scroll;
@@ -644,167 +645,105 @@
     return make_uint4((uint32_t)(H >> 32), (uint32_t)H, (uint32_t)(Lw >> 32), (uint32_t)Lw);
 }
 
-__global__ __launch_bounds__(256) void k_dyn_rows(const DevStream *__restrict__ st,
-                                                  const NalDesc *__restrict__ nal, int ld_nal,
-                                                  const PlanPending *__restrict__ pend,
-                                                  DynFrame *__restrict__ dfr, int ld_fr, DynGeom g,
-                                                  uint32_t *__restrict__ rows, uint32_t *__restrict__ ctr,
-                                                  uint4 *__restrict__ heads, const uint8_t *__restrict__ qpf)
-{
-    __shared__ int32_t wo[8], wl[8], wv[8];
-    __shared__ int32_t gen;
-    const int s = blockIdx.y, f = blockIdx.x, t = threadIdx.x;
-    DynFrame *DF = dfr + (size_t)s * ld_fr + f;
-    const int j = DF->nal;
-    if (j < 0) return;
-    if (t < 8) {
-        wo[t] = pend[s].wo[t];
-        wl[t] = pend[s].wl[t];
-        wv[t] = pend[s].wv[t];
-    }
-    if (t == 0) gen = 0;
-    __syncthreads();
-    const DevStream *S = st + s;
-    const NalDesc d = nal[(size_t)s * ld_nal + j];
-    const NalCtx c = nal_ctx(S, d, wo, wl, wv);
-    if (t < 12) {
-        const HeadCtx H = head_ctx(c);
-        CapSink hc{0, 0, 0};
-        H.put_class(hc, t);
-        uint4 *hv = heads + ((size_t)s * ld_fr + f) * DYN_HEAD_VECS;
-        hv[t] = body_msb(hc.hi, hc.lo, min(hc.n, 128u));
-        reinterpret_cast<uint32_t *>(hv + 12)[t] = hc.n | (hc.over() ? 0x80000000u : 0u);
-    }
-    const Regions rg = regions(c);
-    const int w = c.w, h = c.h, a_end = (h - c.off) / 16;
-    const uint32_t ysz = (uint32_t)w * (uint32_t)h, pic = ysz + ysz / 2;
-    const WpTab T{wo, wv, h};
-    uint32_t *rw = rows + ((size_t)s * ld_fr + f) * (size_t)(32 * g.h);
-    bool my_gen = false;
-    for (int i = t; i < 32 * g.h; i += 256) {
-        uint32_t e;
-        if (i < 16 * g.h) {
-            const int Y = 16 * g.y0 + i, row = Y >> 4;
-            const bool cA = row < a_end;
-            int yo;
-            const int b = luma_row(T, cA ? rg.ra : rg.rb, Y + (cA ? rg.mva : rg.mvb), yo);
-            e = (uint32_t)b * pic + (uint32_t)yo * (uint32_t)w;
-        } else {
-            const int i2 = i - 16 * g.h, bot = i2 >= 8 * g.h;
-            const int Y = 8 * g.y0 + (bot ? i2 - 8 * g.h : i2), row = Y >> 3;
-            const bool cA = row < a_end;
-            const int q = 4 * (cA ? rg.mva : rg.mvb), o = q >> 3, fr = q & 7;
-            int yo;
-            const int b = chroma_row(T, cA ? rg.ra : rg.rb, Y + o + bot, yo);
-            if (b < 0) {
-                e = ROW_GEN;
-                if (!bot || fr) my_gen = true;
-            } else {
-                e = ((uint32_t)b * pic + ysz + (uint32_t)yo * (uint32_t)(w / 2)) | (uint32_t)fr << 28;
-            }
-        }
-        rw[i] = e;
-    }
-    const uint32_t qe = qpf ? qpf[(size_t)s * ld_fr + f] : 0xFFu;
-    const int qpy = qe <= 51u ? (int)qe : S->dyn_qp;
-    if (my_gen || qpy < QP_MIN) gen = 1;
-    __syncthreads();
-    if (t == 0) {
-        uint32_t e = 0u;
-        if (gen) {
-            const uint32_t k = atomicAdd(&ctr[1], 1u);
-            if (k < g.gen_cap) {
-                DF->rbsp_bytes = k;
-                ctr[DYN_CTR_LIST + k] = (uint32_t)((size_t)s * ld_fr + f);
-                e = DF_GENERAL;
-            } else {
-                e = DF_OVER;
-            }
-        }
-        DF->err = e;
-        DF->ep = (uint32_t)qpy;
-    }
-}
-
-constexpr int GW = 64;
+constexpr int FRONT_T = 256;
 #ifndef SCROLL_GBUF_WORDS
-#define SCROLL_GBUF_WORDS 256
+#define SCROLL_GBUF_WORDS 1024
 #endif
 constexpr int GBUF_WORDS = SCROLL_GBUF_WORDS;
+constexpr int SGROUPS_MAX = (DYN_MAX_MBH - 1 + 2 * (DYN_STATIC_ROWS - 1)) / DYN_STATIC_ROWS;
+constexpr int SROWS1 = DYN_STATIC_ROWS + 1;
 
 struct StaticFixed {
-    uint32_t ncand;
-    uint32_t buf[GBUF_WORDS];
+    uint4 pat[12];
     uint64_t hhi[12], hlo[12];
-    uint4 pat[12];
     uint32_t hlen[12];
     int32_t head_over;
-    int32_t wo[8], wl[8], wv[8];
-    uint32_t moff[DYN_STATIC_ROWS + 1];
+    uint32_t buf[GBUF_WORDS];
+    uint32_t hbuf[HDR_MAX / 32];
+    uint32_t F;
+    uint32_t ncand[SGROUPS_MAX];
+    uint32_t gbit[SGROUPS_MAX];
+    uint32_t gw0[SGROUPS_MAX + 1];
+    uint32_t moff[SGROUPS_MAX * SROWS1];
 };
 
-__global__ __launch_bounds__(GW) void k_dyn_static(const DevStream *__restrict__ st,
-                                                   const NalDesc *__restrict__ nal, int ld_nal,
-                                                   const PlanPending *__restrict__ pend,
-                                                   const DynFrame *__restrict__ dfr, int ld_fr, DynGeom g,
-                                                   uint32_t *__restrict__ rowstage, uint32_t *__restrict__ gbits)
-{
-    __shared__ StaticFixed L;
+struct StaticGeo {
+    int nA, y0, h, mbh;
+    __device__ inline int gi(int k) const { return k < nA ? k : k + h; }
+    __device__ inline int ra(int k) const
+    {
+        return k < nA ? k * DYN_STATIC_ROWS : y0 + h + (k - nA) * DYN_STATIC_ROWS;
+    }
+    __device__ inline int rb(int k) const { return min(ra(k) + DYN_STATIC_ROWS, k < nA ? y0 : mbh); }
+};
+
+__device__ inline int sgroup_of(uint32_t q, int ngs, const uint32_t *gw0)
+{
+    int lo = 0, hi = ngs;
+    while (hi - lo > 1) {
+        const int mid = (lo + hi) >> 1;
+        if (gw0[mid] <= q) lo = mid;
+        else hi = mid;
+    }
+    return lo;
+}
+
+__device__ inline void static_class(StaticFixed &L, int t, const CapSink &hc)
+{
+    L.hhi[t] = hc.hi;
+    L.hlo[t] = hc.lo;
+    L.hlen[t] = hc.n;
+    if (hc.n < 128u && !hc.over()) {
+        const uint64_t hi = (hc.hi << 1) | (hc.lo >> 63), lo = (hc.lo << 1) | 1u;
+        L.pat[t] = body_msb(hi, lo, hc.n + 1u);
+    } else {
+        L.head_over = 1;
+    }
+}
+
+__device__ inline void static_header(StaticFixed &L, const NalCtx &c)
+{
+    static_assert(HDR_MAX % 32 == 0, "the header buffer in whole words");
+    for (int i = 0; i < HDR_MAX / 32; ++i) L.hbuf[i] = 0u;
+    WSink hs{LdsOrWin{L.hbuf, 0u, (uint32_t)(HDR_MAX / 32)}, 0, 0, 0};
+    hs.start(0);
+    emit_slice_header(hs, c);
+    L.F = 32u * hs.wi + (uint32_t)hs.fill;
+    hs.finish();
+}
+
+__device__ inline void static_row_bits(StaticFixed &L, const HeadCtx &H, const DynGeom &g, int mbh, int t)
+{
     constexpr int SR = DYN_STATIC_ROWS;
     const Rect R{g.x0, g.y0, g.w, g.h};
-    const int nA = max(1, (R.y0 + SR - 1) / SR);
-    const int gi = (int)blockIdx.x >= nA ? (int)blockIdx.x + R.h : (int)blockIdx.x;
-    const int ng = g.ngroups, f = blockIdx.y, s = blockIdx.z, t = threadIdx.x;
-    const size_t nb = (size_t)s * ld_fr + f;
-    const DynFrame df = dfr[nb];
-    const int j = df.nal;
-    if (j < 0) return;
-    const bool first = gi == 0, last = gi == ng - 1;
-    if (t < 8) {
-        L.wo[t] = pend[s].wo[t];
-        L.wl[t] = pend[s].wl[t];
-        L.wv[t] = pend[s].wv[t];
-    }
-    if (t == 0) {
-        L.head_over = 0;
-        L.ncand = 0;
-    }
-    const DevStream *S = st + s;
-    const NalDesc d = nal[(size_t)s * ld_nal + j];
-    wave_sync();
-    NalCtx c = nal_ctx(S, d, L.wo, L.wl, L.wv);
-    c.qpd = (int)df.ep - QP_DEFAULT;
-    const HeadCtx H = head_ctx(c);
-    const int mbw = H.mbw, mbh = c.h / 16;
-    int ra, rb;
-    if (gi < nA) {
-        ra = gi * SR;
-        rb = min(ra + SR, R.y0);
-    } else {
-        ra = R.y0 + R.h + (gi - nA - R.h) * SR;
-        rb = min(ra + SR, mbh);
-    }
-    uint32_t F = 0;
-    if (first) {
-        CountSink hc{0};
-        emit_slice_header(hc, c);
-        F = hc.n;
-    }
-    if (t < 12) {
-        CapSink hc{0, 0, 0};
-        H.put_class(hc, t);
-        L.hhi[t] = hc.hi;
-        L.hlo[t] = hc.lo;
-        L.hlen[t] = hc.n;
-        if (hc.over()) L.head_over = 1;
-        if (hc.n < 128u) {
-            const uint64_t hi = (hc.hi << 1) | (hc.lo >> 63), lo = (hc.lo << 1) | 1u;
-            L.pat[t] = body_msb(hi, lo, hc.n + 1u);
-        } else {
-            L.head_over = 1;
-        }
-    }
-    wave_sync();
+    const int mbw = H.mbw, ngs = g.ngroups - R.h;
+    const StaticGeo G{max(1, (R.y0 + SR - 1) / SR), R.y0, R.h, mbh};
+    const bool head_over = L.head_over;
+    for (int i = t; i < ngs * SR; i += 64) {
+        const int k = i / SR, e = i - k * SR, r = G.ra(k) + e;
+        uint32_t len = 0;
+        if (r < G.rb(k)) {
+            if (!head_over) {
+                len = row_static_bits(H, L.hlen, r, R);
+            } else {
+                for (int col = 0; col < mbw; ++col) {
+                    CountSink cn{0};
+                    H.put_slow(cn, r, col);
+                    len += cn.n + 1u;
+                }
+            }
+        }
+        L.moff[k * SROWS1 + e + 1] = len;
+    }
+}
+
+__device__ inline void static_groups(StaticFixed &L, const NalCtx &c, const HeadCtx &H, const DynGeom &g, size_t nb,
+                                     uint32_t *__restrict__ rowstage, uint32_t *__restrict__ gbits, int t)
+{
+    constexpr int SR = DYN_STATIC_ROWS;
+    const Rect R{g.x0, g.y0, g.w, g.h};
+    const int mbw = H.mbw, ng = g.ngroups, ngs = ng - R.h;
+    const StaticGeo G{max(1, (R.y0 + SR - 1) / SR), R.y0, R.h, c.h / 16};
     const bool head_over = L.head_over;
     auto head_bits = [&](int r, int col) -> uint32_t {
         if (!head_over) return L.hlen[H.sel(r, col)];
@@ -812,59 +751,60 @@
         H.put_slow(cn, r, col);
         return cn.n;
     };
-    uint32_t len = 0;
-    const int r = ra + t;
-    if (r < rb) {
-        if (!head_over) {
-            len = row_static_bits(H, L.hlen, r, R);
-        } else {
-            for (int col = 0; col < mbw; ++col) len += head_bits(r, col) + 1u;
-        }
-    }
-    const uint32_t incl = wave_incl_sum(len, t);
-    if (r < rb) L.moff[r - ra] = F + incl - len;
-    const uint32_t rows_end = F + __shfl(incl, GW - 1, GW);
-    if (t == 0) L.moff[rb - ra] = rows_end;
-    const uint32_t bits = rows_end + (last ? 1u : 0u);
-    if (t == 0) gbits[nb * (size_t)ng + gi] = bits;
-    wave_sync();
-
-    uint32_t *out = rowstage + nb * g.rs_frame_words + rs_group_words(g, nA, gi);
-    const uint32_t nw = min((bits + 31u) >> 5, g.rs_static_words - EPC_STATIC);
-    const int ne = rb - ra;
-    auto cnt_le = [&](uint32_t x) -> int {
-        int lo = 0, hi = ne + 1;
-        while (lo < hi) {
-            const int mid = (lo + hi) >> 1;
-            if (L.moff[mid] <= x) lo = mid + 1;
-            else hi = mid;
-        }
-        return lo;
-    };
-    const uint32_t m_mbw = magic32((uint32_t)mbw);
-    for (uint32_t p0 = 0; p0 < nw; p0 += GBUF_WORDS) {
-        const uint32_t n = min((uint32_t)GBUF_WORDS, nw - p0);
-        for (uint32_t i = (uint32_t)t; i < n; i += GW) L.buf[i] = 0u;
-        wave_sync();
-        const LdsOrWin win{L.buf, p0, n};
-        if (head_over && first && t == 0 && p0 * 32u < F) {
-            WSink hs{win, 0, 0, 0};
-            hs.start(0);
-            emit_slice_header(hs, c);
-            hs.finish();
-        }
-        if (!head_over) {
-            const uint32_t rbeg = L.moff[0], rend = L.moff[ne];
-            for (uint32_t i = (uint32_t)t; i < n; i += GW) {
-                const uint32_t W0 = 32u * (p0 + i), W1 = W0 + 32u;
+    const uint32_t wcap = g.rs_static_words - EPC_STATIC;
+    if (t < 64) {
+        uint32_t nwk = 0;
+        if (t < ngs) {
+            uint32_t o = t == 0 ? L.F : 0u;
+            uint32_t *mo = L.moff + t * SROWS1;
+            const int ne = G.rb(t) - G.ra(t);
+            mo[0] = o;
+            for (int e = 1; e <= ne; ++e) {
+                o += mo[e];
+                mo[e] = o;
+            }
+            const uint32_t bits = o + (t == ngs - 1 ? 1u : 0u);
+            L.gbit[t] = bits;
+            L.ncand[t] = 0;
+            gbits[nb * (size_t)ng + G.gi(t)] = bits;
+            nwk = min((bits + 31u) >> 5, wcap);
+        }
+        const uint32_t incl = wave_incl_sum(nwk, t);
+        if (t < ngs) L.gw0[t] = incl - nwk;
+        if (t == ngs - 1) L.gw0[ngs] = incl;
+    }
+    __syncthreads();
+    uint32_t *fr = rowstage + nb * g.rs_frame_words;
+    const uint32_t F = L.moff[0];
+    const uint32_t sbit = L.gbit[ngs - 1] - 1u;
+    const bool stop_in = (sbit >> 5) < L.gw0[ngs] - L.gw0[ngs - 1];
+    if (!head_over) {
+        const uint32_t total = L.gw0[ngs];
+        for (uint32_t q0 = 0; q0 < total; q0 += GBUF_WORDS) {
+            const uint32_t n = min((uint32_t)GBUF_WORDS, total - q0);
+            for (uint32_t i = (uint32_t)t; i < n; i += FRONT_T) {
+                const int k = sgroup_of(q0 + i, ngs, L.gw0);
+                const uint32_t *mo = L.moff + k * SROWS1;
+                const int ra = G.ra(k), ne = G.rb(k) - ra;
+                auto cnt_le = [&](uint32_t x) -> int {
+                    int lo = 0, hi = ne + 1;
+                    while (lo < hi) {
+                        const int mid = (lo + hi) >> 1;
+                        if (mo[mid] <= x) lo = mid + 1;
+                        else hi = mid;
+                    }
+                    return lo;
+                };
+                const uint32_t rbeg = mo[0], rend = mo[ne];
+                const uint32_t W0 = 32u * (q0 + i - L.gw0[k]), W1 = W0 + 32u;
                 uint32_t acc = 0, b = max(W0, rbeg), R0 = 0, R1 = 0, L0 = 0, Lm = 1;
                 int b3 = 0;
                 float inv = 1.0f;
                 while (b < W1 && b < rend) {
                     if (b >= R1 || b < R0) {
                         const int e = cnt_le(b) - 1;
-                        R0 = L.moff[e];
-                        R1 = L.moff[e + 1];
+                        R0 = mo[e];
+                        R1 = mo[e + 1];
                         b3 = H.sel(ra + e, 0);
                         L0 = L.hlen[b3] + 1u;
                         Lm = L.hlen[b3 + 1] + 1u;
@@ -885,71 +825,186 @@
                             off = o2 - (uint32_t)(mbw - 2) * Lm;
                         }
                     }
-                    const uint32_t k = min(L.hlen[cl] + 1u - off, W1 - b);
+                    const uint32_t kb = min(L.hlen[cl] + 1u - off, W1 - b);
                     const uint4 P = L.pat[cl];
                     const uint32_t wi = off >> 5, sh = off & 31u;
                     const uint32_t w0 = wi == 0 ? P.x : (wi == 1 ? P.y : (wi == 2 ? P.z : P.w));
                     const uint32_t w1 = wi == 0 ? P.y : (wi == 1 ? P.z : (wi == 2 ? P.w : 0u));
                     uint32_t v = sh ? __builtin_amdgcn_alignbit(w0, w1, 32u - sh) : w0;
-                    v &= k >= 32u ? 0xffffffffu : ~(0xffffffffu >> k);
+                    v &= kb >= 32u ? 0xffffffffu : ~(0xffffffffu >> kb);
                     acc |= v >> (b - W0);
-                    b += k;
+                    b += kb;
                 }
+                if (k == 0 && W0 < F) acc |= L.hbuf[W0 >> 5];
+                if (k == ngs - 1 && stop_in && W0 == (sbit & ~31u)) acc |= 0x80000000u >> (sbit & 31u);
                 L.buf[i] = acc;
             }
+            __syncthreads();
+            for (uint32_t i = (uint32_t)t; i < n; i += FRONT_T) {
+                const int k = sgroup_of(q0 + i, ngs, L.gw0);
+                const uint32_t p = q0 + i - L.gw0[k], nwk = L.gw0[k + 1] - L.gw0[k];
+                const uint32_t w = L.buf[i];
+                const uint32_t nx = p + 1u < nwk ? (i + 1u < n ? L.buf[i + 1u] : 0u) : 0xffffffffu;
+                fr[rs_group_words(g, G.nA, G.gi(k)) + p] = w;
+                if (ep_quick(w, nx)) {
+                    const uint32_t j = atomicAdd(&L.ncand[k], 1u);
+                    if (j < (uint32_t)EPC_STATIC - 1u) fr[rs_runs_words(g, G.nA, G.gi(k)) + 1u + j] = p;
+                }
+            }
+            __syncthreads();
+        }
+    } else {
+        const uint32_t m_mbw = magic32((uint32_t)mbw);
+        for (int k = 0; k < ngs; ++k) {
+            const uint32_t *mo = L.moff + k * SROWS1;
+            const int ra = G.ra(k), ne = G.rb(k) - ra;
+            const uint32_t nw = L.gw0[k + 1] - L.gw0[k];
+            uint32_t *out = fr + rs_group_words(g, G.nA, G.gi(k));
+            auto cnt_le = [&](uint32_t x) -> int {
+                int lo = 0, hi = ne + 1;
+                while (lo < hi) {
+                    const int mid = (lo + hi) >> 1;
+                    if (mo[mid] <= x) lo = mid + 1;
+                    else hi = mid;
+                }
+                return lo;
+            };
+            for (uint32_t p0 = 0; p0 < nw; p0 += GBUF_WORDS) {
+                const uint32_t n = min((uint32_t)GBUF_WORDS, nw - p0);
+                for (uint32_t i = (uint32_t)t; i < n; i += FRONT_T) L.buf[i] = 0u;
+                __syncthreads();
+                const LdsOrWin win{L.buf, p0, n};
+                if (k == 0 && p0 == 0u && t < HDR_MAX / 32 && (uint32_t)t < n) atomicOr(&L.buf[t], L.hbuf[t]);
+                const int ea = max(cnt_le(32u * p0) - 1, 0), eb = min(cnt_le(32u * (p0 + n) - 1u), ne);
+                const int nm = eb * mbw;
+                for (int m = ea * mbw + t; m < nm; m += FRONT_T) {
+                    const int rr = (int)div_m((uint32_t)m, m_mbw), col = m - rr * mbw, rw = ra + rr;
+                    uint32_t off = mo[rr];
+                    WSink sk{win, 0, 0, 0};
+                    for (int c2 = 0; c2 < col; ++c2) off += head_bits(rw, c2) + 1u;
+                    sk.start(off);
+                    H.put_slow(sk, rw, col);
+                    sk.put(1, 1);
+                    sk.finish();
+                }
+                if (k == ngs - 1 && t == 64 && stop_in) {
+                    WSink sk{win, 0, 0, 0};
+                    sk.start(sbit);
+                    sk.put(1, 1);
+                    sk.finish();
+                }
+                __syncthreads();
+                flush_window(L.buf, n, p0, p0 + n >= nw, out, &L.ncand[k],
+                             fr + rs_runs_words(g, G.nA, G.gi(k)), EPC_STATIC - 1, t, FRONT_T);
+                __syncthreads();
+            }
+        }
+    }
+    if (t < ngs) fr[rs_runs_words(g, G.nA, G.gi(t))] = L.ncand[t];
+}
+
+template <bool STATIC>
+__global__ __launch_bounds__(FRONT_T) void k_dyn_rows(const DevStream *__restrict__ st,
+                                                      const NalDesc *__restrict__ nal, int ld_nal,
+                                                      const PlanPending *__restrict__ pend,
+                                                      DynFrame *__restrict__ dfr, int ld_fr, DynGeom g,
+                                                      uint32_t *__restrict__ rows, uint32_t *__restrict__ ctr,
+                                                      uint4 *__restrict__ heads, const uint8_t *__restrict__ qpf,
+                                                      uint32_t *__restrict__ rowstage, uint32_t *__restrict__ gbits)
+{
+    __shared__ int32_t wo[8], wl[8], wv[8];
+    __shared__ int32_t gen;
+    __shared__ typename std::conditional<STATIC, StaticFixed, int>::type L;
+    const int s = blockIdx.y, f = blockIdx.x, t = threadIdx.x;
+    DynFrame *DF = dfr + (size_t)s * ld_fr + f;
+    const int j = DF->nal;
+    if (j < 0) return;
+    if (t < 8) {
+        wo[t] = pend[s].wo[t];
+        wl[t] = pend[s].wl[t];
+        wv[t] = pend[s].wv[t];
+    }
+    if (t == 0) {
+        gen = 0;
+        if constexpr (STATIC) L.head_over = 0;
+    }
+    __syncthreads();
+    const DevStream *S = st + s;
+    const NalDesc d = nal[(size_t)s * ld_nal + j];
+    const NalCtx c = nal_ctx(S, d, wo, wl, wv);
+    const HeadCtx H = head_ctx(c);
+    if (t < 12) {
+        CapSink hc{0, 0, 0};
+        H.put_class(hc, t);
+        uint4 *hv = heads + ((size_t)s * ld_fr + f) * DYN_HEAD_VECS;
+        hv[t] = body_msb(hc.hi, hc.lo, min(hc.n, 128u));
+        reinterpret_cast<uint32_t *>(hv + 12)[t] = hc.n | (hc.over() ? 0x80000000u : 0u);
+        if constexpr (STATIC) static_class(L, t, hc);
+    }
+    const uint32_t qe = qpf ? qpf[(size_t)s * ld_fr + f] : 0xFFu;
+    const int qpy = qe <= 51u ? (int)qe : S->dyn_qp;
+    if constexpr (STATIC) {
+        if (t < 64) {
             wave_sync();
-            if (first && t == 0 && p0 * 32u < F) {
-                WSink hs{win, 0, 0, 0};
-                hs.start(0);
-                emit_slice_header(hs, c);
-                hs.finish();
-            }
-            if (last && t == 0) {
-                WSink sk{win, 0, 0, 0};
-                sk.start(bits - 1u);
-                sk.put(1, 1);
-                sk.finish();
-            }
-            wave_sync();
-            flush_window(L.buf, n, p0, p0 + n >= nw, out, &L.ncand,
-                         rowstage + nb * g.rs_frame_words + rs_runs_words(g, nA, gi), EPC_STATIC - 1, t, GW);
-            wave_sync();
-            continue;
-        }
-        const int ea = max(cnt_le(32u * p0) - 1, 0), eb = min(cnt_le(32u * (p0 + n) - 1u), ne);
-        const int nm = eb * mbw;
-        for (int m = ea * mbw + t; m < nm; m += GW) {
-            const int rr = (int)div_m((uint32_t)m, m_mbw), col = m - rr * mbw, rw = ra + rr;
-            uint32_t off = L.moff[rr];
-            WSink sk{win, 0, 0, 0};
-            if (!head_over) {
-                const int b3 = H.sel(rw, 0);
-                off += col == 0 ? 0u : L.hlen[b3] + 1u + (uint32_t)(col - 1) * (L.hlen[b3 + 1] + 1u);
-                if (off >= 32u * (p0 + n)) continue;
-                const int cls = b3 + (col == 0 ? 0 : (col == mbw - 1 ? 2 : 1));
-                if (off + L.hlen[cls] + 1u <= 32u * p0) continue;
-                sk.start(off);
-                sk.put_cap(CapSink{L.hhi[cls], L.hlo[cls], L.hlen[cls]});
+            static_row_bits(L, H, g, c.h / 16, t);
+        } else if (t == 64) {
+            NalCtx cq = c;
+            cq.qpd = qpy - QP_DEFAULT;
+            static_header(L, cq);
+        }
+    }
+    const bool rows_mine = !STATIC || t < 64 || t >= 128;
+    const int rt = STATIC && t >= 128 ? t - 64 : t, rn = STATIC ? FRONT_T - 64 : FRONT_T;
+    const Regions rg = regions(c);
+    const int w = c.w, h = c.h, a_end = (h - c.off) / 16;
+    const uint32_t ysz = (uint32_t)w * (uint32_t)h, pic = ysz + ysz / 2;
+    const WpTab T{wo, wv, h};
+    uint32_t *rw = rows + ((size_t)s * ld_fr + f) * (size_t)(32 * g.h);
+    bool my_gen = false;
+    for (int i = rt; rows_mine && i < 32 * g.h; i += rn) {
+        uint32_t e;
+        if (i < 16 * g.h) {
+            const int Y = 16 * g.y0 + i, row = Y >> 4;
+            const bool cA = row < a_end;
+            int yo;
+            const int b = luma_row(T, cA ? rg.ra : rg.rb, Y + (cA ? rg.mva : rg.mvb), yo);
+            e = (uint32_t)b * pic + (uint32_t)yo * (uint32_t)w;
+        } else {
+            const int i2 = i - 16 * g.h, bot = i2 >= 8 * g.h;
+            const int Y = 8 * g.y0 + (bot ? i2 - 8 * g.h : i2), row = Y >> 3;
+            const bool cA = row < a_end;
+            const int q = 4 * (cA ? rg.mva : rg.mvb), o = q >> 3, fr = q & 7;
+            int yo;
+            const int b = chroma_row(T, cA ? rg.ra : rg.rb, Y + o + bot, yo);
+            if (b < 0) {
+                e = ROW_GEN;
+                if (!bot || fr) my_gen = true;
             } else {
-                for (int c2 = 0; c2 < col; ++c2) off += head_bits(rw, c2) + 1u;
-                sk.start(off);
-                H.put_slow(sk, rw, col);
-            }
-            sk.put(1, 1);
-            sk.finish();
-        }
-        if (last && t == 0) {
-            WSink sk{win, 0, 0, 0};
-            sk.start(bits - 1u);
-            sk.put(1, 1);
-            sk.finish();
-        }
-        wave_sync();
-        flush_window(L.buf, n, p0, p0 + n >= nw, out, &L.ncand,
-                     rowstage + nb * g.rs_frame_words + rs_runs_words(g, nA, gi), EPC_STATIC - 1, t, GW);
-        wave_sync();
-    }
-    if (t == 0) rowstage[nb * g.rs_frame_words + rs_runs_words(g, nA, gi)] = L.ncand;
+                e = ((uint32_t)b * pic + ysz + (uint32_t)yo * (uint32_t)(w / 2)) | (uint32_t)fr << 28;
+            }
+        }
+        rw[i] = e;
+    }
+    if (my_gen || qpy < QP_MIN) gen = 1;
+    __syncthreads();
+    if (t == 0) {
+        uint32_t e = 0u;
+        if (gen) {
+            const uint32_t k = atomicAdd(&ctr[1], 1u);
+            if (k < g.gen_cap) {
+                DF->rbsp_bytes = k;
+                ctr[DYN_CTR_LIST + k] = (uint32_t)((size_t)s * ld_fr + f);
+                e = DF_GENERAL;
+            } else {
+                e = DF_OVER;
+            }
+        }
+        DF->err = e;
+        DF->ep = (uint32_t)qpy;
+    }
+    if constexpr (STATIC) {
+        static_groups(L, c, H, g, (size_t)s * ld_fr + f, rowstage, gbits, t);
+    }
 }
 
 
@@ -2263,10 +2318,29 @@
     const uint32_t nc = cbase[ng];
     if (!slow) {
         if (wave == NT / 64 - 1) {
-            for (int k = lane; k < ng; k += 64) {
-                const uint32_t S = goff[k];
-                if (S < T) ep_eval_bytes(S >> 3, (S + 7) >> 3, nin, ng, T, goff, gb, gw, fr, bm, lst, &nlst, lcap);
-            }
+            uint32_t walked = 0, carry_b = 0, carry_s = 0;
+            for (int k0 = 0; k0 < ng; k0 += 64) {
+                const int k = k0 + lane;
+                const bool in = k < ng;
+                const uint32_t bk = in ? gb[k] : 0u, nwk = (bk + 31u) >> 5;
+                const uint32_t *src = fr + (in ? gw[k] : 0u);
+                const uint32_t first = nwk ? src[0] : 0u, last = nwk ? src[nwk - 1u] : 0u;
+                const uint32_t sk = seam::seam_word_of(bk, first, last, 0u, false);
+                uint32_t bl = (uint32_t)__shfl_up((int)bk, 1, 64), sl = (uint32_t)__shfl_up((int)sk, 1, 64);
+                if (lane == 0) {
+                    bl = carry_b;
+                    sl = carry_s;
+                }
+                const bool wk = in && goff[k] < T && seam::seam_walk(k, bl, sl, bk, sk);
+                if (wk) {
+                    const uint32_t S = goff[k];
+                    ep_eval_bytes(S >> 3, (S + 7) >> 3, nin, ng, T, goff, gb, gw, fr, bm, lst, &nlst, lcap);
+                }
+                walked += (uint32_t)__builtin_popcountll(__builtin_amdgcn_ballot_w64(wk));
+                carry_b = (uint32_t)__shfl((int)bk, 63, 64);
+                carry_s = (uint32_t)__shfl((int)sk, 63, 64);
+            }
+            if (lane == 0) E.cnt[4] = walked;
             if (stp && lane == 0) stp[7] = __builtin_amdgcn_s_memrealtime();
         }
         constexpr int CB = NC >= 192 ? 2 : 4;
@@ -2411,7 +2485,7 @@
         DF->err = DF_FIXED;
         DF->rbsp_bytes = nin;
         DF->ep = nu;
-        if (stp) stp[6] = (uint64_t)nc | (uint64_t)nu << 32;
+        if (stp) stp[6] = (uint64_t)nc | (uint64_t)min(nu, 0xffffu) << 32 | (uint64_t)min(E.cnt[4], 0xffffu) << 48;
     }
     stamp(5);
 }
@@ -2436,7 +2510,7 @@
     extern __shared__ uint32_t gdyn[];
     const GTab GT = gtab_of(gdyn, g.ngroups);
     uint32_t *goff = GT.goff, *gb = GT.gb, *gw = GT.gw, *cw = GT.cw, *cbase = GT.cbase;
-    __shared__ uint32_t cnt[4], ws[NT / 64];
+    __shared__ uint32_t cnt[5], ws[NT / 64];
     const int f = blockIdx.x, s = blockIdx.y, t = threadIdx.x;
     if (f >= nframes) return;
     const size_t nb = (size_t)s * ld_fr + f;
@@ -3073,17 +3147,18 @@
                     uint32_t *ctr, uint4 *heads, const uint8_t *qpf)
 {
     if (nframes <= 0 || S <= 0) return 0;
-    hipLaunchKernelGGL(k_dyn_rows, dim3(nframes, S), dim3(256), 0, hs, st, nal, ld_nal, pend, dfr, ld_fr,
-                       *g, rows, ctr, heads, qpf);
+    hipLaunchKernelGGL(k_dyn_rows<false>, dim3(nframes, S), dim3(FRONT_T), 0, hs, st, nal, ld_nal, pend, dfr,
+                       ld_fr, *g, rows, ctr, heads, qpf, (uint32_t *)nullptr, (uint32_t *)nullptr);
     return hipGetLastError() != hipSuccess ? -1 : 0;
 }
 
 int dyn_launch_code(hipStream_t hs, int nframes, int S, DevStream *st, const NalDesc *nal,
                     int ld_nal, const PlanPending *pend, DynFrame *dfr, int ld_fr,
                     const DynGeom *g, const uint8_t *src, const uint8_t *refs, const DynScratch *x,
-                    uint32_t epoch, int mbw, uint64_t *stamps, const DynFork *fk, hipEvent_t ev0, hipEvent_t ev1)
+                    uint32_t epoch, int mbw, uint64_t *stamps, hipEvent_t ev0, hipEvent_t ev1)
 {
     if (nframes <= 0 || S <= 0) return 0;
+    if (g->ngroups - g->h > SGROUPS_MAX) return -1;
     {
         static std::mutex mu;
         static uint64_t ready = 0;
@@ -3096,16 +3171,11 @@
             ready |= 1ull << dev;
         }
     }
-    if (dyn_launch_rows(hs, nframes, S, st, nal, ld_nal, pend, dfr, ld_fr, g, x->rows, x->ctr, x->heads, x->qpf))
-        return -1;
-    hipStream_t hg = hs;
-    if (fk) {
-        if (hipEventRecord(fk->e0, hs) != hipSuccess || hipStreamWaitEvent(fk->side, fk->e0, 0) != hipSuccess)
-            return -1;
-        hg = fk->side;
-    }
+    hipLaunchKernelGGL(k_dyn_rows<true>, dim3(nframes, S), dim3(FRONT_T), 0, hs, st, nal, ld_nal, pend, dfr, ld_fr,
+                       *g, x->rows, x->ctr, x->heads, x->qpf, x->rowstage, x->gbits);
+    if (hipGetLastError() != hipSuccess) return -1;
     const int nchunk = (24 * g->w * g->h + CODE_T - 1) / CODE_T;
-    hipLaunchKernelGGL(k_dyn_code_general, dim3(nchunk, CODE_GEN_Y), dim3(CODE_T), 0, hg, st, dfr, ld_fr,
+    hipLaunchKernelGGL(k_dyn_code_general, dim3(nchunk, CODE_GEN_Y), dim3(CODE_T), 0, hs, st, dfr, ld_fr,
                        pend, nal, ld_nal, *g, x->rows, src, refs, x->meta, x->body_lo, x->body_hi, x->body_w,
                        x->ctr);
     if (hipGetLastError() != hipSuccess) return -1;
@@ -3148,35 +3218,14 @@
     if (hipGetLastError() != hipSuccess) return -1;
     if (ev1 && hipEventRecord(ev1, hs) != hipSuccess) return -1;
     hipLaunchKernelGGL(kgen, dim3(g->h, std::min<uint32_t>(g->gen_cap, (uint32_t)(nframes * S)), 1),
-                       dim3(row_threads(g->w)), row_lds_bytes(g->w), hg, ra);
-    if (hipGetLastError() != hipSuccess) return -1;
-    if (fk) {
-        if (dyn_launch_static(hg, nframes, S, st, nal, ld_nal, pend, dfr, ld_fr, g, x) ||
-            hipEventRecord(fk->e1, hg) != hipSuccess)
-            return -1;
-    }
-    return 0;
-}
-
-int dyn_launch_static(hipStream_t hs, int nframes, int S, DevStream *st, const NalDesc *nal, int ld_nal,
-                      const PlanPending *pend, DynFrame *dfr, int ld_fr, const DynGeom *g, const DynScratch *x)
+                       dim3(row_threads(g->w)), row_lds_bytes(g->w), hs, ra);
+    return hipGetLastError() != hipSuccess ? -1 : 0;
+}
+
+int dyn_launch_pack(hipStream_t hs, int nframes, int S, DevStream *st, DynFrame *dfr, int ld_fr,
+                    const DynGeom *g, const DynScratch *x, uint8_t *eps, uint64_t *stamps)
 {
     if (nframes <= 0 || S <= 0) return 0;
-    hipLaunchKernelGGL(k_dyn_static, dim3(g->ngroups - g->h, nframes, S), dim3(GW), 0, hs, st, nal, ld_nal,
-                       pend, dfr, ld_fr, *g, x->rowstage, x->gbits);
-    return hipGetLastError() == hipSuccess ? 0 : -1;
-}
-
-int dyn_launch_pack(hipStream_t hs, int nframes, int S, DevStream *st, const NalDesc *nal,
-                    int ld_nal, const PlanPending *pend, DynFrame *dfr, int ld_fr,
-                    const DynGeom *g, const DynScratch *x, uint8_t *eps, uint64_t *stamps, const DynFork *fk)
-{
-    if (nframes <= 0 || S <= 0) return 0;
-    if (fk) {
-        if (hipStreamWaitEvent(hs, fk->e1, 0) != hipSuccess) return -1;
-    } else if (dyn_launch_static(hs, nframes, S, st, nal, ld_nal, pend, dfr, ld_fr, g, x)) {
-        return -1;
-    }
     if (g->ep_cap >= (uint32_t)EPF_BIG_LIST)
         hipLaunchKernelGGL((k_dyn_epfix<EPF_T, EPF_BIG_LIST>), dim3(nframes, S), dim3(EPF_T), gtab_bytes(g->ngroups, true),
                            hs, st, dfr, ld_fr, nframes, *g, x->rowstage, x->gbits, eps, stamps);
@@ -3251,6 +3300,8 @@
     return ((bits / 8 + 32 + DYN_OVF_BYTES) + 255) & ~(size_t)255;
 }
 
+extern "C" int scroll_debug_dyn_static_rows(void) { return DYN_STATIC_ROWS; }
+
 extern "C" int scroll_debug_row_occupancy(int w, int mbw, int extra_lds)
 {
     int n = -1;
diff --git a/h264-scroll-encoder_amd/csrc/seam_rule.h b/h264-scroll-encoder_amd/csrc/seam_rule.h
--- /dev/null
+++ b/h264-scroll-encoder_amd/csrc/seam_rule.h
@@ -0,0 +1,55 @@
+#ifndef SCROLL_SEAM_RULE_H
+#define SCROLL_SEAM_RULE_H
+
+#include <stdint.h>
+
+#if !defined(__HIPCC__) && !defined(__device__)
+#define __device__
+#define __host__
+#endif
+
+namespace scroll {
+namespace seam {
+
+constexpr uint32_t SEAM_CAP = 12u;
+constexpr uint32_t EP_RUN_BITS = 22u;
+
+__host__ __device__ inline uint32_t seam_lead(uint32_t w) { return w & 0xffffu; }
+__host__ __device__ inline uint32_t seam_trail(uint32_t w) { return w >> 16; }
+
+__host__ __device__ inline uint32_t seam_word_of(uint32_t bits, uint32_t first, uint32_t last, uint32_t prev,
+                                                 bool have_prev)
+{
+    if (bits == 0u) return 0u;
+    const uint32_t f = bits >= 32u ? first : first | (0xffffffffu >> bits);
+    uint32_t lead = f ? (uint32_t)__builtin_clz(f) : SEAM_CAP;
+    if (lead > SEAM_CAP && lead < bits) lead = SEAM_CAP;
+    const uint32_t r = bits - 32u * ((bits - 1u) >> 5);
+    const uint32_t l = last >> (32u - r);
+    uint32_t trail;
+    if (l) {
+        trail = (uint32_t)__builtin_ctz(l);
+    } else if (bits <= 32u) {
+        trail = bits;
+    } else if (have_prev && prev) {
+        trail = r + (uint32_t)__builtin_ctz(prev);
+    } else {
+        trail = SEAM_CAP;
+    }
+    if (trail > SEAM_CAP && trail < bits) trail = SEAM_CAP;
+    return lead | trail << 16;
+}
+
+__host__ __device__ inline bool seam_walk(int k, uint32_t bl, uint32_t sl, uint32_t br, uint32_t sr)
+{
+    if (k == 0) return true;
+    const uint32_t t = seam_trail(sl), l = seam_lead(sr);
+    if (t >= SEAM_CAP || l >= SEAM_CAP) return true;
+    if (t >= bl || l >= br) return true;
+    return t + l >= EP_RUN_BITS;
+}
+
+}
+}
+
+#endif
```

Measured after the change: 3.123 million frames/s. Within noise of the previous version (-0.4%).
